# gphocs-dev/G-PhoCS

Hardware: AMD Instinct MI355X
Metric: locus-likelihood evals/sec (+ MCMC iters/sec), 100k loci, 1/2/4/8 MI355X (higher is better)
Workload: dtype f64

## Files before the change

g-phocs_amd/csrc/gph_backend.h:

```cpp
#pragma once

struct GphGrid { int x, y; };


#ifdef GPH_HOSTEMU
#define SETDEV(e) ((void)0)

struct gph_engine : gph_engine_state {
  std::vector<char> lds;
};

static int dev_alloc(void **p, size_t bytes) { *p = calloc(1, bytes ? bytes : 1); return *p ? 0 : GPH_EHIP; }
static void dev_free(void *p) { free(p); }
static int h2d(gph_engine *, void *d, const void *h, size_t n) { memcpy(d, h, n); return 0; }
static int d2h(gph_engine *, void *h, const void *d, size_t n) { memcpy(h, d, n); return 0; }
static int acc_zero(gph_engine *, void *p, size_t bytes) { if (p) memset(p, 0, bytes); return 0; }
static int stream_sync(gph_engine *e) { e->n_syncs++; return 0; }
static int collect_times(gph_engine *) { return 0; }
static int tm_begin(gph_engine *, int) { return -1; }
static void tm_end(gph_engine *, int) {}
static int push_G(gph_engine *e) { e->G_dirty = false; return 0; }
static int pull_G(gph_engine *e) { e->n_syncs++; return 0; }
static int pull_row(gph_engine *e) { memcpy(e->h_red, e->d_red, sizeof(double) * GPH_RED_ROW); e->n_syncs++; return 0; }
static bool resident(const gph_engine *) { return false; }
static int flush_pending(gph_engine *) { return 0; }
static int stage_defer(gph_engine *, int, int, int, bool &queued) { queued = false; return 0; }
static void flat_launched(gph_engine *, int, int) {}

static int reduce_local(gph_engine *e, int sec, int ncols)
{
  double *red = e->d_red + sec * GPH_RED_STRIDE;
  for (int c = 0; c < ncols; c++) {
    double s = 0, mn = 1e300, mx = -1e300;
    for (int64_t g = 0; g < e->L; g++) {
      double v;
      if (sec == 0) v = e->dev.out[(size_t)g * GPH_OUT_SLOTS + c];
      else v = e->dev.stats[(size_t)g * ncols + c];
      s += v; mn = v < mn ? v : mn; mx = v > mx ? v : mx;
    }
    red[c] = s; red[GPH_RED_COLS + c] = mn; red[2 * GPH_RED_COLS + c] = mx;
  }
  red[3 * GPH_RED_COLS] = (double)*e->dev.err;
  return 0;
}

static int backend_open(gph_engine *e)
{
  e->G_h = (GphGlobal *)calloc(1, sizeof(GphGlobal));
  e->G_d = e->G_h;
  e->h_red = (double *)calloc(GPH_RED_ROW, sizeof(double));
  e->d_red = (double *)calloc(GPH_RED_ROW, sizeof(double));
  e->d_gather = e->d_red;
  return 0;
}
static void backend_close(gph_engine *e) { free(e->h_red); free(e->G_h); }
static int wide_terms_bytes(int P) { return 8 * P; }
static int zero_error_word(gph_engine *e) { if (e->dev.err) *e->dev.err = 0; return 0; }
static int loci_loaded(gph_engine *) { return 0; }
static int scan_lds_limit(gph_engine *) { return 0; }
static int peer_stream(gph_engine *, gph_comm *) { return 0; }
static void runtime_version(char *buf, size_t n) { snprintf(buf, n, "host emulation (no HIP runtime)"); }
#ifdef GPH_BOUNDS
static int oob_take(int32_t *where) { *where = gph_oob_word; gph_oob_word = 0; return 0; }
#endif

static void launch_pre(gph_engine *e)
{
  g_model = e->G_h->model; g_lay = e->lay; gph_G_emu = e->G_h;
  GPH_KA_MODEL(e->ka, e); e->ka.lay = e->lay; e->ka.G = e->G_h;
}
template <class... P, class... A>
static int launch_loci(gph_engine *e, int cls, void (*kernel)(int, GphKargs, GphDev, int, P...), A &&...args)
{
  launch_pre(e);
  for (auto &bk : e->buckets) {
    e->lds.assign(bk.lds_bytes + 8 * e->lay.Pmax + 64, 0);
    gph_sm = e->lds.data();
    for (int b = 0; b < bk.count; b++) kernel(b, e->ka, e->dev, bk.j0, static_cast<P>(args)...);
  }
  e->last_which = cls; e->cls_launches[cls] += 1; e->n_launches++;
  return 0;
}
template <class... P, class... A>
static int launch_wave(gph_engine *e, int cls, void (*kernel)(int, GphKargs, GphDev, int, P...), size_t lds_bytes, A &&...args)
{
  launch_pre(e);
  e->lds.assign(lds_bytes + 64, 0);
  gph_sm = e->lds.data();
  kernel(0, e->ka, e->dev, 0, static_cast<P>(args)...);
  e->last_which = cls; e->cls_launches[cls] += 1;
  return 0;
}
template <class... P, class... A>
static int run_blocks(std::vector<char> &lds, GphGrid grid, int block, size_t lds_bytes, void (*kernel)(GphBlk, P...), A &&...args)
{
  for (int x = 0; x < grid.x; x++)
    for (int y = 0; y < grid.y; y++) {
      lds.assign(lds_bytes + 64, 0);
      kernel(GphBlk{x, y, block, lds.data()}, static_cast<P>(args)...);
    }
  return 0;
}
template <class... P, class... A>
static int launch_grid(gph_engine *e, GphGrid grid, int block, size_t lds_bytes, void (*kernel)(GphBlk, P...), A &&...args)
{
  return run_blocks(e->lds, grid, block, lds_bytes, kernel, args...);
}

static int debug_math(const double *x, const double *y, int n, double *out, int)
{
  GphKargs ka;
  memset(&ka, 0, sizeof ka);
  fill_math_constants(ka);
  std::vector<char> lds;
  return run_blocks(lds, GphGrid{(n + 255) / 256, 1}, 256, 0, k_debug_math, ka, x, y, n, out);
}

#else
#define HIPCHK(x) do { hipError_t e_ = (x); if (e_ != hipSuccess) { fprintf(stderr, "gphocs_hip: %s failed: %s (%s:%d)\n", #x, hipGetErrorString(e_), __FILE__, __LINE__); return GPH_EHIP; } } while (0)
#define SETDEV(e) do { if (hipSetDevice((e)->cfg.device) != hipSuccess) return GPH_EHIP; } while (0)

struct gph_engine : gph_engine_state {
  unsigned *d_ticket = nullptr;
  int pend_nc0 = 0, pend_nc1 = 0;
  GphStageList pend_sl = {0, {0}, {0}};
  int pend_iteration = 0;
  hipStream_t stream = nullptr;
  hipStream_t stream_wide = nullptr;
  hipEvent_t ev_fork = nullptr, ev_join = nullptr;
  bool side_stream = true;
  struct Tm { hipEvent_t a, b; int which; };
  std::vector<Tm> tm;
  size_t tm_used = 0;
};

static int dev_alloc(void **p, size_t bytes) { return hipMalloc(p, bytes ? bytes : 16) == hipSuccess ? 0 : GPH_EHIP; }
static void dev_free(void *p) { if (p) (void)hipFree(p); }
static int collect_times(gph_engine *e)
{
  for (size_t i = 0; i < e->tm_used; i++) {
    float ms = 0;
    if (hipEventElapsedTime(&ms, e->tm[i].a, e->tm[i].b) == hipSuccess) { e->last_ms[e->tm[i].which] = ms; e->cls_ms[e->tm[i].which] += ms; }
  }
  e->tm_used = 0;
  return 0;
}
static int stream_sync(gph_engine *e)
{
  HIPCHK(hipStreamSynchronize(e->stream));
  e->n_syncs++;
  return collect_times(e);
}
static int h2d(gph_engine *e, void *d, const void *h, size_t n)
{
  HIPCHK(hipMemcpyAsync(d, h, n, hipMemcpyHostToDevice, e->stream));
  HIPCHK(hipStreamSynchronize(e->stream));
  return 0;
}
static int d2h(gph_engine *e, void *h, const void *d, size_t n)
{
  HIPCHK(hipMemcpyAsync(h, d, n, hipMemcpyDeviceToHost, e->stream));
  HIPCHK(hipStreamSynchronize(e->stream));
  return 0;
}
static int acc_zero(gph_engine *e, void *p, size_t bytes)
{
  if (p) HIPCHK(hipMemsetAsync(p, 0, bytes, e->stream));
  return 0;
}
static int tm_begin(gph_engine *e, int which)
{
  if (!((e->timing_mask >> which) & 1)) return -1;
  if (e->tm_used == e->tm.size()) {
    gph_engine::Tm t;
    if (hipEventCreate(&t.a) != hipSuccess || hipEventCreate(&t.b) != hipSuccess) return -1;
    e->tm.push_back(t);
  }
  e->tm[e->tm_used].which = which;
  (void)hipEventRecord(e->tm[e->tm_used].a, e->stream);
  return (int)e->tm_used++;
}
static void tm_end(gph_engine *e, int slot) { if (slot >= 0) (void)hipEventRecord(e->tm[slot].b, e->stream); }
static int push_G(gph_engine *e)
{
  e->G_dirty = false;
  return h2d(e, e->G_d, e->G_h, sizeof(GphGlobal));
}
static int pull_G(gph_engine *e)
{
  HIPCHK(hipMemcpyAsync(e->G_h, e->G_d, sizeof(GphGlobal), hipMemcpyDeviceToHost, e->stream));
  { int rcs = stream_sync(e); if (rcs) return rcs; }
  e->mirror_current = true;
  return 0;
}
static int pull_row(gph_engine *e)
{
  HIPCHK(hipMemcpyAsync(e->h_red, e->d_red, sizeof(double) * GPH_RED_ROW, hipMemcpyDeviceToHost, e->stream));
  return stream_sync(e);
}
static bool resident(const gph_engine *e)
{
  if (e->force_host || e->allreduce || e->var_rates) return false;
  if (e->comm && !gph_comm_on_stream(e->comm)) return false;
  return true;
}
static void flat_launched(gph_engine *e, int cls, int k) { e->n_launches += k; if (cls >= 0) e->last_which = cls; }

static void launch_pre(gph_engine *e) { GPH_KA_MODEL(e->ka, e); e->ka.lay = e->lay; e->ka.G = e->G_d; }
template <class... P, class... A>
static int launch_on(hipStream_t stream, GphGrid grid, int block, size_t lds_bytes, void (*kernel)(P...), A &&...args)
{
  hipLaunchKernelGGL(kernel, dim3((unsigned)grid.x, (unsigned)grid.y), dim3((unsigned)block), lds_bytes, stream, static_cast<P>(args)...);
  HIPCHK(hipGetLastError());
  return 0;
}
template <class... P, class... A>
static int launch_grid(gph_engine *e, GphGrid grid, int block, size_t lds_bytes, void (*kernel)(P...), A &&...args)
{
  return launch_on(e->stream, grid, block, lds_bytes, kernel, args...);
}

static int flush_pending(gph_engine *e)
{
  const bool red = e->pend_nc0 > 0 || e->pend_nc1 > 0;
  if (!red && e->pend_sl.n == 0) return 0;
  const GphStageList sl = e->pend_sl;
  const int nc0 = e->pend_nc0, nc1 = e->pend_nc1;
  e->pend_nc0 = e->pend_nc1 = 0;
  e->pend_sl.n = 0;
  const bool multi = e->comm && gph_comm_world(e->comm) > 1;
  int rc;
  launch_pre(e);
  if (red) {
    const bool inkernel = multi && e->peer_rows != nullptr;
    const int fuse = sl.n > 0 && (!multi || inkernel);
    GphPeerX X{1, 0, 0, 0, nullptr, nullptr, nullptr, 0};
    if (inkernel) X = GphPeerX{gph_comm_world(e->comm), gph_comm_rank(e->comm), e->peer_stride, 0, e->peer_rows, e->peer_flags, e->d_gather, gph_comm_peer_next_gen(e->comm)};
    if ((rc = launch_grid(e, GphGrid{GPH_RED_BLOCKS, 1}, GPH_RED_THREADS, 0, k_reduce_stage, e->ka, e->dev, nc0, nc1, e->d_part, e->d_ticket,
                          e->d_red, fuse, sl, e->pend_iteration, X))) return rc;
    e->n_launches++;
    if (inkernel) {
      e->n_collectives++;
    } else if (multi) {
      if (gph_comm_allgather_stream(e->comm, e->d_red, e->d_gather, GPH_RED_ROW, (void *)e->stream)) return GPH_EHIP;
      e->n_collectives++;
    } else if (e->comm) {
      e->n_collectives++;
      if (gph_comm_allgather_stream(e->comm, e->d_red, e->d_gather, GPH_RED_ROW, (void *)e->stream)) return GPH_EHIP;
    }
    if (fuse) return 0;
  }
  if (sl.n > 0) {
    const double *rows = e->comm ? e->d_gather : e->d_red;
    if ((rc = launch_grid(e, GphGrid{1, 1}, GPH_RED_THREADS, 0, k_global, e->ka, rows, world_of(e), sl, e->pend_iteration))) return rc;
    e->n_launches++;
  }
  return 0;
}
static int reduce_local(gph_engine *e, int sec, int ncols)
{
  if (resident(e)) {
    if (e->pend_sl.n > 0) { int rcf = flush_pending(e); if (rcf) return rcf; }
    if (sec == 0) e->pend_nc0 = ncols; else e->pend_nc1 = ncols;
    return 0;
  }
  int rc;
  if ((rc = flush_pending(e))) return rc;
  GphStageList none = {0, {0}, {0}};
  launch_pre(e);
  if ((rc = launch_grid(e, GphGrid{GPH_RED_BLOCKS, 1}, GPH_RED_THREADS, 0, k_reduce_stage, e->ka, e->dev, sec == 0 ? ncols : 0, sec == 1 ? ncols : 0,
                        e->d_part, e->d_ticket, e->d_red, 0, none, 0, GphPeerX{1, 0, 0, 0, nullptr, nullptr, nullptr, 0}))) return rc;
  e->n_launches += 1;
  return 0;
}
static int stage_defer(gph_engine *e, int stage, int arg, int iteration, bool &queued)
{
  queued = resident(e);
  if (!queued) return flush_pending(e);
  if (e->pend_sl.n == 6) { int rcf = flush_pending(e); if (rcf) return rcf; }
  e->pend_sl.stage[e->pend_sl.n] = stage;
  e->pend_sl.arg[e->pend_sl.n] = arg;
  e->pend_sl.n++;
  e->pend_iteration = iteration;
  e->mirror_current = false;
  return 0;
}

template <class... P, class... A>
static int launch_loci(gph_engine *e, int cls, void (*kernel)(GphKargs, GphDev, int, P...), A &&...args)
{
  { int rcf = flush_pending(e); if (rcf) return rcf; }
  launch_pre(e);
  const int tms = tm_begin(e, cls);
  const size_t nb = e->buckets.size();
  const bool fork = e->side_stream && nb >= 2;
  if (fork) { HIPCHK(hipEventRecord(e->ev_fork, e->stream)); HIPCHK(hipStreamWaitEvent(e->stream_wide, e->ev_fork, 0)); }
  for (size_t bi = 0; bi < nb; bi++) {
    const gph_engine::Bucket &bk = e->buckets[bi];
    e->ka.lay.dyn_bytes = bk.lds_bytes;
    { int rcl = launch_on(fork && bi + 1 < nb ? e->stream_wide : e->stream, GphGrid{bk.count, 1}, GPH_WAVE, bk.lds_bytes + e->lds_pad[cls],
                          kernel, e->ka, e->dev, bk.j0, args...); if (rcl) return rcl; }
    e->n_launches++;
  }
  if (fork) { HIPCHK(hipEventRecord(e->ev_join, e->stream_wide)); HIPCHK(hipStreamWaitEvent(e->stream, e->ev_join, 0)); }
  tm_end(e, tms);
  e->last_which = cls; e->cls_launches[cls] += 1;
  return 0;
}
template <class... P, class... A>
static int launch_wave(gph_engine *e, int cls, void (*kernel)(GphKargs, GphDev, int, P...), size_t lds_bytes, A &&...args)
{
  { int rcf = flush_pending(e); if (rcf) return rcf; }
  launch_pre(e);
  const int tms = tm_begin(e, cls);
  { int rcl = launch_on(e->stream, GphGrid{1, 1}, GPH_WAVE, lds_bytes, kernel, e->ka, e->dev, 0, args...); if (rcl) return rcl; }
  tm_end(e, tms);
  e->last_which = cls; e->cls_launches[cls] += 1;
  return 0;
}

static int fill_math_tables(GphKargs &ka)
{
  void *p = nullptr;
  if (hipGetSymbolAddress(&p, HIP_SYMBOL(gph_log_t_d)) != hipSuccess) return 1;
  ka.log_t = (const double *)p;
  if (hipGetSymbolAddress(&p, HIP_SYMBOL(gph_exp_t_d)) != hipSuccess) return 1;
  ka.exp_t = (const uint64_t *)p;
  return 0;
}
static int backend_open(gph_engine *e)
{
  int ndev = 0;
  if (hipGetDeviceCount(&ndev) != hipSuccess || ndev <= e->cfg.device) {
    fprintf(stderr, "gphocs_hip: no usable HIP device %d (found %d) -- this library has no CPU path\n", e->cfg.device, ndev);
    return GPH_EHIP;
  }
  if (hipSetDevice(e->cfg.device) != hipSuccess || fill_math_tables(e->ka)) {
    fprintf(stderr, "gphocs_hip: cannot resolve the device math tables\n");
    return GPH_EHIP;
  }
  if (const char *ov = getenv("GPH_SIDE_STREAM")) e->side_stream = atoi(ov) != 0;
  const bool nb_ = getenv("GPH_NONBLOCKING_STREAM") && atoi(getenv("GPH_NONBLOCKING_STREAM")) != 0;
  if ((nb_ ? hipStreamCreateWithFlags(&e->stream, hipStreamNonBlocking) : hipStreamCreate(&e->stream)) != hipSuccess ||
      hipStreamCreateWithFlags(&e->stream_wide, hipStreamNonBlocking) != hipSuccess ||
      hipEventCreateWithFlags(&e->ev_fork, hipEventDisableTiming) != hipSuccess || hipEventCreateWithFlags(&e->ev_join, hipEventDisableTiming) != hipSuccess ||
      hipHostMalloc((void **)&e->G_h, sizeof(GphGlobal), hipHostMallocDefault) != hipSuccess ||
      hipMalloc((void **)&e->G_d, sizeof(GphGlobal)) != hipSuccess ||
      hipHostMalloc((void **)&e->h_red, sizeof(double) * GPH_RED_ROW * 64, hipHostMallocDefault) != hipSuccess ||
      hipMalloc((void **)&e->d_red, sizeof(double) * GPH_RED_ROW) != hipSuccess ||
      hipMemset(e->d_red, 0, sizeof(double) * GPH_RED_ROW) != hipSuccess ||
      hipMalloc((void **)&e->d_ticket, 64) != hipSuccess || hipMemset(e->d_ticket, 0, 64) != hipSuccess ||
      hipStreamSynchronize(nullptr) != hipSuccess) return GPH_EHIP;
  e->d_gather = e->d_red;
  return 0;
}
static void backend_close(gph_engine *e)
{
  dev_free(e->G_d);
  dev_free(e->d_ticket);
  if (e->h_red) (void)hipHostFree(e->h_red);
  if (e->G_h) (void)hipHostFree(e->G_h);
  for (auto &t : e->tm) { (void)hipEventDestroy(t.a); (void)hipEventDestroy(t.b); }
  if (e->ev_fork) (void)hipEventDestroy(e->ev_fork);
  if (e->ev_join) (void)hipEventDestroy(e->ev_join);
  if (e->stream_wide) (void)hipStreamDestroy(e->stream_wide);
  if (e->stream) (void)hipStreamDestroy(e->stream);
}
static int wide_terms_bytes(int) { return 0; }
static int zero_error_word(gph_engine *e)
{
  return hipMemset(e->dev.err, 0, sizeof(int32_t)) != hipSuccess || hipStreamSynchronize(nullptr) != hipSuccess ? GPH_EHIP : 0;
}
static int loci_loaded(gph_engine *e)
{
  const void *ks[] = {(const void *)k_init, (const void *)k_sweep, (const void *)k_tau_eval, (const void *)k_tau_finish,
                      (const void *)k_mix_eval, (const void *)k_mix_finish,
                      (const void *)k_sync, (const void *)k_check, (const void *)k_lrate_apply, (const void *)k_lrate_prep,
                      (const void *)k_unit};
  int pad_max = 0;
  if (const char *pe = getenv("GPH_LDS_PAD")) {
    for (const char *q = pe; *q;) {
      int w = -1, by = 0;
      if (sscanf(q, "%d:%d", &w, &by) == 2 && w >= 0 && w < 16 && by >= 0) { e->lds_pad[w] = by; pad_max = by > pad_max ? by : pad_max; }
      while (*q && *q != ',') q++;
      if (*q == ',') q++;
    }
  }
  if (e->lay.lds_bytes + pad_max + (int)sizeof(GphLds) > 160 * 1024) {
    fprintf(stderr, "gphocs_hip: %d-byte image + %d-byte sequence block%s = %d bytes of LDS per locus, the CU has %d%s\n", (int)sizeof(GphLds),
            e->lay.lds_bytes, pad_max ? " + GPH_LDS_PAD" : "", e->lay.lds_bytes + pad_max + (int)sizeof(GphLds), 160 * 1024,
            getenv("GPH_HUGE_LDS") ? " (GPH_HUGE_LDS is set: lower it, the block then stays in HBM)" : "");
    return GPH_EARG;
  }
  for (auto k : ks) HIPCHK(hipFuncSetAttribute(k, hipFuncAttributeMaxDynamicSharedMemorySize, e->lay.lds_bytes + pad_max));
  return 0;
}
static int scan_lds_limit(gph_engine *e)
{
  HIPCHK(hipFuncSetAttribute((const void *)k_lrate_scan, hipFuncAttributeMaxDynamicSharedMemorySize, e->lr_lds_bytes));
  return 0;
}
static int peer_stream(gph_engine *e, gph_comm *c)
{
  if (!(c && gph_comm_world(c) > 1 && gph_comm_on_stream(c))) return 0;
  double *rows = nullptr; unsigned long long *flags = nullptr; int32_t stride = 0;
  int least_ = 0, greatest_ = 0;
  if (hipDeviceGetStreamPriorityRange(&least_, &greatest_) != hipSuccess) { least_ = greatest_ = 0; }
  const int levels_ = least_ - greatest_ + 1;
  if (gph_comm_peer_exchange(c, &rows, &flags, &stride) && stride >= GPH_RED_ROW && gph_comm_world(c) > levels_) {
    if (gph_comm_rank(c) == 0)
      fprintf(stderr, "gphocs_hip: the in-kernel exchange is offered for up to %d thread ranks on one device (one stream priority level "
                      "each); %d ranks use the event-ordered gather\n", levels_, gph_comm_world(c));
  } else if (gph_comm_peer_exchange(c, &rows, &flags, &stride) && stride >= GPH_RED_ROW) {
    e->peer_rows = rows; e->peer_flags = flags; e->peer_stride = stride;
    hipStream_t ns = nullptr;
    int least = 0, greatest = 0;
    if (hipDeviceGetStreamPriorityRange(&least, &greatest) != hipSuccess) { least = greatest = 0; }
    const int levels = least - greatest + 1;
    const int prio = levels > 1 ? least - (gph_comm_rank(c) % levels) : 0;
    if (hipStreamSynchronize(e->stream) != hipSuccess || hipStreamCreateWithPriority(&ns, hipStreamNonBlocking, prio) != hipSuccess) return GPH_EHIP;
    (void)hipStreamDestroy(e->stream);
    e->stream = ns;
  }
  return 0;
}
static void runtime_version(char *buf, size_t n)
{
  int rt = 0, dr = 0;
  if (hipRuntimeGetVersion(&rt) != hipSuccess) rt = -1;
  if (hipDriverGetVersion(&dr) != hipSuccess) dr = -1;
  snprintf(buf, n, "HIP runtime %d, driver %d", rt, dr);
}
#ifdef GPH_BOUNDS
static int oob_take(int32_t *where)
{
  int w = 0, z = 0;
  HIPCHK(hipMemcpyFromSymbol(&w, HIP_SYMBOL(gph_oob_word), sizeof(int)));
  if (w != 0) HIPCHK(hipMemcpyToSymbol(HIP_SYMBOL(gph_oob_word), &z, sizeof(int)));
  *where = w;
  return 0;
}
#endif
static int debug_math(const double *x, const double *y, int n, double *out, int device)
{
  double *dx = nullptr, *dy = nullptr, *dout = nullptr;
  HIPCHK(hipSetDevice(device));
  HIPCHK(hipMalloc((void **)&dx, sizeof(double) * n));
  HIPCHK(hipMalloc((void **)&dy, sizeof(double) * n));
  HIPCHK(hipMalloc((void **)&dout, sizeof(double) * 5 * n));
  HIPCHK(hipMemcpy(dx, x, sizeof(double) * n, hipMemcpyHostToDevice));
  HIPCHK(hipMemcpy(dy, y, sizeof(double) * n, hipMemcpyHostToDevice));
  GphKargs ka;
  memset(&ka, 0, sizeof ka);
  fill_math_constants(ka);
  if (fill_math_tables(ka)) return GPH_EHIP;
  { int rcl = launch_on(nullptr, GphGrid{(n + 255) / 256, 1}, 256, 0, k_debug_math, ka, dx, dy, n, dout); if (rcl) return rcl; }
  HIPCHK(hipMemcpy(out, dout, sizeof(double) * 5 * n, hipMemcpyDeviceToHost));
  (void)hipFree(dx); (void)hipFree(dy); (void)hipFree(dout);
  return 0;
}
#endif
```

g-phocs_amd/csrc/gph_engine.hip:

```cpp
#include <stdio.h>
#include <stdlib.h>
#include <stddef.h>
#include <string.h>
#include <vector>
#include <string>
#include <algorithm>
#if defined(GPH_HOSTEMU) && defined(GPH_EMU64)
#define GPH_EMU64_IMPL
#endif
#include "gph_kernels.h"
#include "gph_global.h"
#include "gph_summary.h"
#include "gph_coalstats.h"
#include "gph_timeslices.h"
#include "gph_ancestry.h"
#include "gph_genetrees.h"
#include "gph_comm.h"
#include "../../include/gphocs_hip.h"

#ifdef GPH_HOSTEMU
thread_local char *gph_sm = nullptr;
thread_local GphLds gph_lds;
GphLayout g_lay;
GphModel g_model;
// ... 140 lines not shown
      if (col < ncols) reduce_run(src, stride, col, g0 + q, g1, GPH_RED_SUBS, s, mn, mx);
      for (int c0 = 64 * half; c0 < ncols && c0 < 64 * (half + 1); c0 += 16) {
        __syncthreads();
        if (col >= c0 && col < c0 + 16) { sh[0][q][col - c0] = s; sh[1][q][col - c0] = mn; sh[2][q][col - c0] = mx; }
        __syncthreads();
        if (threadIdx.x < 16 && c0 + (int)threadIdx.x < ncols) {
          const int c = threadIdx.x;
          double ts = 0.0, tmn = 1e300, tmx = -1e300;
          for (int k = 0; k < GPH_RED_SUBS; k++) {
            ts += sh[0][k][c];
            tmn = sh[1][k][c] < tmn ? sh[1][k][c] : tmn;
            tmx = sh[2][k][c] > tmx ? sh[2][k][c] : tmx;
          }
          part[(0 * GPH_RED_BLOCKS + b) * GPH_RED_COLS + c0 + c] = ts;
          part[(1 * GPH_RED_BLOCKS + b) * GPH_RED_COLS + c0 + c] = tmn;
          part[(2 * GPH_RED_BLOCKS + b) * GPH_RED_COLS + c0 + c] = tmx;
        }
      }
    }
    __syncthreads();
    return;
  }
  const int ng = 64 / cw, Q = GPH_RED_SUBS * ng;
  const int lane = threadIdx.x & 63, col = lane % cw, q = (threadIdx.x >> 6) * ng + lane / cw;
  double s = 0.0, mn = 1e300, mx = -1e300;
  if (col < ncols) reduce_run(src, stride, col, g0 + q, g1, Q, s, mn, mx);
  for (int c0 = 0; c0 < ncols; c0 += 16) {
    __syncthreads();
    if (col >= c0 && col < c0 + 16) { sh[0][q][col - c0] = s; sh[1][q][col - c0] = mn; sh[2][q][col - c0] = mx; }
    __syncthreads();
    if (threadIdx.x < 16 && c0 + (int)threadIdx.x < ncols) {
      const int c = threadIdx.x;
      double ts = 0.0, tmn = 1e300, tmx = -1e300;
      for (int k = 0; k < Q; k++) {
        ts += sh[0][k][c];
        tmn = sh[1][k][c] < tmn ? sh[1][k][c] : tmn;
        tmx = sh[2][k][c] > tmx ? sh[2][k][c] : tmx;
      }
      part[(0 * GPH_RED_BLOCKS + b) * GPH_RED_COLS + c0 + c] = ts;
      part[(1 * GPH_RED_BLOCKS + b) * GPH_RED_COLS + c0 + c] = tmn;
      part[(2 * GPH_RED_BLOCKS + b) * GPH_RED_COLS + c0 + c] = tmx;
    }
  }
  __syncthreads();
}
__device__ void reduce_final_body(int ncols, int cbase, const double *part, double *red, double (*sh)[GPH_RED_SUBS][128])
{
  part += cbase; red += cbase;
  const int cw = ncols <= 64 ? 64 : 128;
  const int col = threadIdx.x % cw, h = threadIdx.x / cw;
  const int per = GPH_RED_BLOCKS / GPH_RED_SUBS;
  static_assert((GPH_RED_BLOCKS / GPH_RED_SUBS) % 16 == 0, "the final pass folds sixteen block partials per step");
  for (int sub = h; sub < GPH_RED_SUBS; sub += GPH_RED_THREADS / cw) {
    double s = 0.0, mn = 1e300, mx = -1e300;
    if (col < ncols)
      for (int b0 = sub * per; b0 < (sub + 1) * per; b0 += 16) {
        double vs[16], vn[16], vx[16];
#pragma unroll
        for (int u = 0; u < 16; u++) {
          vs[u] = part[(0 * GPH_RED_BLOCKS + b0 + u) * GPH_RED_COLS + col];
          vn[u] = part[(1 * GPH_RED_BLOCKS + b0 + u) * GPH_RED_COLS + col];
          vx[u] = part[(2 * GPH_RED_BLOCKS + b0 + u) * GPH_RED_COLS + col];
        }
#pragma unroll
        for (int u = 0; u < 16; u++) { s += vs[u]; mn = vn[u] < mn ? vn[u] : mn; mx = vx[u] > mx ? vx[u] : mx; }
      }
    if (col < 128) { sh[0][sub][col] = s; sh[1][sub][col] = mn; sh[2][sub][col] = mx; }
  }
  __syncthreads();
  if (h == 0 && col < ncols) {
    double s = 0.0, mn = 1e300, mx = -1e300;
    for (int k = 0; k < GPH_RED_SUBS; k++) {
      s += sh[0][k][col];
      mn = sh[1][k][col] < mn ? sh[1][k][col] : mn;
      mx = sh[2][k][col] > mx ? sh[2][k][col] : mx;
    }
    red[col] = s;
    red[GPH_RED_COLS + col] = mn;
    red[2 * GPH_RED_COLS + col] = mx;
  }
  __syncthreads();
}
struct GphPeerX { int world, rank, stride, pad; double *rows; unsigned long long *flags; double *gather; unsigned long long gen; };
__global__ void __launch_bounds__(GPH_RED_THREADS) k_reduce_stage(GphKargs KA, GphDev D, int nc0, int nc1, double *part, unsigned *ticket, double *red,
                                                                  int do_stage, GphStageList SL, int iteration, GphPeerX X)
{
  __shared__ union { double p[3][GPH_RED_SUBS * 4][16]; double f[3][GPH_RED_SUBS][128]; GphStageShared st; } sh;
  __shared__ int s_last;
  if (nc0 > 0) reduce_partial_body(D, 0, nc0, 0, nc0, part, sh.p);
  for (int cb = 0; cb < nc1; cb += 128) reduce_partial_body(D, 1, nc1 - cb < 128 ? nc1 - cb : 128, cb, nc1, part + 3 * GPH_RED_BLOCKS * GPH_RED_COLS, sh.p);
  __syncthreads();
  if (threadIdx.x == 0) { __threadfence(); s_last = atomicAdd(ticket, 1u) == gridDim.x - 1; }
  __syncthreads();
  if (!s_last) return;
  __builtin_amdgcn_fence(__ATOMIC_ACQUIRE, "agent");
  if (nc0 > 0) reduce_final_body(nc0, 0, part, red, sh.f);
  for (int cb = 0; cb < nc1; cb += 128) reduce_final_body(nc1 - cb < 128 ? nc1 - cb : 128, cb, part + 3 * GPH_RED_BLOCKS * GPH_RED_COLS, red + GPH_RED_STRIDE, sh.f);
  if (threadIdx.x == 0) { red[3 * GPH_RED_COLS] = (double)*D.err; *ticket = 0; }
  __syncthreads();
  const double *rows = red;
  int world = 1;
  if (X.world > 1) {
    double *mine = X.rows + (size_t)(2 * X.rank + (int)(X.gen & 1)) * X.stride;
    for (int c = threadIdx.x; c < GPH_RED_ROW; c += blockDim.x) mine[c] = red[c];
    __threadfence_system();
    __syncthreads();
    if (threadIdx.x == 0) {
      __atomic_thread_fence(__ATOMIC_RELEASE);
      __hip_atomic_store(&X.flags[X.rank], X.gen, __ATOMIC_RELEASE, __HIP_MEMORY_SCOPE_SYSTEM);
      const unsigned long long t0 = __builtin_amdgcn_s_memrealtime();
      for (int r = 0; r < X.world; r++) {
        while (__hip_atomic_load(&X.flags[r], __ATOMIC_ACQUIRE, __HIP_MEMORY_SCOPE_SYSTEM) < X.gen) {
          __builtin_amdgcn_s_sleep(32);
          if (__builtin_amdgcn_s_memrealtime() - t0 > 400000000ull) {
            atomicMax(D.err, 9997); red[3 * GPH_RED_COLS] = 9997.0; r = X.world; break; }
        }
      }
    }
    __syncthreads();
    __threadfence_system();
    for (int r = 0; r < X.world; r++) {
      const double *src = r == X.rank ? red : X.rows + (size_t)(2 * r + (int)(X.gen & 1)) * X.stride;
      for (int c = threadIdx.x; c < GPH_RED_ROW; c += blockDim.x) X.gather[(size_t)r * GPH_RED_ROW + c] = src[c];
    }
    __syncthreads();
    rows = X.gather; world = X.world;
  }
  if (do_stage) stages_body(KA, rows, world, SL, iteration, sh.st);
}
#endif

#ifdef GPH_HOSTEMU
static void k_debug_math(GphBlk b, GphKargs KA, const double *x, const double *y, int n, double *o)
{
  (void)KA;
  for (int i = b.x * b.dim; i < (b.x + 1) * b.dim && i < n; i++) {
    o[i] = gph_exp(x[i]); o[n + i] = gph_log(x[i]); o[2 * n + i] = sqrt(fabs(x[i]));
    o[3 * n + i] = x[i] / y[i]; o[4 * n + i] = floor(x[i]);
  }
}
#else
__global__ void k_debug_math(GphKargs KA, const double *x, const double *y, int n, double *o)
{
  int i = blockIdx.x * blockDim.x + threadIdx.x;
  if (i >= n) return;
  o[i] = gph_exp(x[i]);
  o[n + i] = gph_log(x[i]);
  o[2 * n + i] = sqrt(fabs(x[i]));
  o[3 * n + i] = x[i] / y[i];
  o[4 * n + i] = floor(x[i]);
}
#endif

#define GPH_NCLS 18
struct SmRows {
  char *d = nullptr;
  size_t esz = 0;
  int32_t n = 0, cap = 0, fill = 0;
};
struct SmParts {
  double *d_part = nullptr;
  int32_t rd = 0, chunk = 0, nchunks = 0;
  int32_t chunk_next = 0;
};

struct gph_engine_state {
  gph_config cfg;
  std::vector<int32_t> samplesPerPop, popFather, popSon0, popSon1, bandSrc, bandTgt;
  GphLayout lay;
  GphDev dev;
  GphGlobal *G_h = nullptr, *G_d = nullptr;
  bool G_dirty = true;
  int64_t n_huge = 0;
  double *peer_rows = nullptr;
  unsigned long long *peer_flags = nullptr;
  std::vector<void *> deferred_free;
  int32_t peer_stride = 0;
  int32_t last_error_code = 0;
  long long last_error_locus = -1;
  bool in_error_dump = false;
  int64_t L = 0;
  size_t cond_bytes = 0, pages_bytes = 0, seq_bytes_total = 0;
  std::vector<uint64_t> h_cond_off;
  std::vector<int32_t> h_P;
  std::vector<int32_t> h_orig;
  struct Bucket { int j0, count, lds_bytes; };
  std::vector<Bucket> buckets;
  double *d_mutRate = nullptr;
  int init_predraws = 0;
  bool var_rates = false;
  GphLrRec *d_lrec = nullptr;
  GphLrPre *d_lpre = nullptr;
  double lr_hits = 0;
  int32_t *d_slot_of = nullptr;
  double *d_lr_result = nullptr, *d_lr_gscr = nullptr;
  char *d_ref_page = nullptr, *d_ref_seq = nullptr;
  std::vector<uint64_t> h_seq_off;
  GphLrArgs lr;
  int lr_lds_bytes = 0;
  int lds_pad[16] = {0};
  double *d_part = nullptr, *d_red = nullptr, *d_gather = nullptr;
  double *h_red = nullptr;
  gph_comm *comm = nullptr;
  gph_allreduce_fn allreduce = nullptr;
  void *allreduce_user = nullptr;
  bool force_host = false;
  int64_t n_syncs = 0, n_collectives = 0, n_launches = 0;
  uint32_t seedz = 0;
  bool loaded = false, seeded = false, model_set = false, initialized = false;
  GphKargs ka;
  bool sync_pending = false;
  bool fin_owed = false;
  bool mix_owed = false;
  int32_t slog_sel = 0;
  bool mirror_current = true;
  bool no_fuse = false;
  gph_counters counters = {0, 0, 0.0, 0};
  struct { double *d = nullptr; int32_t ncol = 0; int64_t samples = 0; std::vector<std::string> names; } ls;
  struct { SmParts part; SmRows rows; int32_t bd = 0; std::string name; } cs;
  struct { SmParts part; SmRows rows; GphTsShape shape = {}; std::string name; } ts;
  struct { double *d_acc = nullptr; SmRows rows; int32_t ncol = 0; int64_t samples = 0; GphAnShape shape = {}; std::vector<int32_t> iters; std::string name; } an;
  struct { SmRows rows; GphGtShape shape = {}; int32_t *d_sel = nullptr; std::vector<int64_t> sel; std::vector<int32_t> iters; } gt;
  double last_ms[GPH_NCLS] = {0};
  double cls_launches[GPH_NCLS] = {0}, cls_ms[GPH_NCLS] = {0};
  double cls_evals0[16] = {0}, cls_bytes0[16] = {0}, cls_nodes0[16] = {0};
  int last_which = 0;
  uint32_t timing_mask = 0xffffffffu;
};

static int align_up(int x, int a) { return (x + a - 1) / a * a; }

static void build_layout(GphLayout &y, int n, int Kc, int K, int B, int rootPop, int Pmax, int cnt16)
{
  memset(&y, 0, sizeof y);
  y.n = n; y.N = 2 * n - 1; y.K = K; y.Kc = Kc; y.B = B; y.rootPop = rootPop;
  y.E = 2 * n + 4 * GPH_MAX_MIGS + 3 * B + K + 10;
  y.RB = GPH_MAX_MIGS + 2 * B;
#define OFS(f) ((int32_t)offsetof(GphLds, f))
  y.o_ev = OFS(ev); y.o_nd = OFS(nd); y.o_sv = OFS(sv); y.o_mig_age = OFS(mig_age);
  y.o_coal = OFS(coal); y.o_migst = OFS(migst); y.o_rb_age = OFS(rb_age); y.o_fscal = OFS(fscal);
  y.o_iscal = OFS(iscal);
  y.o_nev = OFS(nev);
  y.o_first = OFS(first);
  y.o_mig_i = OFS(mig_i); y.o_living = OFS(living); y.o_ncoal = OFS(ncoal); y.o_nmig = OFS(nmig); y.o_rb_i = OFS(rb_i);
  y.page_bytes = align_up(OFS(s_dcoal), 16);
#undef OFS
  y.Pmax = Pmax;
  y.cnt16 = cnt16;
  y.dyn_bytes = 0;
  y.lds_bytes = GPH_Q_TERMS(Pmax, n, cnt16) + (Pmax > GPH_WAVE ? 8 * Pmax : 8 * GPH_WAVE);
  y.huge_P = 0x7fffffff;
}

static void build_model_static(gph_engine_state *e)
{
  GphModel &m = e->G_h->model;
  const gph_config &c = e->cfg;
  memset(&m, 0, sizeof m);
  for (int p = 0; p < c.K; p++) {
    m.popFather[p] = e->popFather[p];
    m.popSon0[p] = e->popSon0[p];
    m.popSon1[p] = e->popSon1[p];
    gph_popmask mask = 0;
    for (int d = 0; d < c.K; d++) {
      int x = d;
      while (x >= 0) { if (x == p) { mask |= (gph_popmask)1 << d; break; } x = e->popFather[x]; }
    }
    m.isAnc[p] = mask;
  }
  int cum = 0;
  for (int p = 0; p < c.Kc; p++) { m.samplesPerPop[p] = e->samplesPerPop[p]; cum += e->samplesPerPop[p]; m.cumSamples[p] = cum; }
  for (int b = 0; b < c.B; b++) { m.bandSrc[b] = e->bandSrc[b]; m.bandTgt[b] = e->bandTgt[b]; m.bandsInto[e->bandTgt[b]][b >> 5] |= 1u << (b & 31); }
  for (int p = 0; p < c.K; p++)
    for (int b = 0; b < c.B; b++) if ((m.isAnc[e->bandTgt[b]] >> p) & 1) m.bandsOver[p][b >> 5] |= 1u << (b & 31);
  std::vector<int> order;
  struct Rec { static void go(gph_engine_state *e, int pop, std::vector<int> &o) {
    if (pop >= e->cfg.Kc) { go(e, e->popSon0[pop], o); go(e, e->popSon1[pop], o); }
    o.push_back(pop); } };
  Rec::go(e, c.rootPop, order);
  for (size_t i = 0; i < order.size(); i++) m.postOrder[i] = order[i];
  GphGlobal &G = *e->G_h;
  G.n = c.n; G.K = c.K; G.Kc = c.Kc; G.B = c.B; G.rootPop = c.rootPop; G.Ltot = (double)c.L_total;
  G.tau_limit = (long long)1 << 62;
}

#ifdef GPH_WALKSTAT
long long gph_ws[4];
struct GphWsPrint { ~GphWsPrint() { fprintf(stderr, "WALKSTAT proposals %lld: prune steps %.2f, regraft steps %.2f, common prefix %.2f per proposal\n", gph_ws[3], (double)gph_ws[0] / gph_ws[3], (double)gph_ws[1] / gph_ws[3], (double)gph_ws[2] / gph_ws[3]); } } gph_ws_print;
#endif
#if GPH_BIG_BANDS
#define GPH_KA_MODEL(ka, e) ((void)0)
#else
#define GPH_KA_MODEL(ka, e) ((ka).model = (e)->G_h->model)
#endif
static void fill_math_constants(GphKargs &ka)
{
  const double ec[8] = GPH_EXP_CONSTS, lc[18] = GPH_LOG_CONSTS;
  const double rc[6] = {1.0 / 30269.0, 1.0 / 30307.0, 1.0 / 30323.0, 30269.0, 30307.0, 30323.0};
  memcpy(&ka.mathc[0], ec, sizeof ec);
  memcpy(&ka.mathc[8], lc, sizeof lc);
  memcpy(&ka.mathc[26], rc, sizeof rc);
}
static int world_of(const gph_engine *e);
#include "gph_backend.h"
static int world_of(const gph_engine *e) { return e->comm ? gph_comm_world(e->comm) : 1; }
static int push_if_dirty(gph_engine *e) { return e->G_dirty ? push_G(e) : 0; }

static int reduce_stats(gph_engine *e) { return reduce_local(e, 1, 2 * e->cfg.K + 2 * e->cfg.B); }

struct StageCols { int ns = 0, nm = 0, nx = 0; int s[GPH_RED_COLS + 32][2], m[8][2], x[8][2]; };
static void stage_columns(const gph_engine *e, int stage, StageCols &c)
{
  const int C = 2 * e->cfg.K + 2 * e->cfg.B;
  auto S = [&](int sec, int col) { c.s[c.ns][0] = sec; c.s[c.ns][1] = col; c.ns++; };
  auto M = [&](int sec, int col) { c.m[c.nm][0] = sec; c.m[c.nm][1] = col; c.nm++; };
  auto X = [&](int sec, int col) { c.x[c.nx][0] = sec; c.x[c.nx][1] = col; c.nx++; };
  auto counters = [&]() { S(0, 8); S(0, 9); S(0, 10); S(0, 13); X(0, 11); X(0, -1); };
  auto totals = [&]() { for (int k = 0; k < C; k++) S(1, k); };
  switch (stage) {
  case GS_INIT_DONE: counters(); S(0, 0); S(0, 1); totals(); break;
  case GS_SWEEP_DONE: counters(); for (int k = 0; k < 8; k++) S(0, k); S(0, 12); M(0, 15); totals(); break;
  case GS_TOTALS: totals(); break;
  case GS_TAU_DECIDE: case GS_SAGE_DECIDE: counters(); S(0, 0); S(0, 1); S(0, 3); S(0, 4); M(0, 14); break;
  case GS_MIX_DECIDE: counters(); S(0, 0); break;
  case GS_REFRESH_DONE: counters(); M(0, 0); S(0, 1); S(0, 2); break;
  case GS_CHECK_DONE: counters(); M(0, 0); S(0, 1); S(0, 2); totals(); break;
  case GS_COUNT_ONLY: counters(); S(0, 0); S(0, 1); S(0, 3); S(0, 4); M(0, 14); break;
  default: break;
  }
}
static bool stage_reads_row(int stage)
{
  switch (stage) {
  case GS_INIT_DONE: case GS_SWEEP_DONE: case GS_TOTALS: case GS_TAU_DECIDE: case GS_SAGE_DECIDE: case GS_MIX_DECIDE:
  case GS_REFRESH_DONE: case GS_CHECK_DONE: case GS_COUNT_ONLY: return true;
  default: return false;
  }
}
static double *colp(double *row, const int sc[2], int kind)
{
  if (sc[1] < 0) return row + 3 * GPH_RED_COLS;
  return row + sc[0] * GPH_RED_STRIDE + kind * GPH_RED_COLS + sc[1];
}

static int run_stage(gph_engine *e, int stage, int arg, int iteration)
{
  int rc;
  bool queued;
  if ((rc = stage_defer(e, stage, arg, iteration, queued)) || queued) return rc;
  GphRed R;
  R.rows = e->h_red; R.world = 1;
  if (stage_reads_row(stage)) {
    if ((rc = pull_row(e))) return rc;
    if (e->allreduce || e->comm) {
      StageCols c;
      stage_columns(e, stage, c);
      double sums[GPH_RED_COLS + 32], mins[16];
      for (int k = 0; k < c.ns; k++) sums[k] = *colp(e->h_red, c.s[k], 0);
      for (int k = 0; k < c.nm; k++) mins[k] = *colp(e->h_red, c.m[k], 1);
      for (int k = 0; k < c.nx; k++) mins[c.nm + k] = -*colp(e->h_red, c.x[k], 2);
      if (e->allreduce) rc = e->allreduce(e->allreduce_user, sums, c.ns, mins, c.nm + c.nx);
      else rc = gph_comm_allreduce_host(e->comm, sums, c.ns, mins, c.nm + c.nx);
      if (rc) return GPH_EHIP;
      e->n_collectives++;
      for (int k = 0; k < c.ns; k++) *colp(e->h_red, c.s[k], 0) = sums[k];
      for (int k = 0; k < c.nm; k++) *colp(e->h_red, c.m[k], 1) = mins[k];
      for (int k = 0; k < c.nx; k++) *colp(e->h_red, c.x[k], 2) = -mins[c.nm + k];
    }
  }
  e->G_h->iteration = iteration;
  gg_stage(*e->G_h, R, stage, arg);
  return push_G(e);
}

static void dump_one_locus(const gph_engine *e, FILE *f, long long global_locus, const char *pg, const char *cb, int P)
{
  const GphLayout &y = e->lay;
  const double *fs = (const double *)(pg + y.o_fscal);
  const int32_t *is = (const int32_t *)(pg + y.o_iscal);
  const GphNode *nd = (const GphNode *)(pg + y.o_nd);
  const int16_t *ne = (const int16_t *)(pg + y.o_nev);
  const int16_t *first = (const int16_t *)(pg + y.o_first);
  const GphEv *evr = (const GphEv *)(pg + y.o_ev);
  fprintf(f, "LOCUS %lld root %d dataLnL %a genLnL %a rng %u %u %u\n", (long long)global_locus, is[IS_ROOT],
          fs[FS_DATALNL], fs[FS_GENLNL], (unsigned)is[IS_RX], (unsigned)is[IS_RY], (unsigned)is[IS_RZ]);
  if (e->var_rates) fprintf(f, "R %a\n", fs[FS_MUTRATE]);
  for (int i = 0; i < y.N; i++)
    fprintf(f, "N %d %d %d %d %a %d %d\n", i, nd[i].father, nd[i].left, nd[i].right, nd[i].age, nd[i].npop, i < y.n ? -1 : ne[i]);
  for (int pop = 0; pop < y.K; pop++) {
    fprintf(f, "C %d", pop);
    int guard = 0;
    for (int ev = first[pop]; ev >= 0 && guard++ < y.E; ev = evr[ev].next)
      fprintf(f, " %d:%d:%d:%d:%a", ev, evr[ev].type, evr[ev].node, evr[ev].nlin, evr[ev].time);
    fprintf(f, "\n");
  }
  fprintf(f, "S");
  for (int pop = 0; pop < y.K; pop++)
    fprintf(f, " %a %d", ((const double *)(pg + y.o_coal))[pop], ((const int16_t *)(pg + y.o_ncoal))[pop]);
  for (int b = 0; b < y.B; b++)
    fprintf(f, " %a %d", ((const double *)(pg + y.o_migst))[b], ((const int16_t *)(pg + y.o_nmig))[b]);
  fprintf(f, "\n");
  fprintf(f, "M %d", is[IS_NUM_MIGS]);
  for (int i = 0; i < is[IS_NUM_MIGS]; i++) {
    int mg = ((const int16_t *)(pg + y.o_living))[i];
    const int16_t *mi = (const int16_t *)(pg + y.o_mig_i) + mg * MG_COUNT;
    fprintf(f, " %d:%d:%d:%d:%d:%d:%d:%a", mg, mi[MG_BRANCH], mi[MG_BAND], mi[MG_SPOP], mi[MG_TPOP], mi[MG_SEV],
            mi[MG_TEV], ((const double *)(pg + y.o_mig_age))[mg]);
  }
  fprintf(f, "\n");
  if (cb) {
    for (int i = y.n; i < y.N; i++) {
      const double *c = (const double *)(cb + ((size_t)((int)(((uint32_t)is[IS_CBIT0 + (i >> 5)] >> (i & 31)) & 1) * (y.n - 1) + (i - y.n)) * P) * 32);
      fprintf(f, "K %d", i);
      for (int k = 0; k < 4 * P; k++) fprintf(f, " %a", c[k]);
      fprintf(f, "\n");
    }
  }
}

static void eng_free(gph_engine *e, void *p)
{
  if (!p) return;
  if (e->peer_rows) e->deferred_free.push_back(p);
  else dev_free(p);
}

static int check_error(gph_engine *e)
{
  const int code = e->G_h->error;
  if (code != 0) {
    const long long gl = e->G_h->error_locus;
    e->last_error_code = code;
    e->last_error_locus = gl;
    if (code == 75) fprintf(stderr, "gphocs_hip: synchronizeEvents found an inconsistency (Fatal Error 0075/0076)\n");
    else if (code == 9999) fprintf(stderr, "gphocs_hip: checkAll failed at iteration %d\n", e->G_h->iteration);
    else if (gl >= 0) fprintf(stderr, "gphocs_hip: Fatal Error %04d reported by a locus kernel, first in locus %lld (iteration %d)\n", code, gl, e->G_h->iteration);
    else fprintf(stderr, "gphocs_hip: Fatal Error %04d reported by a locus kernel\n", code);
    const long long lo = gl - e->cfg.locus_begin;
    if (gl >= 0 && lo >= 0 && lo < e->L && !e->in_error_dump) {
      e->in_error_dump = true;
      int64_t slot = -1;
      for (int64_t j = 0; j < e->L; j++) if (e->h_orig[j] == lo) { slot = j; break; }
      std::vector<char> pg(e->lay.page_bytes);
      if (slot >= 0 && !d2h(e, pg.data(), (const char *)e->dev.pages + (size_t)slot * e->lay.page_bytes, e->lay.page_bytes)) {
        fprintf(stderr, "gphocs_hip: genealogy and event chains of locus %lld:\n", gl);
        dump_one_locus(e, stderr, gl, pg.data(), nullptr, 0);
      }
      e->in_error_dump = false;
    }
    return GPH_EKERNEL;
  }
  return 0;
}
static int finish_sync(gph_engine *e)
{
  { int rcf = flush_pending(e); if (rcf) return rcf; }
  if (resident(e)) { int rc = pull_G(e); if (rc) return rc; }
  return check_error(e);
}

static int run_stage_now(gph_engine *e, int stage, int arg);
static int mix_finish_owed(gph_engine *e)
{
  if (!e->mix_owed) return 0;
  e->mix_owed = false;
  return launch_loci(e, 7, k_mix_finish, 0);
}
static int flush_sync(gph_engine *e, bool now)
{
  int rc;
  if ((rc = mix_finish_owed(e))) return rc;
  if (!e->sync_pending) return 0;
  e->sync_pending = false;
  if ((rc = push_if_dirty(e))) return rc;
  if ((rc = launch_loci(e, 8, k_sync, 0))) return rc;
  if ((rc = reduce_local(e, 0, GPH_OUT_SLOTS))) return rc;
  if (now) return run_stage_now(e, GS_REFRESH_DONE, 0);
  return run_stage(e, GS_REFRESH_DONE, 0, e->G_h->iteration);
}

static int run_stage_now(gph_engine *e, int stage, int arg)
{
  const bool fh = e->force_host;
  e->force_host = true;
  int rc = run_stage(e, stage, arg, e->G_h->iteration);
  e->force_host = fh;
  if (rc) return rc;
  return check_error(e);
}

extern "C" {

int gph_engine_create(const gph_config *cfg, gph_engine **out)
{
  if (!cfg || !out) return GPH_EARG;
  if (cfg->n > 200 || cfg->K > 39 || cfg->B > 100)
    fprintf(stderr, "gphocs_hip: n=%d K=%d B=%d exceed even the reference's compile-time caps (NS 200, 2*NSPECIES-1 = 39, MAX_MIG_BANDS 100: upstream src/patch.h:17-22)\n", cfg->n, cfg->K, cfg->B);
  if (cfg->n < 2 || cfg->n > GPH_CAP_LEAVES || cfg->K > GPH_CAP_K || cfg->B > GPH_CAP_B || cfg->K != 2 * cfg->Kc - 1) {
    fprintf(stderr, "gphocs_hip: unsupported dimensions n=%d K=%d B=%d (this library variant: n<=%d leaves, K<=%d populations, B<=%d bands; the largest variant covers the reference's own caps 200 / 39 / 100, upstream src/patch.h:17-22)\n",
            cfg->n, cfg->K, cfg->B, GPH_CAP_LEAVES, GPH_CAP_K, GPH_CAP_B);
    return GPH_EARG;
  }
  gph_engine *e = new gph_engine();
  e->cfg = *cfg;
  e->samplesPerPop.assign(cfg->samplesPerPop, cfg->samplesPerPop + cfg->Kc);
  e->popFather.assign(cfg->popFather, cfg->popFather + cfg->K);
  e->popSon0.assign(cfg->popSon0, cfg->popSon0 + cfg->K);
  e->popSon1.assign(cfg->popSon1, cfg->popSon1 + cfg->K);
  if (cfg->B > 0) { e->bandSrc.assign(cfg->bandSrc, cfg->bandSrc + cfg->B); e->bandTgt.assign(cfg->bandTgt, cfg->bandTgt + cfg->B); }
  e->cfg.samplesPerPop = e->samplesPerPop.data();
  e->cfg.popFather = e->popFather.data();
  e->cfg.popSon0 = e->popSon0.data();
  e->cfg.popSon1 = e->popSon1.data();
  e->cfg.bandSrc = e->bandSrc.data();
  e->cfg.bandTgt = e->bandTgt.data();
  memset(&e->dev, 0, sizeof e->dev);
  memset(&e->ka, 0, sizeof e->ka);
  fill_math_constants(e->ka);
  if (const char *fh = getenv("GPH_HOST_DECISIONS")) e->force_host = atoi(fh) != 0;
  if (const char *nf = getenv("GPH_NO_FUSE")) e->no_fuse = atoi(nf) != 0;
  if (int rc = backend_open(e)) { gph_engine_destroy(e); return rc; }
  memset(e->G_h, 0, sizeof(GphGlobal));
  e->G_h->error_locus = -1;
  build_model_static(e);
  *out = e;
  return 0;
}

void gph_engine_destroy(gph_engine *e)
{
  if (!e) return;
  dev_free(e->dev.pages); dev_free(e->dev.shadow); dev_free(e->dev.cond); dev_free((void *)e->dev.cond_off);
  dev_free((void *)e->dev.seq); dev_free((void *)e->dev.seq_off); dev_free((void *)e->dev.orig); dev_free((void *)e->dev.P); dev_free(e->dev.out); dev_free(e->dev.stats); dev_free(e->d_mutRate);
  dev_free(e->d_lrec); dev_free(e->d_lpre); dev_free(e->d_slot_of); dev_free(e->d_lr_result); dev_free(e->d_lr_gscr); dev_free(e->d_ref_page); dev_free(e->d_ref_seq);
  dev_free(e->d_part); dev_free(e->dev.err);
  dev_free(e->ls.d); dev_free(e->cs.part.d_part); dev_free(e->cs.rows.d); dev_free(e->ts.part.d_part); dev_free(e->ts.rows.d);
  dev_free(e->an.d_acc); dev_free(e->an.rows.d);
  dev_free(e->gt.rows.d); dev_free(e->gt.d_sel);
  for (void *p : e->deferred_free) dev_free(p);
  e->deferred_free.clear();
  dev_free((void *)e->dev.slog_map); dev_free(e->dev.slog); dev_free(e->dev.slog_n);
  if (e->d_gather != e->d_red) dev_free(e->d_gather);
  dev_free(e->d_red);
  backend_close(e);
  delete e;
}

int gph_engine_set_allreduce(gph_engine *e, gph_allreduce_fn fn, void *user)
{
  if (!e) return GPH_EARG;
  e->allreduce = fn;
  e->allreduce_user = user;
  return 0;
}

int gph_engine_set_comm(gph_engine *e, gph_comm *c)
{
  if (!e) return GPH_EARG;
  SETDEV(e);
  e->comm = c;
  if (e->d_gather != e->d_red) { dev_free(e->d_gather); e->d_gather = e->d_red; }
  if (c && gph_comm_world(c) > 1 && gph_comm_on_stream(c)) {
    if (gph_comm_world(c) > 64) return GPH_EARG;
    if (dev_alloc((void **)&e->d_gather, sizeof(double) * GPH_RED_ROW * gph_comm_world(c))) return GPH_EHIP;
  }
  e->peer_rows = nullptr; e->peer_flags = nullptr; e->peer_stride = 0;
  return peer_stream(e, c);
}

GphGlobal *gph_engine_global_(gph_engine *e) { if (!e) return nullptr; e->G_dirty = true; return e->G_h; }
const GphGlobal *gph_engine_global_ro_(gph_engine *e) { return e ? e->G_h : nullptr; }

int gph_engine_load_loci(gph_engine *e, int64_t L, const int64_t *poff, const uint8_t *leafcodes,
                         const uint16_t *numPhases, const int32_t *counts, const double *mutRates)
{
  if (!e || L <= 0 || !poff || !leafcodes || !numPhases || !counts) return GPH_EARG;
  if (e->loaded) { fprintf(stderr, "gphocs_hip: gph_engine_load_loci called twice on one engine\n"); return GPH_ESTATE; }
  SETDEV(e);
  const int n = e->cfg.n;
  int Pmax = 1;
  for (int64_t g = 0; g < L; g++) { int P = (int)(poff[g + 1] - poff[g]); if (P > Pmax) Pmax = P; if (P < 0) return GPH_EARG; }
  int cnt16 = 1;
  for (int64_t i = 0; i < poff[L]; i++) if (counts[i] < 0 || counts[i] > 65535) { cnt16 = 0; break; }
  if (const char *ov = getenv("GPH_CNT16")) cnt16 = cnt16 && atoi(ov) != 0;
  build_layout(e->lay, n, e->cfg.Kc, e->cfg.K, e->cfg.B, e->cfg.rootPop, Pmax, cnt16);
  {
    int budget = 32 * 1024;
    if (budget < (int)sizeof(GphLds) + 16 * 1024) budget = (int)sizeof(GphLds) + 16 * 1024;
    if (const char *ov = getenv("GPH_HUGE_LDS")) {
      budget = atoi(ov);
      if (budget <= 0) { fprintf(stderr, "gphocs_hip: GPH_HUGE_LDS=%s is not a byte count\n", ov); return GPH_EARG; }
    }
    if (budget > 160 * 1024) budget = 160 * 1024;
    int hp = GPH_WAVE;
    while (hp < Pmax && (int)sizeof(GphLds) + GPH_Q_BYTES(hp + 1, n, cnt16) <= budget) hp++;
    e->lay.huge_P = hp >= Pmax ? 0x7fffffff : hp;
  }
  e->L = L;
  e->h_orig.resize(L);
  for (int64_t g = 0; g < L; g++) e->h_orig[g] = (int32_t)g;
  std::stable_sort(e->h_orig.begin(), e->h_orig.end(), [&](int32_t a, int32_t b) {
    return (poff[a + 1] - poff[a]) > (poff[b + 1] - poff[b]); });
  e->buckets.clear();
  {
    int64_t nwide = 0, nhuge = 0;
    while (nhuge < L && (poff[e->h_orig[nhuge] + 1] - poff[e->h_orig[nhuge]]) > e->lay.huge_P) nhuge++;
    nwide = nhuge;
    while (nwide < L && (poff[e->h_orig[nwide] + 1] - poff[e->h_orig[nwide]]) > GPH_WAVE) nwide++;
    e->n_huge = nhuge;
    if (nhuge > 0 && e->cfg.locus_begin == 0)
      fprintf(stderr, "gphocs_hip: %lld loci with more than %d phased patterns (up to %d) keep their sequence block in HBM\n",
              (long long)nhuge, e->lay.huge_P, Pmax);
    if (nhuge > 0) {
      gph_engine::Bucket bk;
      bk.j0 = 0; bk.count = (int)nhuge;
      bk.lds_bytes = 64;
      e->buckets.push_back(bk);
    }
    if (nwide > nhuge) {
      const int pw = (int)(poff[e->h_orig[nhuge] + 1] - poff[e->h_orig[nhuge]]);
      gph_engine::Bucket bk;
      bk.j0 = (int)nhuge; bk.count = (int)(nwide - nhuge);
      bk.lds_bytes = GPH_Q_TERMS(pw, n, cnt16) + wide_terms_bytes(pw);
      e->buckets.push_back(bk);
    }
    if (nwide < L) {
      const int pn = (int)(poff[e->h_orig[nwide] + 1] - poff[e->h_orig[nwide]]);
      gph_engine::Bucket bk;
      bk.j0 = (int)nwide; bk.count = (int)(L - nwide);
      bk.lds_bytes = GPH_Q_BYTES(pn, n, cnt16);
      {
        auto resident = [](int bytes) { const int g = (bytes + 1279) / 1280; const int w = 128 / g; return w < 4 * GPH_SWEEP_WAVES_ ? w : 4 * GPH_SWEEP_WAVES_; };
        const int base = (int)sizeof(GphLds) + bk.lds_bytes;
        const int full = 8 * ((pn + 7) & ~7);
        e->lay.lds_sum = 1;
        if (resident(base + full) == resident(base)) bk.lds_bytes += full;
        else {
          int room = (base + 1279) / 1280 * 1280;
          while (resident(room + 1280) == resident(base)) room += 1280;
          bk.lds_bytes = (room - (int)sizeof(GphLds)) & ~15;
        }
        if (const char *ov = getenv("GPH_LDS_SUM")) {
          e->lay.lds_sum = atoi(ov) != 0;
          bk.lds_bytes = GPH_Q_BYTES(pn, n, cnt16) + (e->lay.lds_sum ? full : 0);
        }
      }
      e->buckets.push_back(bk);
    }
  }
  e->lay.lds_bytes = 0;
  for (auto &bk : e->buckets) if (bk.lds_bytes > e->lay.lds_bytes) e->lay.lds_bytes = bk.lds_bytes;
  e->h_cond_off.resize(L + 1);
  e->h_P.resize(L);
  std::vector<uint64_t> seq_off(L + 1);
  std::vector<double> rates(L, 1.0);
  uint64_t off = 0, soff = 0;
  for (int64_t j = 0; j < L; j++) {
    int64_t g = e->h_orig[j];
    int P = (int)(poff[g + 1] - poff[g]);
    e->h_P[j] = P;
    e->h_cond_off[j] = off;
    off += (uint64_t)2 * (n - 1) * P * 32;
    seq_off[j] = soff;
    soff += GPH_Q_BYTES(P, n, cnt16);
    if (P > e->lay.huge_P) soff += (uint64_t)8 * ((P + 1) & ~1);
    if (mutRates) rates[j] = mutRates[g];
  }
  e->h_cond_off[L] = off;
  seq_off[L] = soff;
  e->h_seq_off = seq_off;
  std::vector<char> seq(soff, 0);
  for (int64_t j = 0; j < L; j++) {
    int64_t g = e->h_orig[j];
    int P = e->h_P[j];
    char *blk = seq.data() + seq_off[j];
    for (int p = 0; p < P; p++) {
      for (int i = 0; i < n; i++) {
        uint8_t c = leafcodes[(size_t)(poff[g] + p) * n + i];
        if (c > 4) return GPH_EARG;
        blk[GPH_Q_LEAF + p * GPH_Q_NH(n) + (i >> 1)] |= (char)(c << ((i & 1) << 2));
      }
      ((uint16_t *)(blk + GPH_Q_PHASES(P, n)))[p] = numPhases[poff[g] + p];
      if (cnt16) ((uint16_t *)(blk + GPH_Q_COUNT(P, n)))[p] = (uint16_t)counts[poff[g] + p];
      else ((int32_t *)(blk + GPH_Q_COUNT(P, n)))[p] = counts[poff[g] + p];
    }
  }
  e->cond_bytes = off;
  e->seq_bytes_total = soff;
  e->pages_bytes = (size_t)L * e->lay.page_bytes;
  int rc = 0;
  rc |= dev_alloc((void **)&e->dev.pages, e->pages_bytes);
  rc |= dev_alloc((void **)&e->dev.shadow, e->pages_bytes);
  rc |= dev_alloc((void **)&e->dev.cond, e->cond_bytes);
  rc |= dev_alloc((void **)&e->dev.cond_off, sizeof(uint64_t) * (L + 1));
  rc |= dev_alloc((void **)&e->dev.seq, seq.size());
  rc |= dev_alloc((void **)&e->dev.seq_off, sizeof(uint64_t) * (L + 1));
  rc |= dev_alloc((void **)&e->dev.P, sizeof(int32_t) * 2 * L);
  rc |= dev_alloc((void **)&e->dev.orig, sizeof(int32_t) * L);
  rc |= dev_alloc((void **)&e->dev.out, sizeof(double) * GPH_OUT_SLOTS * L);
  rc |= dev_alloc((void **)&e->dev.stats, sizeof(double) * (2 * e->cfg.K + 2 * e->cfg.B) * L);
  rc |= dev_alloc((void **)&e->d_part, sizeof(double) * 2 * 3 * GPH_RED_BLOCKS * GPH_RED_COLS);
  rc |= dev_alloc((void **)&e->dev.err, sizeof(int32_t));
  if (!rc) rc = zero_error_word(e);
  if (mutRates) rc |= dev_alloc((void **)&e->d_mutRate, sizeof(double) * L);
  if (rc) { fprintf(stderr, "gphocs_hip: device allocation failed\n"); return GPH_EHIP; }
  rc |= h2d(e, (void *)e->dev.cond_off, e->h_cond_off.data(), sizeof(uint64_t) * (L + 1));
  rc |= h2d(e, (void *)e->dev.seq, seq.data(), seq.size());
  rc |= h2d(e, (void *)e->dev.seq_off, seq_off.data(), sizeof(uint64_t) * (L + 1));
  {
    std::vector<int32_t> pu((size_t)2 * L);
    for (int64_t j = 0; j < L; j++) {
      const int64_t g = e->h_orig[j];
      int U = 0;
      for (int64_t p = poff[g]; p < poff[g + 1]; p++) U += numPhases[p] > 0;
      pu[2 * j] = e->h_P[j]; pu[2 * j + 1] = U;
    }
    rc |= h2d(e, (void *)e->dev.P, pu.data(), sizeof(int32_t) * 2 * L);
  }
  rc |= h2d(e, (void *)e->dev.orig, e->h_orig.data(), sizeof(int32_t) * L);
  if (mutRates) rc |= h2d(e, e->d_mutRate, rates.data(), sizeof(double) * L);
  if (rc) return GPH_EHIP;
  e->dev.L = (int32_t)L;
  e->dev.Ltot = (int32_t)e->cfg.L_total;
  e->dev.locus_begin = e->cfg.locus_begin;
  e->loaded = true;
  return loci_loaded(e);
}

int gph_engine_set_model(gph_engine *e, const double *theta, const double *popAge, const double *sampleAge,
                         const double *migRate, const double *bandStart, const double *bandEnd)
{
  if (!e || !theta || !popAge || !sampleAge) return GPH_EARG;
  GphModel &m = e->G_h->model;
  for (int p = 0; p < e->cfg.K; p++) { gg_set_theta(*e->G_h, p, theta[p]); m.popAge[p] = popAge[p]; m.sampleAge[p] = sampleAge[p]; }
  for (int b = 0; b < e->cfg.B; b++) { gg_set_mig(*e->G_h, b, migRate[b]); m.bandStart[b] = bandStart[b]; m.bandEnd[b] = bandEnd[b]; }
  e->model_set = true;
  e->G_dirty = true;
  return 0;
}

int gph_engine_seed(gph_engine *e, uint32_t seed)
{
  if (!e) return GPH_EARG;
  e->seedz = 170u * (seed % 178u) + 137u;
  e->seeded = true;
  return 0;
}

int gph_engine_init_genealogies(gph_engine *e, double *sumGen, double *sumData)
{
  if (!e || !e->loaded || !e->seeded || !e->model_set) return GPH_ESTATE;
  SETDEV(e);
  { int rcf = flush_pending(e); if (rcf) return rcf; }
  e->mix_owed = e->fin_owed = e->sync_pending = false;
  if (e->G_h->mix_flag || e->G_h->tau_flag) { e->G_h->mix_flag = 0; e->G_h->tau_flag = 0; e->G_dirty = true; }
  { int rcp = push_if_dirty(e); if (rcp) return rcp; }
  if (e->ls.d && e->ls.ncol != gph_ls_columns(e->cfg.K, e->cfg.B, e->var_rates)) { int rce = gph_engine_locus_summary_enable(e, 1); if (rce) return rce; }
  e->ls.samples = e->an.samples = 0;
  e->cs.rows.fill = e->ts.rows.fill = e->an.rows.fill = e->gt.rows.fill = 0;
  e->an.iters.clear();
  e->gt.iters.clear();
  { int rcz = acc_zero(e, e->ls.d, sizeof(double) * (size_t)e->ls.ncol * e->L); if (rcz) return rcz; }
  { int rcz = acc_zero(e, e->an.d_acc, sizeof(double) * (size_t)e->an.ncol * e->L); if (rcz) return rcz; }
  int rc = launch_loci(e, 3, k_init, e->seedz, e->d_mutRate, e->init_predraws);
  if (!rc) rc = reduce_local(e, 0, GPH_OUT_SLOTS);
  if (!rc) rc = reduce_stats(e);
  if (rc) return rc;
  e->G_h->nrec = 0;
  e->G_h->iteration = -1;
  if ((rc = run_stage_now(e, GS_INIT_DONE, 0))) return rc;
  { GphRed R; R.rows = e->h_red; R.world = 1;
    if (sumGen) *sumGen = R.sum(0, 0);
    if (sumData) *sumData = R.sum(0, 1); }
  e->initialized = true;
  return rc;
}

static int sweep_launch(gph_engine *e, int flags, double ftCoal, double ftMig, int &with_sync)
{
  int rc;
  with_sync = e->sync_pending ? 8 : 0;
  e->sync_pending = false;
  int with_mix = 0;
  if (e->mix_owed) {
    if (!e->mirror_current && (rc = finish_sync(e))) return rc;
    e->mix_owed = false;
    if (e->G_h->mix_flag) with_mix = 16;
  }
  if ((rc = launch_loci(e, 0, k_sweep, flags | with_sync | with_mix, ftCoal, ftMig, e->G_h->mix_c, e->G_h->mix_lnc))) return rc;
  if ((rc = reduce_local(e, 0, GPH_OUT_SLOTS))) return rc;
  return reduce_stats(e);
}

int gph_engine_genealogy_sweep(gph_engine *e, int32_t flags, double ftCoal, double ftMig, gph_sweep_result *out)
{
  if (!e || !e->initialized || !out) return GPH_ESTATE;
  SETDEV(e);
  int rc, with_sync;
  if ((rc = push_if_dirty(e))) return rc;
  GphGlobal &G = *e->G_h;
  const int64_t a0 = G.acc[0], a1 = G.acc[1], a2 = G.acc[2], a7 = G.acc[7];
  if ((rc = sweep_launch(e, flags, ftCoal, ftMig, with_sync))) return rc;
  if ((rc = run_stage_now(e, GS_SWEEP_DONE, with_sync))) return rc;
  GphRed R; R.rows = e->h_red; R.world = 1;
  out->accepted_internal = G.acc[0] - a0;
  out->accepted_mignode = G.acc[1] - a1;
  out->accepted_spr = G.acc[2] - a2;
  out->total_mig_nodes = G.acc[7] - a7;
  out->dData_internal = R.sum(0, 3);
  out->dLog_internal = R.sum(0, 4);
  out->dLog_mignode = R.sum(0, 5);
  out->dData_spr = R.sum(0, 6);
  out->dLog_spr = R.sum(0, 7);
  return 0;
}

int gph_engine_tau_evaluate(gph_engine *e, const gph_tau_args *a, gph_tau_result *out)
{
  if (!e || !e->initialized || !a || !out) return GPH_ESTATE;
  if (a->num_aff > 2 * GPH_MAXB) return GPH_EARG;
  SETDEV(e);
  { int rcs = flush_sync(e, true); if (rcs) return rcs; }
  GphTauArgs &A = e->G_h->tau;
  memset(&A, 0, sizeof A);
  A.ap = a->ap; A.son0 = a->son0; A.son1 = a->son1; A.isRoot = a->isRoot; A.num_aff = a->num_aff; A.mode = a->mode;
  A.tauold = a->tauold; A.taunew = a->taunew; A.taub0 = a->taub0; A.taub1 = a->taub1;
  A.taufactor0 = a->taufactor0; A.taufactor1 = a->taufactor1;
  for (int i = 0; i < a->num_aff; i++) {
    A.aff_bands[i] = a->aff_bands[i];
    A.start_or_end[i] = a->start_or_end[i];
    A.new_band_ages[i] = a->new_band_ages[i];
  }
  int rc = push_G(e);
  if (rc) return rc;
  if ((rc = launch_loci(e, 1, k_tau_eval, 0))) return rc;
  if ((rc = reduce_local(e, 0, GPH_OUT_SLOTS))) return rc;
  if ((rc = run_stage_now(e, GS_COUNT_ONLY, 1))) return rc;
  GphRed R; R.rows = e->h_red; R.world = 1;
  out->ntj0 = (int64_t)R.sum(0, 0);
  out->ntj1 = (int64_t)R.sum(0, 1);
  out->genDelta = R.sum(0, 3);
  out->dataDelta = R.sum(0, 4);
  out->first_conflict_locus = R.mn(0, 14) < 1e299 ? (int64_t)R.mn(0, 14) : -1;
  return 0;
}

static int tau_finish_now(gph_engine *e, int flag, long long limit)
{
  if (!e || !e->initialized) return GPH_ESTATE;
  SETDEV(e);
  e->G_h->tau_flag = flag;
  e->G_h->tau_limit = limit;
  gg_fill_fin(*e->G_h, flag, limit);
  int rc = push_G(e);
  if (rc) return rc;
  return launch_loci(e, 5, k_tau_finish, 0);
}
int gph_engine_tau_commit(gph_engine *e) { return tau_finish_now(e, 1, (long long)1 << 62); }
int gph_engine_tau_revert(gph_engine *e, int64_t first_conflict)
{
  return tau_finish_now(e, 0, first_conflict >= 0 ? (long long)first_conflict : (long long)1 << 62);
}

int gph_engine_mixing_evaluate(gph_engine *e, double c, double *dataDelta)
{
  if (!e || !e->initialized || !dataDelta) return GPH_ESTATE;
  SETDEV(e);
  { int rcs = flush_sync(e, true); if (rcs) return rcs; }
  e->G_h->mix_c = c;
  int rc = push_G(e);
  if (rc) return rc;
  if ((rc = launch_loci(e, 2, k_mix_eval, 0))) return rc;
  if ((rc = reduce_local(e, 0, GPH_OUT_SLOTS))) return rc;
  if ((rc = run_stage_now(e, GS_COUNT_ONLY, 2))) return rc;
  GphRed R; R.rows = e->h_red; R.world = 1;
  *dataDelta = R.sum(0, 0);
  return 0;
}

int gph_engine_mixing_commit(gph_engine *e, double c, double lnc)
{
  if (!e || !e->initialized) return GPH_ESTATE;
  SETDEV(e);
  e->G_h->mix_flag = 1; e->G_h->mix_c = c; e->G_h->mix_lnc = lnc;
  int rc = push_G(e);
  if (rc) return rc;
  return launch_loci(e, 7, k_mix_finish, 0);
}

int gph_engine_mixing_revert(gph_engine *e) { return e ? 0 : GPH_EARG; }

static int finish_owed(gph_engine *e);
static int owed_finishes(gph_engine *e)
{
  int rc = finish_owed(e);
  if (!rc) rc = mix_finish_owed(e);
  return rc;
}
static int apply_list(gph_engine *e)
{
  int rc;
  if ((rc = owed_finishes(e))) return rc;
  if ((rc = flush_pending(e))) return rc;
  launch_pre(e);
  if ((rc = launch_grid(e, GphGrid{(int)((e->L + 255) / 256), 1}, 256, 0, k_apply_list, e->ka, e->dev))) return rc;
  flat_launched(e, -1, 1);
  return 0;
}

static int apply_one(gph_engine *e, int kind, int idx, int limit, double lnc, double diff)
{
  if (!e || !e->initialized || idx < 0 || idx >= limit) return GPH_EARG;
  SETDEV(e);
  { int rco = owed_finishes(e); if (rco) return rco; }
  GphGlobal &G = *e->G_h;
  G.napply = 1;
  G.apply[0].kind = kind; G.apply[0].idx = idx; G.apply[0].lnc = lnc; G.apply[0].diff = diff;
  int rc = push_G(e);
  if (rc) return rc;
  return apply_list(e);
}
int gph_engine_apply_theta(gph_engine *e, int32_t pop, double lnc, double thetaold, double thetanew)
{
  return apply_one(e, 0, pop, e ? e->cfg.K : 0, lnc, (1 / thetanew - 1 / thetaold));
}
int gph_engine_apply_migrate(gph_engine *e, int32_t band, double lnc, double old_rate, double new_rate)
{
  return apply_one(e, 1, band, e ? e->cfg.B : 0, lnc, (new_rate - old_rate));
}

int gph_engine_get_totals(gph_engine *e, double *cs, double *nc, double *ms, double *nm)
{
  if (!e || !e->initialized) return GPH_ESTATE;
  SETDEV(e);
  const int K = e->cfg.K, B = e->cfg.B;
  int rc;
  if ((rc = push_if_dirty(e))) return rc;
  if ((rc = mix_finish_owed(e))) return rc;
  if ((rc = reduce_stats(e))) return rc;
  if ((rc = run_stage_now(e, GS_TOTALS, 0))) return rc;
  const GphGlobal &G = *e->G_h;
  for (int p = 0; p < K; p++) { if (cs) cs[p] = G.tot_coal[p]; if (nc) nc[p] = G.tot_ncoal[p]; }
  for (int b = 0; b < B; b++) { if (ms) ms[b] = G.tot_mig[b]; if (nm) nm[b] = G.tot_nmig[b]; }
  return rc;
}

int gph_engine_synchronize(gph_engine *e, int32_t refresh, double *oldGen, double *newGen)
{
  if (!e || !e->initialized) return GPH_ESTATE;
  SETDEV(e);
  if (!refresh) {
    e->sync_pending = true;
    if (oldGen) *oldGen = 0.0;
    if (newGen) *newGen = 0.0;
    return 0;
  }
  int rc;
  if ((rc = flush_sync(e, true))) return rc;
  if ((rc = push_if_dirty(e))) return rc;
  if ((rc = launch_loci(e, 8, k_sync, refresh))) return rc;
  if ((rc = reduce_local(e, 0, GPH_OUT_SLOTS))) return rc;
  if ((rc = run_stage_now(e, GS_REFRESH_DONE, 0))) return rc;
  GphRed R; R.rows = e->h_red; R.world = 1;
  if (oldGen) *oldGen = R.sum(0, 1);
  if (newGen) *newGen = R.sum(0, 2);
  return rc;
}

int gph_engine_check_all(gph_engine *e, int32_t *ok, double *sumData, double *sumGen)
{
  if (!e || !e->initialized) return GPH_ESTATE;
  SETDEV(e);
  int rc;
  if ((rc = flush_sync(e, true))) return rc;
  if ((rc = push_if_dirty(e))) return rc;
  if ((rc = launch_loci(e, 4, k_check, 0))) return rc;
  if ((rc = reduce_local(e, 0, GPH_OUT_SLOTS))) return rc;
  if ((rc = reduce_stats(e))) return rc;
  e->G_h->nrec = 0;
  rc = run_stage_now(e, GS_CHECK_DONE, 0);
  if (ok) *ok = e->G_h->error != 9999;
  if (e->G_h->error == 9999) { e->G_h->error = 0; e->G_h->error_locus = -1; e->G_dirty = true; rc = 0; }
  { GphRed R; R.rows = e->h_red; R.world = 1;
    if (sumData) *sumData = R.sum(0, 1);
    if (sumGen) *sumGen = R.sum(0, 2); }
  return rc;
}

int gph_engine_get_counters(gph_engine *e, gph_counters *out, int32_t reset)
{
  if (!e || !out) return GPH_EARG;
  const GphGlobal &G = *e->G_h;
  double ev = 0, nd = 0, by = 0;
  for (int k = 0; k < 16; k++) { ev += G.cls_evals[k]; nd += G.cls_nodes[k]; by += G.cls_bytes[k]; }
  out->evals = (int64_t)ev - e->counters.evals;
  out->eval_nodes = (int64_t)nd - e->counters.eval_nodes;
  out->eval_bytes = by - e->counters.eval_bytes;
  out->not_enough_migs = (int64_t)G.cnt_notenough - e->counters.not_enough_migs;
  if (reset) { e->counters.evals = (int64_t)ev; e->counters.eval_nodes = (int64_t)nd; e->counters.eval_bytes = by; e->counters.not_enough_migs = (int64_t)G.cnt_notenough; }
  return 0;
}

int gph_engine_last_kernel_ms(gph_engine *e, int32_t which, double *ms)
{
  if (!e || !ms || which < 0 || which >= GPH_NCLS) return GPH_EARG;
  *ms = e->last_ms[which];
  return 0;
}

int64_t gph_engine_num_loci(gph_engine *e) { return e ? e->L : 0; }

int gph_engine_class_stats(gph_engine *e, int32_t which, double *out5, int32_t reset)
{
  if (!e || !out5 || which < 0 || which >= GPH_NCLS) return GPH_EARG;
  const GphGlobal &G = *e->G_h;
  if (which >= 16) {
    out5[0] = e->cls_launches[which]; out5[1] = e->cls_ms[which]; out5[2] = out5[3] = out5[4] = 0.0;
    if (reset) e->cls_launches[which] = e->cls_ms[which] = 0;
    return 0;
  }
  out5[0] = e->cls_launches[which]; out5[1] = e->cls_ms[which]; out5[2] = G.cls_evals[which] - e->cls_evals0[which];
  out5[3] = G.cls_bytes[which] - e->cls_bytes0[which]; out5[4] = G.cls_nodes[which] - e->cls_nodes0[which];
  if (reset) {
    e->cls_launches[which] = e->cls_ms[which] = 0;
    e->cls_evals0[which] = G.cls_evals[which]; e->cls_bytes0[which] = G.cls_bytes[which]; e->cls_nodes0[which] = G.cls_nodes[which];
  }
  return 0;
}

int gph_engine_host_stats(gph_engine *e, int64_t *syncs, int64_t *collectives, int64_t *launches, int32_t *resident_mode)
{
  if (!e) return GPH_EARG;
  if (syncs) *syncs = e->n_syncs;
  if (collectives) *collectives = e->n_collectives;
  if (launches) *launches = e->n_launches;
  if (resident_mode) *resident_mode = resident(e) ? 1 : 0;
  return 0;
}
int gph_engine_set_timing(gph_engine *e, uint32_t class_mask)
{
  if (!e) return GPH_EARG;
  e->timing_mask = class_mask;
  return 0;
}

int gph_debug_math(const double *x, const double *y, int32_t n, double *out, int32_t device)
{
  if (!x || !y || !out || n <= 0) return GPH_EARG;
  return debug_math(x, y, n, out, device);
}

#ifndef GPH_BUILD_ID
#define GPH_BUILD_ID "unidentified"
#endif
const char *gph_build_id(void) { return GPH_BUILD_ID; }
const char *gph_build_compiler(void)
{
#ifdef __clang_version__
  return "clang " __clang_version__;
#else
  return "g++ " __VERSION__;
#endif
}
const char *gph_runtime_version(void)
{
  static char buf[96];
  runtime_version(buf, sizeof buf);
  return buf;
}

int gph_engine_steplog_enable(gph_engine *e, const int64_t *loci, int32_t n, int32_t cap)
{
#if !defined(GPH_LOGSTEPS) && !defined(GPH_BBCOUNT)
  (void)e; (void)loci; (void)n; (void)cap;
  return GPH_EARG;
#else
  if (!e || !e->loaded || n < 0 || cap < 1 || (n > 0 && !loci)) return GPH_EARG;
  SETDEV(e);
  if (e->initialized) { int rcs = flush_sync(e, true); if (!rcs) rcs = finish_sync(e); if (rcs) return rcs; }
  eng_free(e, (void *)e->dev.slog_map); eng_free(e, e->dev.slog); eng_free(e, e->dev.slog_n);
  e->dev.slog_map = nullptr; e->dev.slog = nullptr; e->dev.slog_n = nullptr; e->dev.slog_cap = 0;
  e->slog_sel = n;
  if (n == 0) return 0;
  std::vector<int32_t> map((size_t)e->L, -1);
  for (int64_t j = 0; j < e->L; j++)
    for (int k = 0; k < n; k++)
      if (e->h_orig[j] + e->cfg.locus_begin == loci[k]) map[j] = k;
  std::vector<int32_t> zero((size_t)n, 0);
  int32_t *d_map = nullptr, *d_n = nullptr;
  double *d_log = nullptr;
  if (dev_alloc((void **)&d_map, sizeof(int32_t) * e->L) || dev_alloc((void **)&d_log, sizeof(double) * 8 * (size_t)n * cap) ||
      dev_alloc((void **)&d_n, sizeof(int32_t) * n) ||
      h2d(e, d_map, map.data(), sizeof(int32_t) * e->L) || h2d(e, d_n, zero.data(), sizeof(int32_t) * n)) {
    eng_free(e, d_map); eng_free(e, d_log); eng_free(e, d_n);
    e->slog_sel = 0;
    return GPH_EHIP;
  }
  e->dev.slog_map = d_map; e->dev.slog = d_log; e->dev.slog_n = d_n;
  e->dev.slog_cap = cap;
  return 0;
#endif
}
int gph_engine_steplog_fetch(gph_engine *e, int32_t idx, double *out, int32_t max_records, int32_t *nrec, int32_t reset)
{
#if !defined(GPH_LOGSTEPS) && !defined(GPH_BBCOUNT)
  (void)e; (void)idx; (void)out; (void)max_records; (void)nrec; (void)reset;
  return GPH_EARG;
#else
  if (!e || !e->dev.slog || idx < 0 || idx >= e->slog_sel || !nrec) return GPH_EARG;
  SETDEV(e);
  { int rcs = finish_sync(e); if (rcs) return rcs; }
  int32_t n = 0;
  if (d2h(e, &n, e->dev.slog_n + idx, sizeof n)) return GPH_EHIP;
  *nrec = n;
#ifdef GPH_BBCOUNT
  n = e->dev.slog_cap;
#endif
  const int32_t m = std::min(std::min(n, e->dev.slog_cap), max_records);
  if (out && m > 0 && d2h(e, out, e->dev.slog + (size_t)idx * e->dev.slog_cap * 8, sizeof(double) * 8 * (size_t)m)) return GPH_EHIP;
  if (reset) { const int32_t z = 0; if (h2d(e, e->dev.slog_n + idx, &z, sizeof z)) return GPH_EHIP; }
  return 0;
#endif
}

int gph_engine_hbm_bytes(gph_engine *e, double *bytes)
{
  if (!e || !bytes) return GPH_EARG;
  *bytes = 2.0 * e->pages_bytes + (double)e->cond_bytes + (double)e->seq_bytes_total + 8.0 * GPH_OUT_SLOTS * e->L;
  return 0;
}

int gph_engine_set_locus_rates(gph_engine *e, const double *rates, int32_t draws, int32_t variable)
{
  if (!e || !e->loaded || e->initialized || !rates || draws < 0) return GPH_ESTATE;
  SETDEV(e);
  std::vector<double> r(e->L);
  for (int64_t j = 0; j < e->L; j++) r[j] = rates[e->h_orig[j]];
  if (!e->d_mutRate && dev_alloc((void **)&e->d_mutRate, sizeof(double) * e->L)) return GPH_EHIP;
  if (h2d(e, e->d_mutRate, r.data(), sizeof(double) * e->L)) return GPH_EHIP;
  e->init_predraws = draws;
  e->var_rates = variable != 0;
  return 0;
}

static int xreduce(gph_engine *e, double *sums, int nsum, double *mins, int nmin)
{
  int rc = 0;
  if (e->allreduce) rc = e->allreduce(e->allreduce_user, sums, nsum, mins, nmin);
  else if (e->comm) rc = gph_comm_allreduce_host(e->comm, sums, nsum, mins, nmin);
  else return 0;
  e->n_collectives++;
  return rc ? GPH_EHIP : 0;
}
static bool multi_rank(const gph_engine *e) { return e->allreduce || (e->comm && gph_comm_world(e->comm) > 1); }
static int lr_share(gph_engine *e, bool mine, std::vector<double> &v)
{
  if (!multi_rank(e)) return 0;
  for (size_t off = 0; off < v.size(); off += 24) {
    double buf[24];
    const int nn = (int)(v.size() - off < 24 ? v.size() - off : 24);
    for (int i = 0; i < nn; i++) buf[i] = mine ? v[off + i] : 0.0;
    int rc = xreduce(e, buf, nn, nullptr, 0);
    if (rc) return rc;
    for (int i = 0; i < nn; i++) v[off + i] = buf[i];
  }
  return 0;
}

int gph_engine_locus_rate_update(gph_engine *e, double finetune, double alpha, gph_locus_rate_result *io)
{
  if (!e || !e->initialized || !io) return GPH_ESTATE;
  io->accepted = 0;
  if (finetune <= 0.0) return 0;
  const bool owner = e->cfg.locus_begin == 0;
  SETDEV(e);
  if (!multi_rank(e) && (!owner || e->cfg.L_total != e->L)) {
    fprintf(stderr, "gphocs_hip: UpdateLocusRate over a shard of the loci needs the all-reduce hook (gph_engine_set_allreduce)\n");
    return GPH_EARG;
  }
  int rc = 0;
  if ((rc = flush_sync(e, true))) return rc;
  if ((rc = push_if_dirty(e))) return rc;
  const GphLayout &y = e->lay;
  const int n = e->cfg.n, N = 2 * n - 1;
  std::vector<char> refpg(y.page_bytes, 0);
  int jr = -1;
  if (owner) {
    for (int64_t j = 0; j < e->L; j++) if (e->h_orig[j] == 0) jr = (int)j;
    if ((rc = d2h(e, refpg.data(), e->dev.pages + (size_t)jr * y.page_bytes, y.page_bytes))) return rc;
  }
  {
    std::vector<double> v(4 * N + 4, 0.0);
    if (owner) {
      const uint32_t *w = (const uint32_t *)(refpg.data() + y.o_nd);
      for (int i = 0; i < 4 * N; i++) v[i] = (double)w[i];
      v[4 * N] = ((const double *)(refpg.data() + y.o_fscal))[FS_MUTRATE];
      v[4 * N + 1] = ((const double *)(refpg.data() + y.o_fscal))[FS_DATALNL];
      v[4 * N + 2] = (double)((const int32_t *)(refpg.data() + y.o_iscal))[IS_ROOT];
      v[4 * N + 3] = (double)e->h_P[jr];
    }
    if ((rc = lr_share(e, owner, v))) return rc;
    if (!owner) {
      uint32_t *w = (uint32_t *)(refpg.data() + y.o_nd);
      for (int i = 0; i < 4 * N; i++) w[i] = (uint32_t)v[i];
      ((double *)(refpg.data() + y.o_fscal))[FS_MUTRATE] = v[4 * N];
      ((double *)(refpg.data() + y.o_fscal))[FS_DATALNL] = v[4 * N + 1];
      ((int32_t *)(refpg.data() + y.o_iscal))[IS_ROOT] = (int32_t)v[4 * N + 2];
    }
    e->lr.ref_P = (int32_t)v[4 * N + 3];
    e->lr.rref0 = v[4 * N];
    e->lr.likref0 = v[4 * N + 1];
  }
  const int Pr = e->lr.ref_P, Pmax = y.Pmax > Pr ? y.Pmax : Pr;
  if (!e->d_lrec) {
    std::vector<int32_t> slot_of(e->L);
    for (int64_t j = 0; j < e->L; j++) slot_of[e->h_orig[j]] = (int32_t)j;
    const int seqb = align_up(GPH_Q_TERMS(Pmax, n, y.cnt16) + (Pmax > GPH_WAVE ? 8 * Pmax : 0), 16), ndb = N * (int)sizeof(GphNode);
    const int fixed = 2 * seqb + 2 * ndb;
    const int progb = GPH_BIG_TREE ? 0 : (n - 1) * GPH_WAVE * 16;
    const int lfb = !GPH_BIG_TREE && Pr >= 1 && Pr <= GPH_WAVE ? n * Pr * 32 : 0;
    const int budget = 96 * 1024 - (int)sizeof(GphLds) - progb - align_up(N * 8, 16) - lfb;
    int Pscr = (budget - fixed) / ((n - 1) * 32);
    if (const char *ov = getenv("GPH_LR_PSCR")) Pscr = atoi(ov) < Pscr ? atoi(ov) : Pscr;
    if (Pscr > Pmax) Pscr = Pmax;
    if (Pscr < 0) Pscr = 0;
    const double finetune0 = e->lr.finetune; (void)finetune0;
    const int32_t refP = e->lr.ref_P; const double r0 = e->lr.rref0, l0 = e->lr.likref0;
    memset(&e->lr, 0, sizeof e->lr);
    e->lr.ref_P = refP; e->lr.rref0 = r0; e->lr.likref0 = l0;
    e->lr.o_rseq = seqb; e->lr.o_gnd = 2 * seqb; e->lr.o_rnd = 2 * seqb + ndb; e->lr.o_scr = fixed; e->lr.Pscr = Pscr;
    e->lr.o_prog = fixed + (n - 1) * Pscr * 32;
    e->lr.o_pe = e->lr.o_prog + progb;
    e->lr.o_lf = lfb ? e->lr.o_pe + align_up(N * 8, 16) : 0;
    e->lr_lds_bytes = e->lr.o_pe + align_up(N * 8, 16) + lfb;
    {
      const int lds_max = 160 * 1024;
      double too_big[1] = {e->lr_lds_bytes + (int)sizeof(GphLds) > lds_max ? 1.0 : 0.0};
      if (multi_rank(e) && (rc = xreduce(e, too_big, 1, nullptr, 0))) return rc;
      if (too_big[0] != 0.0) {
        if (e->lr_lds_bytes + (int)sizeof(GphLds) > lds_max)
          fprintf(stderr, "gphocs_hip: locus-mut-rate VAR: the serial scan of UpdateLocusRate needs %d bytes of LDS for two sequence "
                          "blocks of up to %d phased patterns (%d bytes each) next to the %d-byte image; the CU has %d\n",
                  e->lr_lds_bytes, Pmax, seqb, (int)sizeof(GphLds), lds_max);
        memset(&e->lr, 0, sizeof e->lr);
        return GPH_EARG;
      }
    }
    e->lr.ref_seq_bytes = GPH_Q_BYTES(Pr, n, y.cnt16);
    rc |= dev_alloc((void **)&e->d_lrec, sizeof(GphLrRec) * e->L);
    rc |= dev_alloc((void **)&e->d_lpre, sizeof(GphLrPre) * e->L);
    rc |= dev_alloc((void **)&e->d_slot_of, sizeof(int32_t) * e->L);
    rc |= dev_alloc((void **)&e->d_lr_result, sizeof(double) * 16);
    rc |= dev_alloc((void **)&e->d_lr_gscr, Pmax > Pscr ? sizeof(double) * 4 * (size_t)(n - 1) * Pmax : 16);
    rc |= dev_alloc((void **)&e->d_ref_page, y.page_bytes);
    rc |= dev_alloc((void **)&e->d_ref_seq, e->lr.ref_seq_bytes + 16);
    if (rc) return GPH_EHIP;
    if (h2d(e, e->d_slot_of, slot_of.data(), sizeof(int32_t) * e->L)) return GPH_EHIP;
    e->lr.result = e->d_lr_result; e->lr.rec = e->d_lrec; e->lr.pre = e->d_lpre; e->lr.slot_of = e->d_slot_of; e->lr.gscr = e->d_lr_gscr;
    std::vector<char> seqblk(e->lr.ref_seq_bytes + 16, 0);
    if (owner && e->lr.ref_seq_bytes > 0 &&
        (rc = d2h(e, seqblk.data(), e->dev.seq + e->h_seq_off[jr], e->lr.ref_seq_bytes))) return rc;
    {
      std::vector<double> v(e->lr.ref_seq_bytes / 4, 0.0);
      if (owner) for (size_t i = 0; i < v.size(); i++) v[i] = (double)((const uint32_t *)seqblk.data())[i];
      if ((rc = lr_share(e, owner, v))) return rc;
      if (!owner) for (size_t i = 0; i < v.size(); i++) ((uint32_t *)seqblk.data())[i] = (uint32_t)v[i];
    }
    if (e->lr.ref_seq_bytes > 0 && h2d(e, e->d_ref_seq, seqblk.data(), e->lr.ref_seq_bytes)) return GPH_EHIP;
    e->lr.ref_seq = e->d_ref_seq;
    e->lr.ref_page = e->d_ref_page;
    if ((rc = scan_lds_limit(e))) return rc;
  }
  if (h2d(e, e->d_ref_page, refpg.data(), y.page_bytes)) return GPH_EHIP;
  e->lr.finetune = finetune; e->lr.alpha = alpha;
  e->lr.first = owner ? 1 : 0;
  if ((rc = launch_loci(e, 11, k_lrate_prep, finetune, e->d_lpre))) return rc;
  if ((rc = reduce_local(e, 0, GPH_OUT_SLOTS))) return rc;
  if ((rc = run_stage_now(e, GS_COUNT_ONLY, 11))) return rc;
  double st[8] = {0.0, e->lr.rref0, e->lr.likref0, io->dataLogLikelihood, io->logLikelihood, io->rateVar, 0.0, 0.0};
  double res[16] = {0};
  for (int guard = 0; (int64_t)st[0] < e->cfg.L_total; guard++) {
    if (guard > 1 << 20) return GPH_ESTATE;
    const bool mine = (int64_t)st[0] == e->cfg.locus_begin;
    double nx[8] = {0, 0, 0, 0, 0, 0, 0, 0};
    if (mine) {
      e->lr.rref0 = st[1]; e->lr.likref0 = st[2];
      e->lr.dataLnL = st[3]; e->lr.logL = st[4]; e->lr.rateVar = st[5];
      if ((rc = launch_wave(e, 9, k_lrate_scan, e->lr_lds_bytes, e->lr))) return rc;
      if ((rc = d2h(e, res, e->d_lr_result, sizeof res))) return rc;
      collect_times(e);
      if (res[4] != 0.0) { fprintf(stderr, "gphocs_hip: Fatal Error %04d reported by the locus-rate scan\n", (int)res[4]); return GPH_EKERNEL; }
      nx[0] = (double)(e->cfg.locus_begin + e->L); nx[1] = res[13]; nx[2] = res[14];
      nx[3] = res[1]; nx[4] = res[2]; nx[5] = res[3]; nx[6] = st[6] + res[0]; nx[7] = st[7] + res[5];
    }
    if (multi_rank(e)) { if ((rc = xreduce(e, nx, 8, nullptr, 0))) return rc; }
    else if (!mine) return GPH_ESTATE;
    if (nx[0] <= st[0]) { fprintf(stderr, "gphocs_hip: the ranks' locus blocks do not tile 0..L_total\n"); return GPH_EARG; }
    memcpy(st, nx, sizeof st);
  }
  if (owner) {
    GphLrRec r;
    const int32_t *is = (const int32_t *)(refpg.data() + y.o_iscal);
    r.rate = st[1]; r.lnl = st[2]; r.rx = (uint32_t)is[IS_RX]; r.ry = (uint32_t)is[IS_RY]; r.rz = (uint32_t)is[IS_RZ];
    r.flag = (int32_t)st[6] << 2;
    if (h2d(e, e->d_lrec + jr, &r, sizeof r)) return GPH_EHIP;
  }
  if ((rc = launch_loci(e, 10, k_lrate_apply, e->d_lrec))) return rc;
  if ((rc = reduce_local(e, 0, GPH_OUT_SLOTS))) return rc;
  if ((rc = run_stage_now(e, GS_COUNT_ONLY, 10))) return rc;
  io->accepted = (int64_t)st[6];
  io->dataLogLikelihood = st[3];
  io->logLikelihood = st[4];
  io->rateVar = st[5];
  e->lr_hits = st[7];
#ifdef GPH_LRSTAMP
  fprintf(stderr, "evaluator stamps: setup+exp %.0f, nodes %.0f, root %.0f cycles per call (%.0f calls, %.1f steps)\n", res[8] / res[11], res[9] / res[11], res[10] / res[11], res[11], res[12] / res[11]);
#endif
  if (getenv("GPH_LR_VERBOSE"))
    fprintf(stderr, "gphocs_hip: locus-rate scan: %.0f of %lld proposals decided with the prepared likelihood; %.3g shader cycles in %.3g s (%.0f MHz)\n",
            st[7], (long long)(e->cfg.L_total - 1), res[6], res[7] / 1e8, res[7] > 0 ? res[6] / (res[7] / 1e8) / 1e6 : 0.0);
  return 0;
}

static int finish_owed(gph_engine *e)
{
  if (!e->fin_owed) return 0;
  e->fin_owed = false;
  return launch_loci(e, 5, k_tau_finish, 0);
}
static int evaluate_fused(gph_engine *e, int cls, decltype(&k_tau_eval) kernel)
{
  int rc;
  if (e->no_fuse && (rc = finish_owed(e))) return rc;
  const int fuse = e->fin_owed;
  e->fin_owed = false;
  if ((rc = launch_loci(e, cls, kernel, fuse))) return rc;
  return reduce_local(e, 0, GPH_OUT_SLOTS);
}
static int part_sweep(gph_engine *e, int32_t iteration, double ftCoal, double ftMig)
{
  int rc, with_sync;
  if ((rc = sweep_launch(e, 7, ftCoal, ftMig, with_sync))) return rc;
  return run_stage(e, GS_SWEEP_DONE, with_sync, iteration);
}
static int part_lrate(gph_engine *e, int32_t iteration, const double *lr_alpha_finetune, int64_t *lr_accepted, double *lr_rateVar)
{
  int rc;
  GphGlobal &Gh = *e->G_h;
  gph_locus_rate_result R;
  R.accepted = 0; R.dataLogLikelihood = Gh.dataLogLikelihood; R.logLikelihood = Gh.logLikelihood; R.rateVar = *lr_rateVar;
  if ((rc = gph_engine_locus_rate_update(e, lr_alpha_finetune[1], lr_alpha_finetune[0], &R))) return rc;
  Gh.dataLogLikelihood = R.dataLogLikelihood; Gh.logLikelihood = R.logLikelihood; *lr_rateVar = R.rateVar;
  *lr_accepted += R.accepted;
  gg_rec(Gh, REC_LRATE, 0, (long long)R.accepted);
  if ((rc = push_G(e))) return rc;
  if ((rc = reduce_stats(e))) return rc;
  return run_stage(e, GS_TOTALS, 0, iteration);
}
static int part_tau(gph_engine *e, int32_t iteration, bool first_proposed)
{
  int rc;
  const GphGlobal &Gh = *e->G_h;
  const int K = Gh.K, Kc = Gh.Kc;
  for (int ap = Kc; ap < K; ++ap) {
    if ((ap > Kc || !first_proposed) && (rc = run_stage(e, GS_TAU_PROPOSE, ap, iteration))) return rc;
    if ((rc = evaluate_fused(e, 1, k_tau_eval))) return rc;
    if ((rc = run_stage(e, GS_TAU_DECIDE, ap, iteration))) return rc;
    e->fin_owed = true;
  }
  return run_stage(e, GS_TAU_END, 0, iteration);
}
static int part_sage(gph_engine *e, int32_t iteration)
{
  int rc;
  const GphGlobal &Gh = *e->G_h;
  for (int pop = 0; pop < Gh.Kc; ++pop) {
    if (!Gh.updateSampleAge[pop]) continue;
    if ((rc = run_stage(e, GS_SAGE_PROPOSE, pop, iteration))) return rc;
    if ((rc = evaluate_fused(e, 1, k_tau_eval))) return rc;
    if ((rc = run_stage(e, GS_SAGE_DECIDE, pop, iteration))) return rc;
    e->fin_owed = true;
  }
  return run_stage(e, GS_SAGE_END, 0, iteration);
}
static int part_mix(gph_engine *e, int32_t iteration)
{
  int rc;
  const GphGlobal &Gh = *e->G_h;
  if ((rc = run_stage(e, GS_MIX_PROPOSE, 0, iteration))) return rc;
  if (Gh.ftMixing > 0.0) {
    if ((rc = evaluate_fused(e, 2, k_mix_eval))) return rc;
    if ((rc = run_stage(e, GS_MIX_DECIDE, 0, iteration))) return rc;
    e->mix_owed = true;
    if (e->no_fuse) return mix_finish_owed(e);
  }
  return 0;
}
static int part_refresh(gph_engine *e, int32_t iteration)
{
  int rc;
  if ((rc = launch_loci(e, 8, k_sync, 1))) return rc;
  if ((rc = reduce_local(e, 0, GPH_OUT_SLOTS))) return rc;
  return run_stage(e, GS_REFRESH_DONE, 1, iteration);
}
static int part_check(gph_engine *e, int32_t iteration)
{
  int rc;
  if ((rc = flush_sync(e, false))) return rc;
  if ((rc = launch_loci(e, 4, k_check, 0))) return rc;
  if ((rc = reduce_local(e, 0, GPH_OUT_SLOTS))) return rc;
  if ((rc = reduce_stats(e))) return rc;
  return run_stage(e, GS_CHECK_DONE, 0, iteration);
}

int gph_engine_iteration_(gph_engine *e, int32_t iteration, const double *lr_alpha_finetune, int64_t *lr_accepted, double *lr_rateVar)
{
  if (!e || !e->initialized) return GPH_ESTATE;
  SETDEV(e);
  int rc;
  GphGlobal &Gh = *e->G_h;
  if ((rc = push_if_dirty(e))) return rc;
  if ((rc = part_sweep(e, iteration, Gh.ftCoalTime, Gh.ftMigTime))) return rc;
  if (lr_alpha_finetune && (rc = part_lrate(e, iteration, lr_alpha_finetune, lr_accepted, lr_rateVar))) return rc;
  if ((rc = run_stage(e, GS_THETA, 0, iteration))) return rc;
  if (Gh.Kc < Gh.K && (rc = run_stage(e, GS_TAU_PROPOSE, Gh.Kc, iteration))) return rc;
  if ((rc = apply_list(e))) return rc;
  if ((rc = part_tau(e, iteration, true))) return rc;
  if ((rc = part_sage(e, iteration))) return rc;
  if (Gh.doMixing && (rc = part_mix(e, iteration))) return rc;
  if ((rc = finish_owed(e))) return rc;
  if ((iteration == Gh.startMig || (iteration + 1) % Gh.samplesPerLog == 0) && (rc = mix_finish_owed(e))) return rc;
  if (iteration == Gh.startMig) {
    if ((rc = run_stage(e, GS_STARTMIG, 0, iteration))) return rc;
    if ((rc = part_refresh(e, iteration))) return rc;
  } else {
    e->sync_pending = true;
  }
  if ((iteration + 1) % Gh.samplesPerLog == 0 && (rc = part_check(e, iteration))) return rc;
  return finish_sync(e);
}

int gph_engine_part_(gph_engine *e, int32_t part, int32_t iteration, const double *lr_alpha_finetune, int64_t *lr_accepted, double *lr_rateVar)
{
  if (!e || !e->initialized) return GPH_ESTATE;
  SETDEV(e);
  int rc = 0;
  GphGlobal &Gh = *e->G_h;
  if ((rc = push_if_dirty(e))) return rc;
  if (part != GPH_PART_SWEEP && part != GPH_PART_SYNC) { int rcm = mix_finish_owed(e); if (rcm) return rcm; }
  if (part == GPH_PART_LRATE || part == GPH_PART_TAU || part == GPH_PART_SAGE || part == GPH_PART_MIX) {
    int rcs = flush_sync(e, true);
    if (rcs) return rcs;
  }
  switch (part) {
  case GPH_PART_SWEEP: rc = part_sweep(e, iteration, Gh.ftCoalTime, Gh.ftMigTime); break;
  case GPH_PART_LRATE: rc = lr_alpha_finetune ? part_lrate(e, iteration, lr_alpha_finetune, lr_accepted, lr_rateVar) : GPH_EARG; break;
  case GPH_PART_THETA: rc = run_stage(e, GS_THETA_ONLY, 0, iteration); if (!rc) rc = apply_list(e); break;
  case GPH_PART_MIGR: rc = run_stage(e, GS_MIGR_ONLY, 0, iteration); if (!rc) rc = apply_list(e); break;
  case GPH_PART_TAU: rc = part_tau(e, iteration, false); break;
  case GPH_PART_SAGE: rc = part_sage(e, iteration); break;
  case GPH_PART_MIX: rc = part_mix(e, iteration); break;
  case GPH_PART_SYNC: e->sync_pending = true; break;
  case GPH_PART_REFRESH: e->sync_pending = false; rc = part_refresh(e, iteration); break;
  case GPH_PART_CHECK: Gh.nrec = 0; e->G_dirty = true; rc = push_if_dirty(e); if (!rc) rc = part_check(e, iteration); break;
  default: return GPH_EARG;
  }
  if (rc) return rc;
  if ((rc = finish_owed(e))) return rc;
  if (part != GPH_PART_MIX && (rc = mix_finish_owed(e))) return rc;
  return finish_sync(e);
}

int gph_engine_unit(gph_engine *e, int32_t op, int32_t arg, double *out, int32_t stride)
{
  if (!e || !e->initialized || !out || op < 0 || op > 8 || stride < 3 * (e->cfg.n - 1) || stride < 4) return GPH_EARG;
  if ((op == 3 && stride < 1 + 5 * (2 * e->cfg.n - 1)) || (op == 6 && stride < 13)) return GPH_EARG;
  if ((op == 3 || op == 6) && (arg < 0 || arg >= 2 * e->cfg.n - 1)) return GPH_EARG;
  if (op == 8 && (arg < 0 || arg > 100000)) return GPH_EARG;
  SETDEV(e);
  { int rcs = flush_sync(e, true); if (!rcs) rcs = finish_sync(e); if (rcs) return rcs; }
  if (op == 2) {
    if (arg < e->cfg.Kc || arg >= e->cfg.K) return GPH_EARG;
    GphGlobal &G = *e->G_h;
    const GphModel &M = G.model;
    GphTauArgs &A = G.tau;
    memset(&A, 0, sizeof A);
    const int ap = arg, s0 = M.popSon0[ap], s1 = M.popSon1[ap], isRoot = ap == e->cfg.rootPop;
    const double tauold = M.popAge[ap];
    double taub0 = gg_max2(M.popAge[s0], M.popAge[s1]);
    taub0 = gg_max2(taub0, M.sampleAge[s0]);
    taub0 = gg_max2(taub0, M.sampleAge[s1]);
    const double taub1 = isRoot ? GG_OLDAGE : M.popAge[M.popFather[ap]];
    const double taunew = taub0 + 0.55 * (gg_min2(taub1, tauold * 1.4) - taub0);
    A.ap = ap; A.son0 = s0; A.son1 = s1; A.isRoot = isRoot;
    A.tauold = tauold; A.taunew = taunew; A.taub0 = taub0; A.taub1 = taub1;
    A.taufactor0 = (taunew - taub0) / (tauold - taub0);
    A.taufactor1 = isRoot ? A.taufactor0 : (taunew - taub1) / (tauold - taub1);
    e->G_dirty = true;
  }
  { int rcp = push_if_dirty(e); if (rcp) return rcp; }
  double *d_out = nullptr;
  const size_t bytes = sizeof(double) * (size_t)stride * e->L;
  if (dev_alloc((void **)&d_out, bytes)) return GPH_EHIP;
  int rc = acc_zero(e, d_out, bytes);
  if (!rc) rc = launch_loci(e, 12, k_unit, op, arg, d_out, stride);
  if (!rc) rc = reduce_local(e, 0, GPH_OUT_SLOTS);
  if (!rc) rc = run_stage_now(e, GS_COUNT_ONLY, 12);
  if (!rc) rc = d2h(e, out, d_out, bytes);
  dev_free(d_out);
  return rc;
}

int gph_engine_last_error(gph_engine *e, int64_t *locus, int32_t *code)
{
  if (!e) return GPH_EARG;
  if (locus) *locus = e->last_error_locus;
  if (code) *code = e->last_error_code;
  return 0;
}

int gph_engine_debug_break_chain(gph_engine *e, int64_t global_locus, int32_t pop)
{
  if (!e || !e->initialized || pop < 0 || pop >= e->cfg.K) return GPH_EARG;
  SETDEV(e);
  { int rcs = flush_sync(e, true); if (!rcs) rcs = finish_sync(e); if (rcs) return rcs; }
  const long long lo = global_locus - e->cfg.locus_begin;
  if (lo < 0 || lo >= e->L) return GPH_EARG;
  int64_t slot = -1;
  for (int64_t j = 0; j < e->L; j++) if (e->h_orig[j] == lo) { slot = j; break; }
  if (slot < 0) return GPH_ESTATE;
  const GphLayout &y = e->lay;
  std::vector<char> pg(y.page_bytes);
  char *dp = (char *)e->dev.pages + (size_t)slot * y.page_bytes;
  int rc = d2h(e, pg.data(), dp, y.page_bytes);
  if (rc) return rc;
  const int16_t *first = (const int16_t *)(pg.data() + y.o_first);
  GphEv *evr = (GphEv *)(pg.data() + y.o_ev);
  if (first[pop] < 0) return GPH_ESTATE;
  evr[first[pop]].next = -1;
  return h2d(e, dp, pg.data(), y.page_bytes);
}

int gph_engine_debug_oob(gph_engine *e, int32_t *where, int32_t *checked)
{
  if (!e || !where || !checked) return GPH_EARG;
  *where = 0;
#ifndef GPH_BOUNDS
  *checked = 0;
  return 0;
#else
  *checked = 1;
  SETDEV(e);
  if (e->initialized) { int rcs = flush_sync(e, true); if (!rcs) rcs = finish_sync(e); if (rcs) return rcs; }
  return oob_take(where);
#endif
}

#if defined(GPH_HOSTEMU) && defined(GPH_EMU64)
int gph_debug_emu64_stats(long long *waves, long long *rendezvous)
{
  if (waves) *waves = gph_emu::tw.waves_total;
  if (rendezvous) *rendezvous = gph_emu::tw.rendezvous_total;
  return gph_emu::g_enabled;
}
#endif

int gph_engine_dump_loci(gph_engine *e, const char *path, int32_t withCond, int32_t append)
{
  if (!e || !e->initialized || !path) return GPH_ESTATE;
  SETDEV(e);
  { int rcs = flush_sync(e, true); if (!rcs) rcs = finish_sync(e); if (rcs) return rcs; }
  const GphLayout &y = e->lay;
  std::vector<char> pages(e->pages_bytes), cond(withCond ? e->cond_bytes : 0);
  int rc = d2h(e, pages.data(), e->dev.pages, e->pages_bytes);
  if (!rc && withCond) rc = d2h(e, cond.data(), e->dev.cond, e->cond_bytes);
  if (rc) return rc;
  FILE *f = fopen(path, append ? "a" : "w");
  if (!f) return GPH_EARG;
  std::vector<int32_t> slot_of(e->L);
  for (int64_t j = 0; j < e->L; j++) slot_of[e->h_orig[j]] = (int32_t)j;
  const int dstride = getenv("GPH_DUMP_STRIDE") && atoi(getenv("GPH_DUMP_STRIDE")) > 0 ? atoi(getenv("GPH_DUMP_STRIDE")) : 1;
  for (int64_t go = 0; go < e->L; go++) {
    if ((go + e->cfg.locus_begin) % dstride != 0) continue;
    const int64_t g = slot_of[go];
    dump_one_locus(e, f, go + e->cfg.locus_begin, pages.data() + (size_t)g * y.page_bytes, withCond ? cond.data() + e->h_cond_off[g] : nullptr, e->h_P[g]);
  }
  fclose(f);
  return 0;
}

enum { SETTLE_PAGES, SETTLE_PAGES_AND_AGES, SETTLE_CHAIN };
static int sample_settle(gph_engine *e, int level)
{
  if (level == SETTLE_CHAIN) { int rcp = push_if_dirty(e); if (rcp) return rcp; }
  if (level != SETTLE_PAGES) { int rcw = finish_owed(e); if (rcw) return rcw; }
  if (e->mix_owed && e->mirror_current && !e->G_h->mix_flag) e->mix_owed = false;
  return mix_finish_owed(e);
}

static int sample_begin(gph_engine *e, int cls, int &tms)
{
  tms = -1;
  { int rcf = flush_pending(e); if (rcf) return rcf; }
  tms = tm_begin(e, cls);
  return 0;
}
static void sample_end(gph_engine *e, int cls, int k, int tms)
{
  tm_end(e, tms);
  flat_launched(e, cls, k);
  e->cls_launches[cls] += 1;
}

static void rows_free(gph_engine *e, SmRows &b) { eng_free(e, b.d); b = SmRows{}; }
static int rows_alloc(SmRows &b, size_t esz, int32_t n, int32_t cap)
{
  if (dev_alloc((void **)&b.d, esz * (size_t)n * cap)) { b.d = nullptr; return GPH_EHIP; }
  b.esz = esz; b.n = n; b.cap = cap; b.fill = 0;
  return 0;
}
static void *rows_next(const SmRows &b) { return b.d + b.esz * (size_t)b.n * b.fill; }
static int rows_fetch(gph_engine *e, SmRows &b, void *out, int32_t *rows)
{
  *rows = b.fill;
  if (b.fill > 0) { int rc = d2h(e, out, b.d, b.esz * (size_t)b.n * b.fill); if (rc) return rc; }
  b.fill = 0;
  return 0;
}

static void parts_free(gph_engine *e, SmParts &p) { eng_free(e, p.d_part); p.d_part = nullptr; p.rd = p.chunk = p.nchunks = 0; }
static int parts_alloc(gph_engine *e, SmParts &p, int32_t rd, int32_t default_chunk)
{
// ... 464 lines not shown
```

g-phocs_amd/csrc/gph_kernels.h:

```cpp
#pragma once
#include "gph_rt.h"

struct GphDev {
  char *pages;
  char *shadow;
  char *cond;
  const uint64_t *cond_off;
  const char *seq;
  const uint64_t *seq_off;
  const int32_t *P;
  const int32_t *orig;
  double *out;
  double *stats;
  int32_t L;
  int32_t Ltot;
  int64_t locus_begin;
  int32_t *err;
  const int32_t *slog_map;
  double *slog;
  int32_t *slog_n;
  int32_t slog_cap, pad_;
};

#include "gph_locus.h"


#undef GPH_FILE_ID
#define GPH_FILE_ID 2
GPH_DEV void copy16_g2l(int lds_off, const char *src, int bytes) { gph_copy16_in(GPH_SMB + lds_off, src, bytes >> 4); }
GPH_DEV void page_in(const char *page) { gph_copy16_in(GPH_LDSP(&gph_lds), page, g_lay.page_bytes >> 4); }
GPH_DEV void page_out(char *page) { gph_copy16_out(page, GPH_LDSP(&gph_lds), g_lay.page_bytes >> 4); }

GPH_DEV void scratch_init(const GphDev &D, int g, int P, uint64_t cond_off)
{
  int k;
  for (k = 0; k < CN_COUNT; k++) setCNT(k, 0);
  setCNT(CN_P, P);
  setCNT(CN_QPH, GPH_Q_PHASES(P, g_lay.n)); setCNT(CN_QCNT, GPH_Q_COUNT(P, g_lay.n)); setCNT(CN_QTERMS, GPH_Q_TERMS(P, g_lay.n, g_lay.cnt16));
  setCNT(CN_SUMLDS, g_lay.lds_sum && GPH_Q_TERMS(P, g_lay.n, g_lay.cnt16) + 8 * ((P + 7) & ~7) <= g_lay.dyn_bytes);
  if (P > g_lay.huge_P) {
    const uint64_t a_ = (uint64_t)(uintptr_t)(D.seq + D.seq_off[g]);
    setCNT(CN_HUGE, 1); setCNT(CN_SEQLO, (int)(uint32_t)a_); setCNT(CN_SEQHI, (int)(uint32_t)(a_ >> 32));
  }
  sf64(&GphLds::s_cntf, 0, 0.0);
#if defined(GPH_STAMPS) || defined(GPH_HOSTEMU)
  for (k = 0; k < 8; k++) gph_lds.s_stamp[k] = 0.0;
#endif
  set_cond_base(D.cond + cond_off);
  delta_clear(0);
  delta_clear(1);
}

GPH_DEV void stage_in_copy(const GphDev &D, int g, const char *pages, int withSeq, int &P_, uint64_t &co_)
{
  constexpr int PCH = (int)((offsetof(GphLds, s_dcoal) + 1023) / 1024);
  constexpr int SCH = 2;
  uint64_t o0 = 0, o1 = 0;
  if (withSeq) { o0 = D.seq_off[g]; o1 = D.seq_off[g + 1]; }
  P_ = D.P[2 * g];
  co_ = D.cond_off[g];
  gph_copy16_in2<PCH, SCH>(GPH_LDSP(&gph_lds), pages + (size_t)g * g_lay.page_bytes, g_lay.page_bytes >> 4, GPH_SMB, D.seq + o0,
                           P_ > g_lay.huge_P ? 0 : (int)(o1 - o0) >> 4);
  GPH_SYNC();
}
GPH_DEV void stage_in(const GphDev &D, int g, const char *pages, int withSeq)
{
  int P_; uint64_t co_;
  stage_in_copy(D, g, pages, withSeq, P_, co_);
  load_scalars();
  scratch_init(D, g, P_, co_);
}
GPH_DEV void stage_out_evaluated(const GphDev &D, int g)
{
  flush_scalars();
  GPH_SYNC();
  char *sh = D.shadow + (size_t)g * g_lay.page_bytes;
  if (ISC(IS_RB_NUM) != 0) { page_out(sh); return; }
  gph_copy16_out(sh + g_lay.o_nd, GPH_LDSP(&gph_lds.nd), g_lay.N);
  gph_copy16_out(sh + g_lay.o_mig_age, GPH_LDSP(&gph_lds.mig_age), (g_lay.page_bytes - g_lay.o_mig_age) >> 4);
}
GPH_DEV void stage_in_evaluated(const GphDev &D, int g, int withSeq)
{
  int P_; uint64_t co_;
  stage_in_copy(D, g, D.pages, withSeq, P_, co_);
  const char *sh = D.shadow + (size_t)g * g_lay.page_bytes;
  const int32_t *is = (const int32_t *)(sh + g_lay.o_iscal);
  if (RFL(is[IS_RB_NUM]) != 0) {
    page_in(sh);
  } else {
    gph_copy16_in(GPH_LDSP(&gph_lds.nd), sh + g_lay.o_nd, g_lay.N);
    gph_copy16_in(GPH_LDSP(&gph_lds.mig_age), sh + g_lay.o_mig_age, (g_lay.page_bytes - g_lay.o_mig_age) >> 4);
  }
  GPH_SYNC();
  load_scalars();
  scratch_init(D, g, P_, co_);
}
GPH_DEV void stage_out(const GphDev &D, int g, char *pages, int unused)
{
  (void)unused;
  flush_scalars();
  GPH_SYNC();
  page_out(pages + (size_t)g * g_lay.page_bytes);
  if (pages == D.pages) {
    const int K = g_lay.K, B = g_lay.B, C = 2 * K + 2 * B;
    for (int c = GPH_LANE; c < C; c += GPH_NLANES) {
      double v;
      if (c < K) v = gph_lds.coal[c];
      else if (c < 2 * K) v = (double)gph_lds.ncoal[c - K];
      else if (c < 2 * K + B) v = gph_lds.migst[c - 2 * K];
      else v = (double)gph_lds.nmig[c - 2 * K - B];
      D.stats[(size_t)g * C + c] = v;
    }
  }
}
GPH_DEV double eval_bytes(int U)
{
  const int P = CNT(CN_P), full = CNT(CN_EVALS) - CNT(CN_EMPTY);
  if (P <= 0 || full <= 0) return 0.0;
  return (double)(96ll * (CNT(CN_NODES) - CNT(CN_NODES0)) * P + (long long)(20 * g_lay.N + 8 * U + 8) * full);
}
GPH_DEV void out_common(const GphDev &D, int g)
{
  const double bytes_ = eval_bytes(D.P[2 * g + 1]);
  if (GPH_LANE == 0) {
    double *o = D.out + (size_t)g * GPH_OUT_SLOTS;
    o[8] = CNT(CN_EVALS);
    o[9] = CNT(CN_NODES);
    o[10] = bytes_;
    o[11] = gph_errcode() != 0 ? (double)((((long long)1 << 30) - (long long)(D.orig[g] + D.locus_begin)) * 16384 + (gph_errcode() & 16383)) : 0.0;
    o[13] = CNT(CN_NOTENOUGH);
    if (gph_errcode() != 0) {
      gph_raise(D.err, gph_errcode());
    }
  }
}
#define OUT(g, k, v) do { if (GPH_LANE == 0) D.out[(size_t)(g) * GPH_OUT_SLOTS + (k)] = (v); } while (0)

GPH_DEV void random_gtree(GphRng &rng)
{
  const int n = g_lay.n;
  int pi, pop, nextId = n, num, node1, node2, choice, a, b, base, cur = 0;
  double t, T;
  for (pi = 0; pi < g_lay.K; pi++) {
    pop = g_model.postOrder[pi];
    if (pop < g_lay.Kc) {
      node1 = pop > 0 ? g_model.cumSamples[pop - 1] : 0;
      num = g_model.cumSamples[pop] - node1;
      base = cur;
      for (node2 = 0; node2 < num; ++node2) {
        si16(&GphLds::s_targets, base + node2, node1 + node2);
        setNPOP(node1 + node2, pop);
        setNEV(node1 + node2, -1);
        setLEFT(node1 + node2, -1);
        setRGHT(node1 + node2, -1);
        setFATH(node1 + node2, -1);
        setAGE(node1 + node2, g_model.sampleAge[pop]);
      }
    } else {
      base = gi16(&GphLds::s_dpops, 0, g_model.popSon0[pop]);
      num = cur - base;
    }
    si16(&GphLds::s_dpops, 0, pop, base);
    T = g_model.popAge[pop];
    if (pop < g_lay.Kc) T = g_model.sampleAge[pop];
    for (; num > 1; num--, nextId++) {
      t = -(g_model.theta[pop] / (num * (num - 1.))) * gph_log_u(l_rndu(rng));
      T += t;
      if (pop != g_lay.rootPop && T > g_model.popAge[g_model.popFather[pop]]) break;
      choice = (int)(num * l_rndu(rng));
      a = gi16(&GphLds::s_targets, base + choice);
      si16(&GphLds::s_targets, base + choice, gi16(&GphLds::s_targets, base + num - 1));
      choice = (int)((num - 1) * l_rndu(rng));
      b = gi16(&GphLds::s_targets, base + choice);
      si16(&GphLds::s_targets, base + choice, nextId);
// ... 79 lines not shown
    lnacc = dgen + lnLd;
    if (gph_failed()) break;
    const bool take_ = UNI(lnacc >= 0) || UNI(l_rndu(rng) < gph_exp_u(lnacc));
    GPH_SLOG(3, take_, lnacc, 0, 0, 0, 0);
    if (take_) {
      acc++;
      setFS(FS_GENLNL, FS(FS_GENLNL) + dgen);
      sf64(&GphLds::s_cntf, 2, gf64(&GphLds::s_cntf, 2) + lnLd);
      sf64(&GphLds::s_cntf, 3, gf64(&GphLds::s_cntf, 3) + (dgen + lnLd) / D.Ltot);
      accept_event_chain_changes(0);
      lik_reset_saved();
    } else {
      reject_event_chain_changes(0);
      lik_revert();
    }
  }
  OUT(g, 0, acc);
  OUT(g, 3, gf64(&GphLds::s_cntf, 2));
  OUT(g, 4, gf64(&GphLds::s_cntf, 3));
}

template <class RNG> GPH_DEV void sweep_mignodes(const GphDev &D, int g, double finetune, RNG &rng)
{
  int mi, mignode, pop_s, pop_t, ev_s, ev_t, below, mig_below, mig_above, father, acc = 0, totmigs = 0;
  double t, tnew, tb0, tb1, dgen, lnacc, dLog = 0;
  for (mi = 0; mi < ISC(IS_NUM_MIGS); mi++) {
    mignode = LIVING(mi);
    t = MAGE(mignode);
    pop_s = MG(mignode, MG_SPOP);
    pop_t = MG(mignode, MG_TPOP);
    ev_s = MG(mignode, MG_SEV);
    ev_t = MG(mignode, MG_TEV);
    below = MG(mignode, MG_BRANCH);
    tb0 = g_model.bandStart[MG(mignode, MG_BAND)];
    tb1 = g_model.bandEnd[MG(mignode, MG_BAND)];
    mig_below = find_last_mig(below, t);
    mig_above = find_first_mig(below, t);
    if (mig_below >= 0) tb0 = gmax2(tb0, MAGE(mig_below));
    else tb0 = gmax2(tb0, AGE(below));
    if (mig_above >= 0) tb1 = gmin2(tb1, MAGE(mig_above));
    else {
      father = FATH(below);
      if (father < 0) tb1 = gmin2(tb1, GPH_OLDAGE);
      else tb1 = gmin2(tb1, AGE(father));
    }
    tnew = t + finetune * l_rnd2normal8(rng);
    tnew = l_reflect(tnew, tb0, tb1);
    if (UNI(fabs(tnew - t) < 1e-15)) { acc++; continue; }
    GPH_SLOG(4, mignode, t, tnew, 0, 0, 0);
    dgen = consider_event_move(0, ev_s, pop_s, t, pop_s, tnew);
    dgen += consider_event_move(1, ev_t, pop_t, t, pop_t, tnew);
    lnacc = dgen;
    if (gph_failed()) break;
    const bool take_ = UNI(lnacc >= 0) || UNI(l_rndu(rng) < gph_exp_u(lnacc));
    GPH_SLOG(3, take_, lnacc, 0, 0, 0, 0);
    if (take_) {
      acc++;
      setFS(FS_GENLNL, FS(FS_GENLNL) + dgen);
      dLog += dgen / D.Ltot;
      accept_event_chain_changes(0);
      accept_event_chain_changes(1);
      setMAGE(mignode, tnew);
    } else {
      reject_event_chain_changes(0);
      reject_event_chain_changes(1);
    }
  }
  for (mi = 0; mi < g_lay.B; mi++) totmigs += NMIGB(mi);
  OUT(g, 1, acc);
  OUT(g, 5, dLog);
  OUT(g, 12, totmigs);
}

template <class RNG> GPH_DEV void sweep_spr(const GphDev &D, int g, RNG &rng)
{
  int node, res, father, father_pop_old, sibling, b, i, mig, ev, target, pop, acc = 0, fpn, fen;
  double lnLd, lnacc, t_new;
  sf64(&GphLds::s_cntf, 5, 0.0);
  sf64(&GphLds::s_cntf, 6, 0.0);
  for (node = 0; node < g_lay.N; node++) {
    if (node == ISC(IS_ROOT)) continue;
    father = FATH(node);
    { const GphNodeS F_ = ld_node(father);
      father_pop_old = F_.npop;
      sibling = F_.left + F_.right - node; }
    GPH_SLOG(5, node, father, father_pop_old, 0, 0, 0);
#if GPH_BIG_BANDS || defined(GPH_TWO_WALKS)
    { STAMPA_BEGIN(3); trace_lineage<0>(node, rng); STAMPA_END(3); }
    { STAMPA_BEGIN(4); res = trace_lineage<1>(node, rng); STAMPA_END(4); }
#else
    { STAMPA_BEGIN(3); res = trace_pair(node, rng); STAMPA_END(3); }
#endif
#ifdef GPH_WALKSTAT
    { extern long long gph_ws[4]; int n0 = DI(0, DI_NEV), n1 = DI(1, DI_NEV), c = 0;
      while (c < n0 && c < n1 && gph_lds.s_dev[0][c] == gph_lds.s_dev[1][c]) c++;
      gph_ws[0] += n0; gph_ws[1] += n1; gph_ws[2] += c; gph_ws[3] += 1; }
#endif
    lnLd = -FS(FS_DATALNL);
    { STAMP_BEGIN(1); lnLd += lik_compute(1); STAMP_END(1); }
    lnacc = lnLd;
    if (gph_failed()) break;
    const bool take_ = res >= 0 && (UNI(lnacc >= 0) || UNI(l_rndu(rng) < gph_exp_u(lnacc)));
    GPH_SLOG(3, take_, lnacc, 0, 0, 0, 0);
    if (take_) {
      STAMPC_BEGIN(2);
      acc++;
      setFS(FS_GENLNL, FS(FS_GENLNL) + (SPRLN(1) - SPRLN(0)));
      sf64(&GphLds::s_cntf, 5, gf64(&GphLds::s_cntf, 5) + lnLd);
      sf64(&GphLds::s_cntf, 6, gf64(&GphLds::s_cntf, 6) + (lnLd - SPRLN(0) + SPRLN(1)) / D.Ltot);
      target = SPRI(SI_TARGET);
      t_new = AGE(father);
      for (i = 0; i < ISC(IS_NUM_MIGS); i++) {
        mig = LIVING(i);
        if (MG(mig, MG_BRANCH) == father) setMG(mig, MG_BRANCH, sibling);
        if (target == father) target = sibling;
        if (MG(mig, MG_BRANCH) == target && MAGE(mig) >= t_new) setMG(mig, MG_BRANCH, father);
      }
      remove_event(SPRI(SI_FEV_OLD), father_pop_old);
      fen = SPRI(SI_FEV_NEW);
      setETYPE(fen, GPH_COAL);
      setENODE(fen, father);
      setNEV(father, fen);
      fpn = SPRI(SI_FPOP_NEW);
      if (fpn != father_pop_old) {
        setNPOP(father, fpn);
        setNCOAL(father_pop_old, NCOAL(father_pop_old) - 1);
        setNCOAL(fpn, NCOAL(fpn) + 1);
      }
      replace_mig_nodes(node);
      (void)ev; (void)b; (void)pop;
      GPH_EACH(k, DI(1, DI_NEV)) { const int q = gph_lds.s_dev[1][k]; gph_lds.ev[q].nlin = (uint8_t)(gph_lds.ev[q].nlin + 1); }
      GPH_EACH1(k, g_lay.B) gph_lds.migst[k] = gph_lds.migst[k] + (gph_lds.s_dmig[1][k] - gph_lds.s_dmig[0][k]);
      GPH_EACH1(k, g_lay.K) gph_lds.coal[k] = gph_lds.coal[k] + (gph_lds.s_dcoal[1][k] - gph_lds.s_dcoal[0][k]);
      lik_reset_saved();
      STAMPC_END(2);
    } else {
      STAMPC_BEGIN(3);
      if (res >= 0) remove_event(SPRI(SI_FEV_NEW), SPRI(SI_FPOP_NEW));
      for (i = 0; i < SPRI(SI_NNEW); i++) {
        b = SPRA(SA_NEWBAND, i);
        remove_event(SPRA(SA_NEWIN, i), g_model.bandTgt[b]);
        remove_event(SPRA(SA_NEWOUT, i), g_model.bandSrc[b]);
      }
      GPH_EACH(k, DI(0, DI_NEV)) { const int q = gph_lds.s_dev[0][k]; gph_lds.ev[q].nlin = (uint8_t)(gph_lds.ev[q].nlin + 1); }
      lik_revert();
      STAMPC_END(3);
    }
  }
  OUT(g, 2, acc);
  OUT(g, 6, gf64(&GphLds::s_cntf, 5));
  OUT(g, 7, gf64(&GphLds::s_cntf, 6));
}

GPH_DEV void kb_sweep(const GphDev &D, int g, int flags, double ftCoal, double ftMig, double mix_c, double mix_lnc)
{
  STAMP_BEGIN(0);
  if (flags & 16) {
    stage_in_evaluated(D, g, 1);
    mix_commit_body(mix_c, mix_lnc);
  } else {
    stage_in(D, g, D.pages, 1);
  }
  GPH_SLOG_OPEN(D, g);
  GphRngB rng;
  rng_load(rng);
  OUT(g, 15, (flags & 8) ? (double)synchronize_events() : 1.0);
  OUT(g, 0, 0.0); OUT(g, 1, 0.0); OUT(g, 2, 0.0); OUT(g, 3, 0.0); OUT(g, 4, 0.0);
  OUT(g, 5, 0.0); OUT(g, 6, 0.0); OUT(g, 7, 0.0); OUT(g, 12, 0.0);
  { STAMP_BEGIN(5); if ((flags & 1) && ftCoal > 0.0) sweep_internal(D, g, ftCoal, rng); STAMP_END(5); }
  { STAMPC_BEGIN(4); if ((flags & 2) && ftMig > 0.0 && !gph_failed()) sweep_mignodes(D, g, ftMig, rng); STAMPC_END(4); }
  { STAMP_BEGIN(6); if ((flags & 4) && !gph_failed()) sweep_spr(D, g, rng); STAMP_END(6); }
  rng_store(rng);
  out_common(D, g);
  STAMP_END(0);
#if defined(GPH_STAMPS) && !defined(GPH_HOSTEMU)
  for (int k = 0; k < 8; k++) OUT(g, k, gph_lds.s_stamp[k]);
#endif
  stage_out(D, g, D.pages, 1);
}

GPH_DEV void kb_tau_eval(const GphDev &D, int g, gph_ctau &A, int fuse)
{
  const int ap = A.ap, s0 = A.son0, s1 = A.son1;
  double age_mt, new_age = 0.0, dGen = 0, dData = 0, gd;
  int srcP, tgtP, fatherNode, inode, inORout = -1, ev = -1, n1_0 = 0, n1_1 = 0, i, mig, mig1, band, pop;
  int conflict = 0, k;
  stage_in_after_finish(D, g, fuse);
  setISC(IS_CONFLICT_LOG, 1);
  setISC(IS_RB_NUM, 0);
  for (i = 0; i < ISC(IS_NUM_MIGS); i++) {
    if (conflict == 0) {
      pop = -1;
      mig = LIVING(i);
      band = MG(mig, MG_BAND);
      srcP = MG(mig, MG_SPOP);
      tgtP = MG(mig, MG_TPOP);
      age_mt = MAGE(mig);
      if (age_mt < A.taub0 || age_mt > A.taub1) continue;
      if (A.mode) {
        const int up = age_mt > A.tauold;
        const double tb = up ? A.taub1 : A.taub0, tf = up ? A.taufactor1 : A.taufactor0;
        if (srcP == ap) {
          inORout = 1;
          ev = MG(mig, MG_TEV);
          pop = tgtP;
          new_age = tb + tf * (age_mt - tb);
          if (up) n1_1++; else n1_0++;
        } else if (tgtP == ap) {
          inORout = 0;
          ev = MG(mig, MG_SEV);
          pop = srcP;
          new_age = tb + tf * (age_mt - tb);
          if (up) n1_1++; else n1_0++;
        }
      } else
      if ((srcP == s0 && tgtP == s1) || (srcP == s1 && tgtP == s0)) {
        n1_0++;
      } else if (srcP == ap) {
        inORout = 1;
        ev = MG(mig, MG_TEV);
        pop = tgtP;
        new_age = A.taub1 + A.taufactor1 * (age_mt - A.taub1);
        n1_1++;
      } else if (tgtP == ap) {
        inORout = 0;
        ev = MG(mig, MG_SEV);
        pop = srcP;
        new_age = A.taub1 + A.taufactor1 * (age_mt - A.taub1);
        n1_1++;
      } else if ((srcP == s0 || srcP == s1) && MAGE(mig) > A.taub0) {
        inORout = 1;
        ev = MG(mig, MG_TEV);
        pop = tgtP;
        new_age = A.taub0 + A.taufactor0 * (age_mt - A.taub0);
        n1_0++;
      } else if ((tgtP == s0 || tgtP == s1) && MAGE(mig) > A.taub0) {
        inORout = 0;
        ev = MG(mig, MG_SEV);
        pop = srcP;
        new_age = A.taub0 + A.taufactor0 * (age_mt - A.taub0);
        n1_0++;
      }
      if (ev >= 0) {
        inode = MG(mig, MG_BRANCH);
        if (new_age >= g_model.bandEnd[band]) conflict = 1;
        else if (new_age <= g_model.bandStart[band]) conflict = 1;
        else if (inORout == 0 && new_age > age_mt) {
          fatherNode = FATH(inode);
          mig1 = find_first_mig(inode, MAGE(mig));
          if (mig1 >= 0 && MG(mig1, MG_SPOP) != ap && MG(mig1, MG_SPOP) != s0 && MG(mig1, MG_SPOP) != s1 &&
              new_age >= MAGE(mig1))
            conflict = 1;
          else if (fatherNode >= 0 && new_age >= AGE(fatherNode))
            conflict = 1;
        } else if (inORout == 1 && new_age < age_mt) {
          mig1 = find_last_mig(inode, MAGE(mig));
          if (mig1 >= 0 && MG(mig1, MG_TPOP) != ap && MG(mig1, MG_TPOP) != s0 && MG(mig1, MG_TPOP) != s1 &&
              new_age <= MAGE(mig1))
            conflict = 1;
          else if (new_age <= AGE(inode))
            conflict = 1;
        }
        if (conflict != 1) {
          k = ISC(IS_RB_NUM);
          setRBI(0, k, ev);
          setRBI(2, k, pop);
          setRBAGE(k, new_age);
          setISC(IS_RB_NUM, k + 1);
          ev = -1;
        }
      }
    }
  }
  if (conflict) {
    setISC(IS_RB_NUM, 0);
  } else {
    for (i = 0; i < A.num_aff; i++) {
      int guard = 0;
      band = A.aff_bands[i];
      tgtP = g_model.bandTgt[band];
      for (ev = FIRSTEV(tgtP); ev >= 0;) {
        const GphEvS R = ld_ev(ev);
        if (R.node == band &&
            ((R.type == GPH_MIG_BAND_START && A.start_or_end[i]) || R.type == GPH_MIG_BAND_END))
          break;
        if (++guard > GPH_CAP_E) { ev = -1; break; }
        ev = R.next;
      }
      if (ev < 0) { gph_fail(74); break; }
      k = ISC(IS_RB_NUM);
      setRBI(0, k, ev);
      setRBI(2, k, tgtP);
      setRBAGE(k, A.new_band_ages[i]);
      setISC(IS_RB_NUM, k + 1);
    }
    if (!gph_failed()) {
      gd = rubber_band_ripple(1);
      if (A.mode) {
        gd += rubber_band(ap, g_model.popAge[ap], A.taub1, A.tauold, A.taufactor1, 0, &n1_1);
        gd += rubber_band(ap, g_model.popAge[ap], A.taub0, A.tauold, A.taufactor0, 0, &n1_0);
      } else {
        if (A.isRoot) gd += rubber_band(ap, g_model.popAge[ap], A.taub0, A.tauold, A.taufactor1, 0, &n1_1);
        else gd += rubber_band(ap, g_model.popAge[ap], A.taub1, A.tauold, A.taufactor1, 0, &n1_1);
        gd += rubber_band(s0, g_model.popAge[s0], A.taub0, A.tauold, A.taufactor0, 0, &n1_0);
        gd += rubber_band(s1, g_model.popAge[s1], A.taub0, A.tauold, A.taufactor0, 0, &n1_0);
      }
      setFS(FS_GENDELTA, gd);
      dGen += gd;
      if (A.mode || n1_0 + n1_1) {
        dData -= FS(FS_DATALNL);
        dData += lik_compute(1, true);
      }
    }
  }
  OUT(g, 0, conflict ? 0 : n1_0);
  OUT(g, 1, conflict ? 0 : n1_1);
  OUT(g, 2, conflict);
  OUT(g, 14, conflict ? (double)(D.orig[g] + D.locus_begin) : 1e300);
  OUT(g, 3, dGen);
  OUT(g, 4, dData);
  out_common(D, g);
  stage_out_evaluated(D, g);
}

GPH_DEV void tau_commit_body(gph_cfin &F)
{
  int dummy = 0, i, mig, nw, ev;
  double age;
  setFS(FS_GENLNL, FS(FS_GENLNL) + FS(FS_GENDELTA));
  if (F.mode) {
    rubber_band(F.ap, F.age_ap, F.taub1, F.tauold, F.taufactor1, 1, &dummy);
// ... 672 lines not shown
```

g-phocs_amd/csrc/gph_locus.h:

```cpp
#pragma once
#include "gph_rt.h"

template <bool GPH_GM> struct GphCtxT {
#ifndef GPH_HOSTEMU
  GPH_DEV gph_cmodel &gmodel() const
  {
#if GPH_BIG_BANDS
    return *(gph_cmodel *)&(((gph_ckargs *)__builtin_amdgcn_kernarg_segment_ptr())->G->model);
#else
    if constexpr (GPH_GM) return *(gph_cmodel *)&(((gph_ckargs *)__builtin_amdgcn_kernarg_segment_ptr())->G->model);
    else return ((gph_ckargs *)__builtin_amdgcn_kernarg_segment_ptr())->model;
#endif
  }
#endif
  GphPad<IS_COUNT + CN_COUNT + SI_COUNT> r_pad;
#ifdef GPH_LOGSTEPS
  double *slog_ = nullptr;
  int32_t *slog_n_ = nullptr;
  int32_t slog_cap_ = 0;
  long long slog_gen_ = 0;
#define GPH_SLOG_OPEN(D, g) do { slog_ = nullptr; if ((D).slog_map && (D).slog_map[g] >= 0) { const int si_ = (D).slog_map[g]; \
      slog_ = (D).slog + (size_t)si_ * (D).slog_cap * 8; slog_n_ = (D).slog_n + si_; slog_cap_ = (D).slog_cap; } } while (0)
#define GPH_SLOG(kind, a, b, c, d, e, f) do { if (slog_ && GPH_LANE == 0) { const int k_ = (*slog_n_)++; if (k_ < slog_cap_) { double *r_ = slog_ + (size_t)k_ * 8; \
      r_[0] = (kind); r_[1] = (double)(a); r_[2] = (double)(b); r_[3] = (double)(c); r_[4] = (double)(d); r_[5] = (double)(e); r_[6] = (double)(f); r_[7] = 0.0; } } } while (0)
// ... 99 lines not shown
#define DI(inst, k) RFL(gph_lds.s_di[inst][k])
#define setDI(inst, k, v) (gph_lds.s_di[inst][k] = (v))
#define SPRI(k) GPH_PADGET(IS_COUNT + CN_COUNT + (k))
#define setSPRI(k, v) GPH_PADSET(IS_COUNT + CN_COUNT + (k), (v))
#define SPRA(k, i) gi16(&GphLds::s_spri16, (k) * GPH_MAX_MIGS + GPH_IX((i), GPH_MAX_MIGS))
#define setSPRA(k, i, v) si16(&GphLds::s_spri16, (k) * GPH_MAX_MIGS + GPH_IX((i), GPH_MAX_MIGS), (v))
#define SPRAGE(i) gf64(&GphLds::s_sprf, GPH_IX((i), GPH_MAX_MIGS + 2))
#define setSPRAGE(i, v) sf64(&GphLds::s_sprf, GPH_IX((i), GPH_MAX_MIGS + 2), (v))
#define SPRLN(r) gf64(&GphLds::s_sprf, GPH_MAX_MIGS + (r))
#define setSPRLN(r, v) sf64(&GphLds::s_sprf, GPH_MAX_MIGS + (r), (v))
#define CNT(k) GPH_PADGET(IS_COUNT + (k))
#define setCNT(k, v) GPH_PADSET(IS_COUNT + (k), (v))

struct LiveList {
  uint64_t bits;
  int n;
};
#if GPH_BIG_BANDS
GPH_DEV int ll_get(const LiveList &l, int i) { (void)l; return gu8(&GphLds::s_live, i); }
GPH_DEV void ll_set(LiveList &l, int i, int v) { (void)l; su8(&GphLds::s_live, i, v); }
GPH_DEV void ll_push(LiveList &l, int v) { ll_set(l, l.n, v); l.n++; }
GPH_DEV int ll_find(const LiveList &l, int v)
{
  for (int i = 0; i < l.n; i++) if (ll_get(l, i) == v) return i;
  return l.n;
}
#else
GPH_DEV int ll_get(const LiveList &l, int i) { return (int)((l.bits >> (4 * i)) & 15); }
GPH_DEV void ll_set(LiveList &l, int i, int v) { l.bits = (l.bits & ~((uint64_t)15 << (4 * i))) | ((uint64_t)v << (4 * i)); }
GPH_DEV void ll_push(LiveList &l, int v) { ll_set(l, l.n, v); l.n++; }
GPH_DEV int ll_find(const LiveList &l, int v)
{
  const uint64_t x = l.bits ^ (0x1111111111111111ull * (uint64_t)v);
  uint64_t t = (x - 0x1111111111111111ull) & ~x & 0x8888888888888888ull;
  if (l.n < 16) t &= (((uint64_t)1 << (4 * l.n)) - 1);
  return t ? (int)(__builtin_ctzll(t) >> 2) : l.n;
}
#endif
GPH_DEV void ll_swap_remove(LiveList &l, int i) { l.n--; ll_set(l, i, ll_get(l, l.n)); }

struct GphNodeS { double age; int father, left, right, npop; };
GPH_DEVHOT GphNodeS ld_node(int node)
{
  GphNodeS r;
  const gph_w4 w = gph_ld16(&gph_lds.nd[GPH_IX(node, GPH_CAP_N)]);
  union { double d; uint32_t u[2]; } t;
  t.u[0] = w.x; t.u[1] = w.y;
  const int w2 = RFL((int)w.z), w3 = RFL((int)w.w);
  r.age = t.d;
  r.father = (int)(int16_t)w2;
  r.left = w2 >> 16;
  r.right = (int)(int16_t)w3;
  r.npop = w3 >> 16;
  return r;
}
struct GphEvS { double time; int next, prev, node, nlin, type; };
GPH_DEVHOT GphEvS ld_ev(int ev)
{
  GphEvS r;
  const gph_w4 w = gph_ld16(&gph_lds.ev[GPH_IX(ev, GPH_CAP_E)]);
  union { double d; uint32_t u[2]; } t;
  t.u[0] = w.x; t.u[1] = w.y;
  const int w2 = RFL((int)w.z), w3 = RFL((int)w.w);
  r.time = t.d;
  r.next = (int)(int16_t)w2;
  r.prev = w2 >> 16;
  r.node = (int)(int16_t)w3;
  r.nlin = (int)(uint8_t)(w3 >> 16);
  r.type = (int)((uint32_t)w3 >> 24);
  return r;
}

#define gmin2(a, b) ((a) < (b) ? (a) : (b))
#define gmax2(a, b) ((a) > (b) ? (a) : (b))

#if defined(GPH_STAMPS) && !defined(GPH_HOSTEMU)
#define STAMP_BEGIN(k) long long stamp_t0_##k = __builtin_readcyclecounter()
#define STAMP_END(k) gph_lds.s_stamp[k] += (double)(__builtin_readcyclecounter() - stamp_t0_##k)
#else
#define STAMP_BEGIN(k) ((void)0)
#define STAMP_END(k) ((void)0)
#endif
#if defined(GPH_STAMPS) && GPH_STAMPS == 2 && !defined(GPH_HOSTEMU)
#define STAMPA_BEGIN(k) ((void)0)
#define STAMPA_END(k) ((void)0)
#define STAMPB_BEGIN(k) STAMP_BEGIN(k)
#define STAMPB_END(k) STAMP_END(k)
#define STAMPC_BEGIN(k) ((void)0)
#define STAMPC_END(k) ((void)0)
#elif defined(GPH_STAMPS) && GPH_STAMPS == 3 && !defined(GPH_HOSTEMU)
#define STAMPA_BEGIN(k) ((void)0)
#define STAMPA_END(k) ((void)0)
#define STAMPB_BEGIN(k) ((void)0)
#define STAMPB_END(k) ((void)0)
#define STAMPC_BEGIN(k) STAMP_BEGIN(k)
#define STAMPC_END(k) STAMP_END(k)
#else
#define STAMPA_BEGIN(k) STAMP_BEGIN(k)
#define STAMPA_END(k) STAMP_END(k)
#define STAMPB_BEGIN(k) ((void)0)
#define STAMPB_END(k) ((void)0)
#define STAMPC_BEGIN(k) ((void)0)
#define STAMPC_END(k) ((void)0)
#endif
GPH_DEV void gph_fail(int code) { if (CNT(CN_ERROR) == 0) setCNT(CN_ERROR, code); }
GPH_DEV int gph_failed() { return CNT(CN_ERROR) != 0; }
GPH_DEV int gph_errcode() { return CNT(CN_ERROR); }

#define pad64(k) ((uint64_t)(uint32_t)ISC(k) | ((uint64_t)(uint32_t)ISC((k) + 1) << 32))
#define setpad64(k, v) do { const uint64_t pv64_ = (v); setISC((k), (int)(uint32_t)pv64_); setISC((k) + 1, (int)(uint32_t)(pv64_ >> 32)); } while (0)
#if GPH_BIG_TREE
template <int K, int Q> GPH_DEV void ns_get_words_(gph_nset &r) { if constexpr (Q < GPH_NSQ) { r.w[Q] = pad64(K + 2 * Q); ns_get_words_<K, Q + 1>(r); } }
template <int K> GPH_DEV gph_nset ns_get_() { gph_nset r; ns_get_words_<K, 0>(r); return r; }
template <int K, int Q> GPH_DEV void ns_put_words_(const gph_nset &v) { if constexpr (Q < GPH_NSQ) { setpad64(K + 2 * Q, v.w[Q]); ns_put_words_<K, Q + 1>(v); } }
template <int K> GPH_DEV void ns_put_(const gph_nset &v) { ns_put_words_<K, 0>(v); }
#endif
GPH_DEV void load_scalars() { r_pad.load(gph_lds.iscal, IS_COUNT); }
GPH_DEV void flush_scalars() { r_pad.store(gph_lds.iscal, IS_COUNT); }

GPH_DEV double gph_div_theta(double a, int pop) { return gph_quot(a, g_model.theta[pop], g_model.thetaInv[pop]); }
GPH_DEV double gph_div_by(double a, double b, double y) { return gph_quot(a, b, y); }
GPH_DEV double gph_div3(double a) { return gph_quot(a, 3.0, 1.0 / 3.0); }

struct GphRng { uint32_t x, y, z; };
GPH_DEV void rng_load(GphRng &g) { g.x = (uint32_t)ISC(IS_RX); g.y = (uint32_t)ISC(IS_RY); g.z = (uint32_t)ISC(IS_RZ); }
GPH_DEV void rng_store(const GphRng &g) { setISC(IS_RX, (int)g.x); setISC(IS_RY, (int)g.y); setISC(IS_RZ, (int)g.z); }
GPH_DEV double l_rndu(GphRng &g)
{
  uint32_t x = g.x, y = g.y, z = g.z;
  double r;
  x = 171u * x - 30269u * (x / 177u);
  y = 172u * y - 30307u * (y / 176u);
  z = 170u * z - 30323u * (z / 178u);
  g.x = x;
  g.y = y;
  g.z = z;
#if defined(GPH_HOSTEMU) || !defined(__HIP_DEVICE_COMPILE__)
  r = x / 30269.0 + y / 30307.0 + z / 30323.0;
#else
  {
    const gph_cdbl *RC = GPH_RNGC;
    const double rx = RC[0], ry = RC[1], rz = RC[2], mx = RC[3], my = RC[4], mz = RC[5];
    double xd = (double)x, yd = (double)y, zd = (double)z, q;
    q = xd * rx; double qx = __builtin_fma(__builtin_fma(-q, mx, xd), rx, q);
    q = yd * ry; double qy = __builtin_fma(__builtin_fma(-q, my, yd), ry, q);
    q = zd * rz; double qz = __builtin_fma(__builtin_fma(-q, mz, zd), rz, q);
    r = qx + qy + qz;
  }
  return __builtin_amdgcn_fract(r);
#endif
  r = (r - (int)r);
  return r;
}
#ifdef GPH_HOSTEMU
typedef GphRng GphRngB;
#else
#ifndef GPH_RNG_BATCH
#define GPH_RNG_BATCH 16
#endif
struct GphRngB {
  int pos;
  double u;
};
GPH_DEV void rng_load(GphRngB &g)
{
  setCNT(CN_RX, ISC(IS_RX)); setCNT(CN_RY, ISC(IS_RY)); setCNT(CN_RZ, ISC(IS_RZ));
  g.pos = GPH_RNG_BATCH; g.u = 0.0;
}
GPH_DEV void rng_store(const GphRngB &g)
{
  uint32_t x = (uint32_t)CNT(CN_RX), y = (uint32_t)CNT(CN_RY), z = (uint32_t)CNT(CN_RZ);
  if (g.pos < GPH_RNG_BATCH) {
    x = (uint32_t)ISC(IS_RX); y = (uint32_t)ISC(IS_RY); z = (uint32_t)ISC(IS_RZ);
    for (int k = 0; k < g.pos; k++) {
      x = 171u * x - 30269u * (x / 177u);
      y = 172u * y - 30307u * (y / 176u);
      z = 170u * z - 30323u * (z / 178u);
    }
  }
  setISC(IS_RX, (int)x); setISC(IS_RY, (int)y); setISC(IS_RZ, (int)z);
}
#ifndef GPH_RNG_ROLLED
template <int K> GPH_DEV void rng_steps_(uint32_t &x, uint32_t &y, uint32_t &z, int &vx, int &vy, int &vz)
{
  if constexpr (K < GPH_RNG_BATCH) {
    x = 171u * x - 30269u * (x / 177u);
    y = 172u * y - 30307u * (y / 176u);
    z = 170u * z - 30323u * (z / 178u);
    asm("v_writelane_b32 %0, %3, %6\n\tv_writelane_b32 %1, %4, %6\n\tv_writelane_b32 %2, %5, %6"
        : "+v"(vx), "+v"(vy), "+v"(vz) : "s"(x), "s"(y), "s"(z), "i"(K));
    rng_steps_<K + 1>(x, y, z, vx, vy, vz);
  }
}
#endif
#ifndef GPH_RNG_VECTOR_REFILL
GPH_DEV void rng_refill(GphRngB &g)
{
  uint32_t x = (uint32_t)CNT(CN_RX), y = (uint32_t)CNT(CN_RY), z = (uint32_t)CNT(CN_RZ);
  int vx = 0, vy = 0, vz = 0;
  setISC(IS_RX, (int)x); setISC(IS_RY, (int)y); setISC(IS_RZ, (int)z);
#ifndef GPH_RNG_ROLLED
  rng_steps_<0>(x, y, z, vx, vy, vz);
#else
#pragma unroll 4
  for (int k = 0; k < GPH_RNG_BATCH; k++) {
    x = 171u * x - 30269u * (x / 177u);
    y = 172u * y - 30307u * (y / 176u);
    z = 170u * z - 30323u * (z / 178u);
    asm("s_mov_b32 m0, %6\n\ts_nop 0\n\tv_writelane_b32 %0, %3, m0\n\tv_writelane_b32 %1, %4, m0\n\tv_writelane_b32 %2, %5, m0"
        : "+v"(vx), "+v"(vy), "+v"(vz) : "s"(x), "s"(y), "s"(z), "s"(k) : "m0");
  }
#endif
  setCNT(CN_RX, (int)x); setCNT(CN_RY, (int)y); setCNT(CN_RZ, (int)z);
#if defined(__HIP_DEVICE_COMPILE__)
  {
    const gph_cdbl *RC = GPH_RNGC;
    const double rx = RC[0], ry = RC[1], rz = RC[2], mx = RC[3], my = RC[4], mz = RC[5];
    double xd = (double)(uint32_t)vx, yd = (double)(uint32_t)vy, zd = (double)(uint32_t)vz, q;
    q = xd * rx; double qx = __builtin_fma(__builtin_fma(-q, mx, xd), rx, q);
    q = yd * ry; double qy = __builtin_fma(__builtin_fma(-q, my, yd), ry, q);
    q = zd * rz; double qz = __builtin_fma(__builtin_fma(-q, mz, zd), rz, q);
    g.u = __builtin_amdgcn_fract(qx + qy + qz);
  }
#endif
  g.pos = 0;
}
#else
#define GPH_RNGV_STEP \
  "v_mul_hi_u32 %[q], %[st], %[mg]\n\t" \
  "v_mul_lo_u32 %[t], %[st], %[a]\n\t" \
  "v_sub_u32 %[st], %[st], %[q]\n\t" \
  "v_lshrrev_b32 %[st], 1, %[st]\n\t" \
  "v_add_u32 %[st], %[st], %[q]\n\t" \
  "v_lshrrev_b32 %[st], 7, %[st]\n\t" \
  "v_mul_lo_u32 %[st], %[st], %[nm]\n\t" \
  "v_add_u32 %[st], %[st], %[t]\n\t" \
  "v_cndmask_b32_dpp %[h], %[h], %[st], vcc row_shl:1 row_mask:0xf bank_mask:0xf bound_ctrl:0\n\t"
#define GPH_RNGV_STEP4 GPH_RNGV_STEP GPH_RNGV_STEP GPH_RNGV_STEP GPH_RNGV_STEP
GPH_DEV void rng_refill(GphRngB &g)
{
  static_assert(GPH_RNG_BATCH == 16, "one draw per lane of a 16-lane row");
  const uint32_t x0 = (uint32_t)CNT(CN_RX), y0 = (uint32_t)CNT(CN_RY), z0 = (uint32_t)CNT(CN_RZ);
  setISC(IS_RX, (int)x0); setISC(IS_RY, (int)y0); setISC(IS_RZ, (int)z0);
#if defined(__HIP_DEVICE_COMPILE__)
  const int row = GPH_LANE >> 4;
  const bool r0 = row == 0, r1 = row == 1;
  uint32_t st = r0 ? x0 : r1 ? y0 : z0, h = 0, q, t;
  const uint32_t mg = r0 ? 0x724287f5u : r1 ? 0x745d1746u : 0x702e05c1u;
  const uint32_t a = r0 ? 171u : r1 ? 172u : 170u;
  const uint32_t nm = r0 ? 0u - 30269u : r1 ? 0u - 30307u : 0u - 30323u;
  asm("s_mov_b32 vcc_lo, 0x80008000\n\t"
      "s_mov_b32 vcc_hi, 0x80008000\n\t"
      GPH_RNGV_STEP4 GPH_RNGV_STEP4 GPH_RNGV_STEP4 GPH_RNGV_STEP4
      : [st] "+v"(st), [h] "+v"(h), [q] "=&v"(q), [t] "=&v"(t) : [mg] "v"(mg), [a] "v"(a), [nm] "v"(nm) : "vcc");
  setCNT(CN_RX, __builtin_amdgcn_readlane((int)st, 0)); setCNT(CN_RY, __builtin_amdgcn_readlane((int)st, 16));
  setCNT(CN_RZ, __builtin_amdgcn_readlane((int)st, 32));
  {
    const gph_cdbl *RC = GPH_RNGC;
    const double rr = r0 ? RC[0] : r1 ? RC[1] : RC[2], mm = r0 ? RC[3] : r1 ? RC[4] : RC[5];
    const double hd = (double)h, q0 = hd * rr;
    const double qq = __builtin_fma(__builtin_fma(-q0, mm, hd), rr, q0);
    union { double d; int32_t i[2]; } u, vy, vz;
    u.d = qq;
    const int ay = (GPH_LANE + 16) << 2, az = (GPH_LANE + 32) << 2;
    vy.i[0] = __builtin_amdgcn_ds_bpermute(ay, u.i[0]); vy.i[1] = __builtin_amdgcn_ds_bpermute(ay, u.i[1]);
    vz.i[0] = __builtin_amdgcn_ds_bpermute(az, u.i[0]); vz.i[1] = __builtin_amdgcn_ds_bpermute(az, u.i[1]);
    g.u = __builtin_amdgcn_fract(qq + vy.d + vz.d);
  }
#endif
  g.pos = 0;
}
#endif
GPH_DEV double l_rndu(GphRngB &g)
{
  if (g.pos >= GPH_RNG_BATCH) rng_refill(g);
  const double u = gph_readlane64(g.u, g.pos);
  g.pos++;
  return u;
}
#endif
template <class RNG> GPH_DEV double l_rndnormal(RNG &g)
{
  double u, v, s;
  int guard = 0;
  for (;;) {
    if (++guard > 100000) { gph_fail(89); return 0.0; }
    u = 2 * l_rndu(g) - 1;
    v = 2 * l_rndu(g) - 1;
    s = u * u + v * v;
    if (UNI(s > 0 && s < 1)) break;
  }
  s = sqrt(-2. * gph_log_u(s) / s);
  return u * s;
}
template <class RNG> GPH_DEV double l_rnd2normal8(RNG &g)
{
  const double m2s2 = 8.;
  double m2N = sqrt(m2s2 / (m2s2 + 1.));
  double s2N = sqrt(1. / (m2s2 + 1.));
  double z = m2N + l_rndnormal(g) * s2N;
  z = UNI(l_rndu(g) < 0.5) ? z : -z;
  return z;
}
GPH_DEV double l_reflect(double x, double a, double b)
{
  const double slack = 0.000000001;
  double xnew, di;
  a += slack;
  b -= slack;
  if (UNI(b <= a)) return (a + b) / 2.;
  if (UNI(x < b && x > a)) return x;
  xnew = x;
  if (UNI(xnew <= a)) xnew = 2. * a - xnew;
  di = 2. * (b - a);
  xnew = xnew - di * floor((xnew - a) / di);
  if (UNI(xnew >= b)) xnew = 2. * b - xnew;
  int guard = 0;
  while (UNI(xnew <= a || xnew >= b)) {
    if (UNI(xnew >= b)) xnew = 2. * b - xnew;
    else xnew = 2 * a - xnew;
    if (++guard > 64) { gph_fail(90); return (a + b) / 2.; }
  }
  return xnew;
}

GPH_DEV int lik_mark_cond(int node)
{
  const gph_nset d = NS_GET(IS_DIRTY0);
  if (CNT(CN_P) <= 0 || ns_has(d, node)) return 1;
  NS_PUT(IS_DIRTY0, ns_with(d, node));
  NS_PUT(IS_CBIT0, ns_flip(NS_GET(IS_CBIT0), node));
  return 0;
}
GPH_DEV void lik_save_node(int node, int recalc)
{
  if (recalc) lik_mark_cond(node);
  NS_PUT(IS_SAVED0, ns_with(NS_GET(IS_SAVED0), node));
  gph_lds.sv[node] = gph_lds.nd[node];
}
GPH_DEV void lik_adjust_age(int node, double age)
{
  lik_save_node(node, 1);
  setAGE(node, age);
}
GPH_DEV void lik_reset_saved()
{
  NS_PUT(IS_SAVED0, ns_none());
  NS_PUT(IS_DIRTY0, ns_none());
  setISC(IS_SV_ROOT, -1);
  setFS(FS_SV_DATALNL, FS(FS_DATALNL));
}
GPH_DEV void lik_revert()
{
  setFS(FS_DATALNL, FS(FS_SV_DATALNL));
  if (ISC(IS_SV_ROOT) >= 0) { setISC(IS_ROOT, ISC(IS_SV_ROOT)); setISC(IS_SV_ROOT, -1); }
  const gph_nset sv_ = NS_GET(IS_SAVED0);
  if (ns_any(sv_)) {
#if GPH_BIG_TREE
    GPH_EACH(k, g_lay.N)
#else
    GPH_EACH1(k, g_lay.N)
#endif
    {
      if (ns_has(sv_, k)) {
        GphNode r = gph_lds.sv[k];
        r.npop = gph_lds.nd[k].npop;
        gph_lds.nd[k] = r;
      }
    }
  }
  NS_PUT(IS_CBIT0, ns_xor(NS_GET(IS_CBIT0), NS_GET(IS_DIRTY0)));
  NS_PUT(IS_DIRTY0, ns_none());
  NS_PUT(IS_SAVED0, ns_none());
}

GPH_DEV double edge_prob(double len)
{
  if (len < 1e-100) return 0.0;
  return ((1 - gph_exp_u(-4 * len / 3.0)) / 4.0);
}

GPH_DEV double edge_prob_v(double len)
{
  if (len < 1e-100) return 0.0;
  return ((1 - gph_exp(gph_div3(-4 * len))) / 4.0);
}

GPH_DEV gdbl *cond_base()
{
  uint64_t lo = (uint32_t)RFL(gph_lds.s_condptr[0]), hi = (uint32_t)RFL(gph_lds.s_condptr[1]);
  return (gdbl *)(uintptr_t)(lo | (hi << 32));
}
GPH_DEV GphSeq seq_ref()
{
  GphSeq S; S.g = nullptr;
  if (CNT(CN_HUGE)) {
    const uint64_t lo = (uint32_t)CNT(CN_SEQLO), hi = (uint32_t)CNT(CN_SEQHI);
    S.g = (GPH_GLB char *)(uintptr_t)(lo | (hi << 32));
  }
  return S;
}
GPH_DEV void set_cond_base(const void *p)
{
  uint64_t v = (uint64_t)(uintptr_t)p;
  gph_lds.s_condptr[0] = (uint32_t)v;
  gph_lds.s_condptr[1] = (uint32_t)(v >> 32);
}
GPH_DEV int cond_off(int node, int bit)
{
  int P = CNT(CN_P);
  return ((bit * (g_lay.n - 1) + (node - g_lay.n)) * P) * 4;
}

template <class CP>
GPH_DEV double child_factor(int child, CP cnd, int p, int a, double pe, double qe, int q_leaf = GPH_Q_LEAF, const GphSeq SQ = GphSeq{nullptr})
{
  double s0, s1, s2, s3, sa, S, Sp;
  if (child < g_lay.n) {
    int code = GPH_LEAFCODE_S(SQ, q_leaf, p, child);
    s0 = (code == 4 || code == 0) ? 1.0 : 0.0;
    s1 = (code == 4 || code == 1) ? 1.0 : 0.0;
    s2 = (code == 4 || code == 2) ? 1.0 : 0.0;
    s3 = (code == 4 || code == 3) ? 1.0 : 0.0;
  } else {
    s0 = cnd[4 * p + 0];
    s1 = cnd[4 * p + 1];
    s2 = cnd[4 * p + 2];
    s3 = cnd[4 * p + 3];
  }
  sa = a == 0 ? s0 : a == 1 ? s1 : a == 2 ? s2 : s3;
  S = 0.0;
  S += s0;
  S += s1;
// ... 1937 lines not shown
```

g-phocs_amd/csrc/gph_types.h:

```cpp
#pragma once
#include <stdint.h>

#ifndef GPH_CAP_LEAVES
#define GPH_CAP_LEAVES 24
#endif
#ifndef GPH_CAP_K
#define GPH_CAP_K 16
#endif
#ifndef GPH_CAP_B
#define GPH_CAP_B 8
#endif
#if GPH_CAP_K > 32
#define GPH_MAXK 40
typedef uint64_t gph_popmask;
#else
#define GPH_MAXK 32
typedef uint32_t gph_popmask;
#endif
#if GPH_CAP_B > 16
#define GPH_MAXB 100
#define GPH_BIG_BANDS 1
#else
#define GPH_MAXB 16
#define GPH_BIG_BANDS 0
#endif
#define GPH_BANDW ((GPH_MAXB + 31) / 32)
#ifndef GPH_MAX_MIGS
#define GPH_MAX_MIGS 10
#endif
#if GPH_CAP_LEAVES > 32
#define GPH_BIG_TREE 1
#define GPH_NSQ ((2 * GPH_CAP_LEAVES - 1 + 63) / 64)
#else
#define GPH_BIG_TREE 0
#define GPH_NSQ 1
#endif
#define GPH_NSW (2 * GPH_NSQ)
#define GPH_OLDAGE 999.0
#define GPH_WAVE 64
#define FS_COUNT_ 5
#define IS_COUNT_ (10 + 3 * GPH_NSW)

enum { GPH_COAL = 0, GPH_IN_MIG, GPH_OUT_MIG, GPH_MIG_BAND_START, GPH_MIG_BAND_END,
       GPH_SAMPLES_START, GPH_END_CHAIN, GPH_DUMMY };

struct GphModel {
  double theta[GPH_MAXK], popAge[GPH_MAXK], sampleAge[GPH_MAXK];
  double thetaInv[GPH_MAXK];
  double logTwoTheta[GPH_MAXK], logMigRate[GPH_MAXB];
  double migRate[GPH_MAXB], bandStart[GPH_MAXB], bandEnd[GPH_MAXB];
  gph_popmask isAnc[GPH_MAXK];
  uint32_t bandsOver[GPH_MAXK][GPH_BANDW];
  uint32_t bandsInto[GPH_MAXK][GPH_BANDW];
  int32_t popFather[GPH_MAXK], popSon0[GPH_MAXK], popSon1[GPH_MAXK], samplesPerPop[GPH_MAXK];
  int32_t bandSrc[GPH_MAXB], bandTgt[GPH_MAXB];
  int32_t postOrder[GPH_MAXK];
  int32_t cumSamples[GPH_MAXK];
};

struct GphLayout {
  int32_t n, N, K, Kc, B, E, RB, rootPop;
  int32_t o_ev;
  int32_t o_nd, o_sv;
  int32_t o_mig_age, o_coal, o_migst, o_rb_age, o_fscal;
  int32_t o_nev;
  int32_t o_first;
  int32_t o_mig_i, o_living, o_ncoal, o_nmig, o_rb_i;
  int32_t o_iscal;
  int32_t page_bytes;
  int32_t Pmax;
  int32_t lds_bytes;
  int32_t lds_sum;
  int32_t cnt16;
  int32_t dyn_bytes;
  int32_t huge_P;
};
struct GphGlobal;
struct GphKargs {
#if !GPH_BIG_BANDS
  GphModel model;
#endif
  GphLayout lay;
  double mathc[32];
  const double *log_t;
  const uint64_t *exp_t;
  GphGlobal *G;
};

#define GPH_PHASES(w) ((int)(w) < 0x8000 ? (int)(w) : (1 << ((int)(w) & 31)))
#define GPH_PHASES_ENCODE_MIN 0x8000
#define GPH_Q_LEAF 0
#define GPH_Q_NH(n) (((n) + 1) >> 1)
#define GPH_Q_PHASES(P, n) (((P) * GPH_Q_NH(n) + 1) & ~1)
#define GPH_Q_COUNT(P, n) ((GPH_Q_PHASES(P, n) + 2 * (P) + 3) & ~3)
#define GPH_Q_BYTES(P, n, c16) ((GPH_Q_COUNT(P, n) + ((c16) ? 2 : 4) * (P) + 15) & ~15)
#define GPH_Q_TERMS(P, n, c16) GPH_Q_BYTES(P, n, c16)
enum { DI_ORIG = 0, DI_UPD, DI_DLIN, DI_NEV, DI_NPOPS, DI_NBANDS, DI_SRCPOP, DI_TGTPOP, DI_COUNT };
enum { SI_FEV_OLD = 0, SI_FEV_NEW, SI_FPOP_NEW, SI_TARGET, SI_NOLD, SI_NNEW, SI_COUNT };
enum { SA_OLD = 0, SA_NEWIN, SA_NEWOUT, SA_NEWBAND };
enum { CN_EVALS = 0, CN_NODES, CN_ERROR, CN_P, CN_NOTENOUGH, CN_RX, CN_RY, CN_RZ, CN_EMPTY, CN_NODES0, CN_QPH, CN_QCNT, CN_QTERMS, CN_SUMLDS, CN_HUGE, CN_SEQLO, CN_SEQHI, CN_COUNT };

enum { FS_DATALNL = 0, FS_SV_DATALNL, FS_GENLNL, FS_GENDELTA, FS_MUTRATE, FS_COUNT };
enum { IS_ROOT = 0, IS_SV_ROOT, IS_DIRTY0, IS_CBIT0 = IS_DIRTY0 + GPH_NSW, IS_SAVED0 = IS_CBIT0 + GPH_NSW,
       IS_FREE = IS_SAVED0 + GPH_NSW, IS_NUM_MIGS, IS_RB_NUM, IS_CONFLICT_LOG, IS_RX, IS_RY, IS_RZ, IS_COUNT };
static_assert(IS_COUNT <= IS_COUNT_, "page scalars");
enum { MG_BRANCH = 0, MG_BAND, MG_SPOP, MG_TPOP, MG_SEV, MG_TEV, MG_COUNT };

#define GPH_OUT_SLOTS 16
enum { OUT_ACCEPT = 0, OUT_DDATA, OUT_DLOG, OUT_EVALS, OUT_EVALNODES, OUT_EVALBYTES,
       OUT_NTJ0, OUT_NTJ1, OUT_CONFLICT, OUT_ERROR, OUT_GENLNL, OUT_DATALNL, OUT_NMIGS };

#define GPH_CAP_N (2 * GPH_CAP_LEAVES - 1)
#define GPH_CAP_E (2 * GPH_CAP_LEAVES + 4 * GPH_MAX_MIGS + 3 * GPH_CAP_B + GPH_CAP_K + 10)
#define GPH_CAP_RB (GPH_MAX_MIGS + 2 * GPH_CAP_B)

struct alignas(16) GphEv {
  double time;
  int16_t next, prev;
  int16_t node;
  uint8_t nlin;
  uint8_t type;
};

struct alignas(16) GphNode {
  double age;
  int16_t father, left, right;
  int16_t npop;
};

#if GPH_CAP_E <= 255
typedef uint8_t gph_evid;
#else
typedef uint16_t gph_evid;
#endif
struct alignas(16) GphLds {
  GphEv ev[GPH_CAP_E];
  GphNode nd[GPH_CAP_N], sv[GPH_CAP_N];
  double mig_age[GPH_MAX_MIGS];
  double coal[GPH_CAP_K], migst[GPH_CAP_B], rb_age[GPH_CAP_RB], fscal[FS_COUNT_];
  int32_t iscal[IS_COUNT_];
  int16_t nev[GPH_CAP_N];
  int16_t first[GPH_CAP_K];
  int16_t mig_i[GPH_MAX_MIGS * 6], living[GPH_MAX_MIGS], ncoal[GPH_CAP_K], nmig[GPH_CAP_B], rb_i[3 * GPH_CAP_RB];
  double s_dcoal[2][GPH_CAP_K], s_dmig[2][GPH_CAP_B];
  double s_cntf[8];
  union {
    struct { double s_sprf[GPH_MAX_MIGS + 2]; int16_t s_spri16[4 * GPH_MAX_MIGS]; };
    struct { double s_chkcoal[GPH_CAP_K], s_chkmig[GPH_CAP_B]; int16_t s_chknc[GPH_CAP_K], s_chknm[GPH_CAP_B]; };
  };
#if defined(GPH_STAMPS) || defined(GPH_HOSTEMU)
  double s_stamp[8];
#endif
  int32_t s_di[2][8];
  uint32_t s_condptr[2];
  int16_t s_dpops[2][GPH_CAP_K], s_dbands[2][GPH_CAP_B];
  int16_t s_targets[GPH_CAP_N + 1];
#if GPH_BIG_TREE || defined(GPH_HOSTEMU)
  int16_t s_ord[GPH_CAP_N + 1], s_stack[GPH_CAP_N + 1];
#endif
  gph_evid s_dev[2][GPH_CAP_E];
#if GPH_BIG_BANDS
  uint8_t s_live[(GPH_CAP_B + 15) & ~15];
#endif
#if GPH_BIG_TREE
  double s_pe[GPH_CAP_N];
#endif
#ifdef GPH_PAD
  char s_pad[GPH_PAD];
#endif
};

static_assert(GPH_CAP_LEAVES <= 200 && GPH_CAP_K <= GPH_MAXK && GPH_CAP_B <= GPH_MAXB, "capacities beyond the reference's own caps (200 leaves, 39 populations, 100 bands: patch.h:17-22)");

struct GphTauArgs {
  int32_t ap, son0, son1, isRoot, num_aff, mode;
  double tauold, taunew, taub0, taub1, taufactor0, taufactor1;
  int32_t aff_bands[GPH_MAXB * 2];
  int32_t start_or_end[GPH_MAXB * 2];
  double new_band_ages[GPH_MAXB * 2];
};

struct GphTauFin {
  int32_t ap, son0, son1, isRoot, mode, flag;
  long long limit;
  double tauold, taunew, taub0, taub1, taufactor0, taufactor1;
  double age_ap, age_s0, age_s1;
};

#if GPH_BIG_BANDS
#define GPH_RED_COLS 384
#else
#define GPH_RED_COLS 128
#endif
#define GPH_RED_STRIDE (3 * GPH_RED_COLS + 8)
#define GPH_RED_ROW (2 * GPH_RED_STRIDE)
enum { GS_INIT_DONE = 0, GS_SWEEP_DONE, GS_TOTALS, GS_THETA, GS_TAU_PROPOSE, GS_TAU_DECIDE, GS_TAU_END, GS_SAGE_PROPOSE,
       GS_SAGE_DECIDE, GS_SAGE_END, GS_MIX_PROPOSE, GS_MIX_DECIDE, GS_STARTMIG, GS_REFRESH_DONE, GS_CHECK_DONE,
       GS_COUNT_ONLY,
       GS_THETA_ONLY, GS_MIGR_ONLY };
enum { GPH_PART_SWEEP = 0, GPH_PART_LRATE, GPH_PART_THETA, GPH_PART_MIGR, GPH_PART_TAU, GPH_PART_SAGE, GPH_PART_MIX,
       GPH_PART_SYNC, GPH_PART_REFRESH, GPH_PART_CHECK };
#define GPH_REC_MAX (16 + 3 * GPH_MAXK)
struct GphRec { int32_t code, idx; int64_t acc; double dataLnL, logL; };
enum { REC_INIT = 0, REC_INT, REC_MIGN, REC_SPR, REC_LRATE, REC_THETA, REC_MIGR, REC_TAU, REC_CONFLICTS, REC_SAGE,
       REC_MIX, REC_CHECK };
struct GphApply { int32_t kind, idx; double lnc, diff; };
struct alignas(16) GphGlobal {
  GphModel model;
  GphTauArgs tau;
  long long tau_limit;
  int32_t tau_flag, mix_flag;
  double mix_c, mix_lnc;
  int32_t napply, pad0;
  GphApply apply[GPH_MAXK + GPH_MAXB];
  int32_t n, K, Kc, B, rootPop, startMig, doMixing, samplesPerLog;
  double Ltot;
  double thetaAlpha[GPH_MAXK], thetaBeta[GPH_MAXK], thetaStart[GPH_MAXK];
  double ageAlpha[GPH_MAXK], ageBeta[GPH_MAXK], ageStart[GPH_MAXK], ftTaus[GPH_MAXK];
  double mrAlpha[GPH_MAXB], mrBeta[GPH_MAXB];
  int32_t updateSampleAge[GPH_MAXK];
  double ftCoalTime, ftMigTime, ftTheta, ftMigRate, ftMixing;
  uint32_t gx, gy, gz, pad1;
  double logLikelihood, dataLogLikelihood;
  double tot_coal[GPH_MAXK], tot_ncoal[GPH_MAXK], tot_mig[GPH_MAXB], tot_nmig[GPH_MAXB];
  int64_t acc[9], accTau[GPH_MAXK], rubberband_conflicts;
  int32_t iteration, error;
  long long error_locus;
  double pend_lnacc, pend_tauold, pend_taunew, pend_taufactor0, pend_taufactor1, pend_dGen;
  int32_t pend_pop, pend_kind;
  int32_t accArr[GPH_MAXK];
  double cls_evals[16], cls_nodes[16], cls_bytes[16], cnt_notenough;
  double migRateShown[GPH_MAXB];
  int32_t nrec, shownValid;
  GphRec rec[GPH_REC_MAX];
  GphTauFin fin;
};

struct GphBlk { int x, y, dim; char *lds; };
```

Before: 436.9 million.

## Pregenerate per-locus RNG draws ahead of the sweep on a side stream

Adds a k_rng_ahead kernel that precomputes each locus's Wichmann-Hill uniform draws into a device buffer, with periodic state checkpoints. The sweep kernel then loads draws from memory rather than generating them serially in-wave. In chained iterations the pregeneration for the next sweep is launched on a separate stream so it overlaps with the remaining stages. The cost is extra HBM per locus, extra launches and event synchronisation, and replaying RNG state from checkpoints at store time to stay bit-exact.

```diff
diff --git a/g-phocs_amd/csrc/gph_backend.h b/g-phocs_amd/csrc/gph_backend.h
--- a/g-phocs_amd/csrc/gph_backend.h
+++ b/g-phocs_amd/csrc/gph_backend.h
@@ -26,6 +26,10 @@
 static int flush_pending(gph_engine *) { return 0; }
 static int stage_defer(gph_engine *, int, int, int, bool &queued) { queued = false; return 0; }
 static void flat_launched(gph_engine *, int, int) {}
+static void dev_clear_error() {}
+static int rng_ahead_side(gph_engine *, GphGrid) { return 0; }
+static int rng_ahead_wait(gph_engine *) { return 0; }
+static void rng_ahead_drain(gph_engine *) {}
 
 static int reduce_local(gph_engine *e, int sec, int ncols)
 {
@@ -129,6 +133,8 @@
   hipStream_t stream_wide = nullptr;
   hipEvent_t ev_fork = nullptr, ev_join = nullptr;
   bool side_stream = true;
+  hipStream_t stream_ra = nullptr;
+  hipEvent_t ev_ra_go = nullptr, ev_ra_done = nullptr;
   struct Tm { hipEvent_t a, b; int which; };
   std::vector<Tm> tm;
   size_t tm_used = 0;
@@ -136,6 +142,7 @@
 
 static int dev_alloc(void **p, size_t bytes) { return hipMalloc(p, bytes ? bytes : 16) == hipSuccess ? 0 : GPH_EHIP; }
 static void dev_free(void *p) { if (p) (void)hipFree(p); }
+static void dev_clear_error() { (void)hipGetLastError(); }
 static int collect_times(gph_engine *e)
 {
   for (size_t i = 0; i < e->tm_used; i++) {
@@ -206,7 +213,6 @@
 }
 static void flat_launched(gph_engine *e, int cls, int k) { e->n_launches += k; if (cls >= 0) e->last_which = cls; }
 
-static void launch_pre(gph_engine *e) { GPH_KA_MODEL(e->ka, e); e->ka.lay = e->lay; e->ka.G = e->G_d; }
 template <class... P, class... A>
 static int launch_on(hipStream_t stream, GphGrid grid, int block, size_t lds_bytes, void (*kernel)(P...), A &&...args)
 {
@@ -214,6 +220,22 @@
   HIPCHK(hipGetLastError());
   return 0;
 }
+static void launch_pre(gph_engine *e) { GPH_KA_MODEL(e->ka, e); e->ka.lay = e->lay; e->ka.G = e->G_d; }
+static int rng_ahead_side(gph_engine *e, GphGrid grid)
+{
+  if (!e->stream_ra) {
+    if (hipStreamCreateWithFlags(&e->stream_ra, hipStreamNonBlocking) != hipSuccess ||
+        hipEventCreateWithFlags(&e->ev_ra_go, hipEventDisableTiming) != hipSuccess ||
+        hipEventCreateWithFlags(&e->ev_ra_done, hipEventDisableTiming) != hipSuccess) return GPH_EHIP;
+  }
+  HIPCHK(hipEventRecord(e->ev_ra_go, e->stream));
+  HIPCHK(hipStreamWaitEvent(e->stream_ra, e->ev_ra_go, 0));
+  { int rcl = launch_on(e->stream_ra, grid, GPH_WAVE, 0, k_rng_ahead, e->ka, e->dev); if (rcl) return rcl; }
+  HIPCHK(hipEventRecord(e->ev_ra_done, e->stream_ra));
+  return 0;
+}
+static int rng_ahead_wait(gph_engine *e) { HIPCHK(hipStreamWaitEvent(e->stream, e->ev_ra_done, 0)); return 0; }
+static void rng_ahead_drain(gph_engine *e) { if (e->stream_ra) (void)hipStreamSynchronize(e->stream_ra); }
 template <class... P, class... A>
 static int launch_grid(gph_engine *e, GphGrid grid, int block, size_t lds_bytes, void (*kernel)(P...), A &&...args)
 {
@@ -361,6 +383,9 @@
   if (e->h_red) (void)hipHostFree(e->h_red);
   if (e->G_h) (void)hipHostFree(e->G_h);
   for (auto &t : e->tm) { (void)hipEventDestroy(t.a); (void)hipEventDestroy(t.b); }
+  if (e->ev_ra_go) (void)hipEventDestroy(e->ev_ra_go);
+  if (e->ev_ra_done) (void)hipEventDestroy(e->ev_ra_done);
+  if (e->stream_ra) (void)hipStreamDestroy(e->stream_ra);
   if (e->ev_fork) (void)hipEventDestroy(e->ev_fork);
   if (e->ev_join) (void)hipEventDestroy(e->ev_join);
   if (e->stream_wide) (void)hipStreamDestroy(e->stream_wide);
diff --git a/g-phocs_amd/csrc/gph_engine.hip b/g-phocs_amd/csrc/gph_engine.hip
--- a/g-phocs_amd/csrc/gph_engine.hip
+++ b/g-phocs_amd/csrc/gph_engine.hip
@@ -316,7 +316,85 @@
 }
 #endif
 
-#define GPH_NCLS 18
+GPH_HD int rng_ahead_count(int kprev, int M)
+{
+  int n = (kprev + 64 + 63) & ~63;
+  return n < 0 ? 0 : n > M ? M : n;
+}
+#ifdef GPH_HOSTEMU
+static void k_rng_ahead(GphBlk b, GphKargs KA, GphDev D)
+{
+  const int cs = D.ra_cshift, nck = (D.ra_M >> cs) + 1;
+  for (int slot = b.x * b.dim; slot < (b.x + 1) * b.dim && slot < D.L; slot++) {
+    const int32_t *is = (const int32_t *)(D.pages + (size_t)slot * KA.lay.page_bytes + KA.lay.o_iscal);
+    uint32_t x = (uint32_t)is[IS_RX], y = (uint32_t)is[IS_RY], z = (uint32_t)is[IS_RZ];
+    const int n = rng_ahead_count(D.ra_kprev[slot], D.ra_M);
+    for (int d = 0; d <= n; d++) {
+      if ((d & ((1 << cs) - 1)) == 0) {
+        uint32_t *c = D.ra_ckpt + 4 * ((size_t)GPH_IX(d >> cs, nck) * D.L + slot);
+        c[0] = x; c[1] = y; c[2] = z; c[3] = 0;
+      }
+      if (d == n) break;
+      GPH_RNG_STEP(x, y, z);
+      const double r = x / 30269.0 + y / 30307.0 + z / 30323.0;
+      D.ra_draws[(size_t)slot * D.ra_M + GPH_IX(d, D.ra_M)] = r - (int)r;
+    }
+    uint32_t *t = D.ra_tail + 4 * (size_t)slot;
+    t[0] = x; t[1] = y; t[2] = z; t[3] = (uint32_t)n;
+  }
+}
+#else
+#define GPH_RA_TILE 16
+__global__ void __launch_bounds__(GPH_WAVE) k_rng_ahead(GphKargs KA, GphDev D)
+{
+  typedef uint32_t gu32x4 __attribute__((ext_vector_type(4)));
+  __shared__ double tile[GPH_WAVE][GPH_RA_TILE + 1];
+  __shared__ int n_of[GPH_WAVE];
+  const int lane = threadIdx.x, slot0 = blockIdx.x * GPH_WAVE, slot = slot0 + lane;
+  const bool live = slot < D.L;
+  const int cs = D.ra_cshift, nck = (D.ra_M >> cs) + 1;
+  const double rx = KA.mathc[26], ry = KA.mathc[27], rz = KA.mathc[28], mx = KA.mathc[29], my = KA.mathc[30], mz = KA.mathc[31];
+  uint32_t x = 0, y = 0, z = 0;
+  int n = 0;
+  gu32x4 *ckpt = (gu32x4 *)D.ra_ckpt;
+  if (live) {
+    const int32_t *is = (const int32_t *)(D.pages + (size_t)slot * KA.lay.page_bytes + KA.lay.o_iscal);
+    x = (uint32_t)is[IS_RX]; y = (uint32_t)is[IS_RY]; z = (uint32_t)is[IS_RZ];
+    n = rng_ahead_count(D.ra_kprev[slot], D.ra_M);
+    ckpt[slot] = gu32x4{x, y, z, 0u};
+  }
+  n_of[lane] = n;
+  int nmax = n;
+  for (int o = 32; o > 0; o >>= 1) { const int w = __shfl_xor(nmax, o, GPH_WAVE); nmax = w > nmax ? w : nmax; }
+  __syncthreads();
+  for (int d0 = 0; d0 < nmax; d0 += GPH_RA_TILE) {
+    if (d0 < n) {
+#pragma unroll
+      for (int t = 0; t < GPH_RA_TILE; t++) {
+        GPH_RNG_STEP(x, y, z);
+        const double xd = (double)x, yd = (double)y, zd = (double)z;
+        double q;
+        q = xd * rx; const double qx = __builtin_fma(__builtin_fma(-q, mx, xd), rx, q);
+        q = yd * ry; const double qy = __builtin_fma(__builtin_fma(-q, my, yd), ry, q);
+        q = zd * rz; const double qz = __builtin_fma(__builtin_fma(-q, mz, zd), rz, q);
+        tile[lane][t] = __builtin_amdgcn_fract(qx + qy + qz);
+      }
+      const int d1 = d0 + GPH_RA_TILE;
+      if ((d1 & ((1 << cs) - 1)) == 0) ckpt[(size_t)GPH_IX(d1 >> cs, nck) * D.L + slot] = gu32x4{x, y, z, 0u};
+    }
+    __syncthreads();
+#pragma unroll
+    for (int i = 0; i < GPH_WAVE / 4; i++) {
+      const int r = (lane >> 4) + 4 * i, c = lane & 15;
+      if (slot0 + r < D.L && d0 < n_of[r]) D.ra_draws[(size_t)(slot0 + r) * D.ra_M + GPH_IX(d0 + c, D.ra_M)] = tile[r][c];
+    }
+    __syncthreads();
+  }
+  if (live) ((gu32x4 *)D.ra_tail)[slot] = gu32x4{x, y, z, (uint32_t)n};
+}
+#endif
+
+#define GPH_NCLS 19
 struct SmRows {
   char *d = nullptr;
   size_t esz = 0;
@@ -379,6 +457,10 @@
   int32_t slog_sel = 0;
   bool mirror_current = true;
   bool no_fuse = false;
+  bool rng_ahead = true;
+  bool ra_place_b = true, ra_b_valid = false;
+  int32_t ra_M = 512, ra_C = 16, ra_first = 320;
+  size_t ra_bytes = 0;
   gph_counters counters = {0, 0, 0.0, 0};
   struct { double *d = nullptr; int32_t ncol = 0; int64_t samples = 0; std::vector<std::string> names; } ls;
   struct { SmParts part; SmRows rows; int32_t bd = 0; std::string name; } cs;
@@ -653,7 +735,32 @@
   return check_error(e);
 }
 
+static int rng_ahead_alloc(gph_engine *e)
+{
+  const size_t L = (size_t)e->L, nck = (size_t)(e->ra_M / e->ra_C) + 1;
+  const size_t b_draws = sizeof(double) * L * e->ra_M, b_ckpt = 16 * nck * L, b_tail = 16 * L, b_kprev = sizeof(int32_t) * L;
+  GphDev &d = e->dev;
+  const bool forced = getenv("GPH_RNG_AHEAD_FAIL_ALLOC") && atoi(getenv("GPH_RNG_AHEAD_FAIL_ALLOC")) != 0;
+  if (dev_alloc((void **)&d.ra_draws, b_draws) || dev_alloc((void **)&d.ra_ckpt, b_ckpt) || dev_alloc((void **)&d.ra_tail, b_tail) ||
+      forced || dev_alloc((void **)&d.ra_kprev, b_kprev)) {
+    dev_clear_error();
+    fprintf(stderr, "gphocs_hip: no memory for %d draws ahead of the sweep per locus (%.1f MB): the sweep kernel generates its own\n",
+            e->ra_M, (double)(b_draws + b_ckpt + b_tail + b_kprev) / 1e6);
+    eng_free(e, d.ra_draws); eng_free(e, d.ra_ckpt); eng_free(e, d.ra_tail); eng_free(e, d.ra_kprev);
+    d.ra_draws = nullptr; d.ra_ckpt = nullptr; d.ra_tail = nullptr; d.ra_kprev = nullptr;
+    e->rng_ahead = false;
+    return 0;
+  }
+  std::vector<int32_t> kp(L, ((e->ra_first + 63) & ~63) - 64);
+  if (h2d(e, d.ra_kprev, kp.data(), b_kprev)) return GPH_EHIP;
+  d.ra_M = e->ra_M;
+  d.ra_cshift = e->ra_C == 64 ? 6 : 4;
+  e->ra_bytes = b_draws + b_ckpt + b_tail + b_kprev;
+  return 0;
+}
+
 extern "C" {
+static void rng_ahead_dirty(gph_engine *e);
 
 int gph_engine_create(const gph_config *cfg, gph_engine **out)
 {
@@ -683,6 +790,16 @@
   fill_math_constants(e->ka);
   if (const char *fh = getenv("GPH_HOST_DECISIONS")) e->force_host = atoi(fh) != 0;
   if (const char *nf = getenv("GPH_NO_FUSE")) e->no_fuse = atoi(nf) != 0;
+  if (const char *ra = getenv("GPH_RNG_AHEAD")) e->rng_ahead = atoi(ra) != 0;
+  if (const char *ra = getenv("GPH_RNG_AHEAD_DRAWS")) e->ra_M = atoi(ra);
+  if (const char *ra = getenv("GPH_RNG_AHEAD_PLACE")) e->ra_place_b = ra[0] == 'B' || ra[0] == 'b';
+  if (const char *ra = getenv("GPH_RNG_AHEAD_CKPT")) e->ra_C = atoi(ra);
+  if (const char *ra = getenv("GPH_RNG_AHEAD_FIRST")) e->ra_first = atoi(ra);
+  if (e->rng_ahead && (e->ra_M < 64 || e->ra_M % 64 != 0 || e->ra_M > (1 << 20) || (e->ra_C != 16 && e->ra_C != 64) || e->ra_first < 0)) {
+    fprintf(stderr, "gphocs_hip: GPH_RNG_AHEAD_DRAWS must be a multiple of 64 (up to 2^20), GPH_RNG_AHEAD_CKPT 16 or 64, GPH_RNG_AHEAD_FIRST >= 0\n");
+    delete e;
+    return GPH_EARG;
+  }
   if (int rc = backend_open(e)) { gph_engine_destroy(e); return rc; }
   memset(e->G_h, 0, sizeof(GphGlobal));
   e->G_h->error_locus = -1;
@@ -694,10 +811,12 @@
 void gph_engine_destroy(gph_engine *e)
 {
   if (!e) return;
+  rng_ahead_drain(e);
   dev_free(e->dev.pages); dev_free(e->dev.shadow); dev_free(e->dev.cond); dev_free((void *)e->dev.cond_off);
   dev_free((void *)e->dev.seq); dev_free((void *)e->dev.seq_off); dev_free((void *)e->dev.orig); dev_free((void *)e->dev.P); dev_free(e->dev.out); dev_free(e->dev.stats); dev_free(e->d_mutRate);
   dev_free(e->d_lrec); dev_free(e->d_lpre); dev_free(e->d_slot_of); dev_free(e->d_lr_result); dev_free(e->d_lr_gscr); dev_free(e->d_ref_page); dev_free(e->d_ref_seq);
   dev_free(e->d_part); dev_free(e->dev.err);
+  dev_free(e->dev.ra_draws); dev_free(e->dev.ra_ckpt); dev_free(e->dev.ra_tail); dev_free(e->dev.ra_kprev);
   dev_free(e->ls.d); dev_free(e->cs.part.d_part); dev_free(e->cs.rows.d); dev_free(e->ts.part.d_part); dev_free(e->ts.rows.d);
   dev_free(e->an.d_acc); dev_free(e->an.rows.d);
   dev_free(e->gt.rows.d); dev_free(e->gt.d_sel);
@@ -885,6 +1004,7 @@
   if (mutRates) rc |= h2d(e, e->d_mutRate, rates.data(), sizeof(double) * L);
   if (rc) return GPH_EHIP;
   e->dev.L = (int32_t)L;
+  if (e->rng_ahead && rng_ahead_alloc(e)) return GPH_EHIP;
   e->dev.Ltot = (int32_t)e->cfg.L_total;
   e->dev.locus_begin = e->cfg.locus_begin;
   e->loaded = true;
@@ -915,6 +1035,7 @@
 {
   if (!e || !e->loaded || !e->seeded || !e->model_set) return GPH_ESTATE;
   SETDEV(e);
+  rng_ahead_dirty(e);
   { int rcf = flush_pending(e); if (rcf) return rcf; }
   e->mix_owed = e->fin_owed = e->sync_pending = false;
   if (e->G_h->mix_flag || e->G_h->tau_flag) { e->G_h->mix_flag = 0; e->G_h->tau_flag = 0; e->G_dirty = true; }
@@ -940,9 +1061,28 @@
   return rc;
 }
 
-static int sweep_launch(gph_engine *e, int flags, double ftCoal, double ftMig, int &with_sync)
-{
+static void rng_ahead_drain_if(gph_engine *e, bool stale) { if (stale && e->ra_b_valid) rng_ahead_drain(e); }
+static void rng_ahead_dirty(gph_engine *e) { rng_ahead_drain_if(e, true); e->ra_b_valid = false; }
+static int rng_ahead_launch(gph_engine *e)
+{
+  if (e->dev.ra_M <= 0) return 0;
   int rc;
+  if ((rc = flush_pending(e))) return rc;
+  launch_pre(e);
+  const int tms = tm_begin(e, 18);
+  if ((rc = launch_grid(e, GphGrid{(int)((e->L + GPH_WAVE - 1) / GPH_WAVE), 1}, GPH_WAVE, 0, k_rng_ahead, e->ka, e->dev))) return rc;
+  tm_end(e, tms);
+  e->cls_launches[18] += 1; e->n_launches++;
+  return 0;
+}
+
+static int sweep_launch(gph_engine *e, int flags, double ftCoal, double ftMig, int &with_sync, bool chained = false)
+{
+  int rc;
+  const bool side = chained && e->ra_place_b && e->dev.ra_M > 0 && resident(e);
+  const bool have = side && e->ra_b_valid;
+  rng_ahead_drain_if(e, !have);
+  e->ra_b_valid = false;
   with_sync = e->sync_pending ? 8 : 0;
   e->sync_pending = false;
   int with_mix = 0;
@@ -951,7 +1091,15 @@
     e->mix_owed = false;
     if (e->G_h->mix_flag) with_mix = 16;
   }
+  if (have) { if ((rc = flush_pending(e)) || (rc = rng_ahead_wait(e))) return rc; }
+  else if ((rc = rng_ahead_launch(e))) return rc;
   if ((rc = launch_loci(e, 0, k_sweep, flags | with_sync | with_mix, ftCoal, ftMig, e->G_h->mix_c, e->G_h->mix_lnc))) return rc;
+  if (side) {
+    launch_pre(e);
+    if ((rc = rng_ahead_side(e, GphGrid{(int)((e->L + GPH_WAVE - 1) / GPH_WAVE), 1}))) return rc;
+    e->cls_launches[18] += 1; e->n_launches++;
+    e->ra_b_valid = true;
+  }
   if ((rc = reduce_local(e, 0, GPH_OUT_SLOTS))) return rc;
   return reduce_stats(e);
 }
@@ -1212,6 +1360,26 @@
 {
   if (!x || !y || !out || n <= 0) return GPH_EARG;
   return debug_math(x, y, n, out, device);
+}
+
+int gph_engine_rng_ahead_(gph_engine *e, int32_t *info, int32_t *kprev, int32_t set)
+{
+  if (!e || !e->loaded) return GPH_EARG;
+  SETDEV(e);
+  if (info) { if (set < 0) { info[0] = e->ra_place_b && e->dev.ra_M > 0 && resident(e); info[1] = e->ra_b_valid; return 0; }
+    info[0] = e->dev.ra_M > 0; info[1] = e->dev.ra_M; info[2] = 1 << e->dev.ra_cshift; info[3] = (int32_t)(e->ra_bytes / (size_t)e->L); }
+  if (!kprev) return 0;
+  if (e->dev.ra_M <= 0) return GPH_ESTATE;
+  if (e->initialized) { int rcs = finish_sync(e); if (rcs) return rcs; }
+  std::vector<int32_t> by_slot((size_t)e->L);
+  if (set) {
+    rng_ahead_dirty(e);
+    for (int64_t j = 0; j < e->L; j++) by_slot[j] = kprev[e->h_orig[j]];
+    return h2d(e, e->dev.ra_kprev, by_slot.data(), sizeof(int32_t) * e->L);
+  }
+  if (d2h(e, by_slot.data(), e->dev.ra_kprev, sizeof(int32_t) * e->L)) return GPH_EHIP;
+  for (int64_t j = 0; j < e->L; j++) kprev[e->h_orig[j]] = by_slot[j];
+  return 0;
 }
 
 #ifndef GPH_BUILD_ID
@@ -1290,7 +1458,7 @@
 int gph_engine_hbm_bytes(gph_engine *e, double *bytes)
 {
   if (!e || !bytes) return GPH_EARG;
-  *bytes = 2.0 * e->pages_bytes + (double)e->cond_bytes + (double)e->seq_bytes_total + 8.0 * GPH_OUT_SLOTS * e->L;
+  *bytes = 2.0 * e->pages_bytes + (double)e->cond_bytes + (double)e->seq_bytes_total + 8.0 * GPH_OUT_SLOTS * e->L + (double)e->ra_bytes;
   return 0;
 }
 
@@ -1336,6 +1504,7 @@
   if (!e || !e->initialized || !io) return GPH_ESTATE;
   io->accepted = 0;
   if (finetune <= 0.0) return 0;
+  rng_ahead_dirty(e);
   const bool owner = e->cfg.locus_begin == 0;
   SETDEV(e);
   if (!multi_rank(e) && (!owner || e->cfg.L_total != e->L)) {
@@ -1501,10 +1670,10 @@
   if ((rc = launch_loci(e, cls, kernel, fuse))) return rc;
   return reduce_local(e, 0, GPH_OUT_SLOTS);
 }
-static int part_sweep(gph_engine *e, int32_t iteration, double ftCoal, double ftMig)
+static int part_sweep(gph_engine *e, int32_t iteration, double ftCoal, double ftMig, bool chained = false)
 {
   int rc, with_sync;
-  if ((rc = sweep_launch(e, 7, ftCoal, ftMig, with_sync))) return rc;
+  if ((rc = sweep_launch(e, 7, ftCoal, ftMig, with_sync, chained))) return rc;
   return run_stage(e, GS_SWEEP_DONE, with_sync, iteration);
 }
 static int part_lrate(gph_engine *e, int32_t iteration, const double *lr_alpha_finetune, int64_t *lr_accepted, double *lr_rateVar)
@@ -1584,7 +1753,7 @@
   int rc;
   GphGlobal &Gh = *e->G_h;
   if ((rc = push_if_dirty(e))) return rc;
-  if ((rc = part_sweep(e, iteration, Gh.ftCoalTime, Gh.ftMigTime))) return rc;
+  if ((rc = part_sweep(e, iteration, Gh.ftCoalTime, Gh.ftMigTime, true))) return rc;
   if (lr_alpha_finetune && (rc = part_lrate(e, iteration, lr_alpha_finetune, lr_accepted, lr_rateVar))) return rc;
   if ((rc = run_stage(e, GS_THETA, 0, iteration))) return rc;
   if (Gh.Kc < Gh.K && (rc = run_stage(e, GS_TAU_PROPOSE, Gh.Kc, iteration))) return rc;
@@ -1610,6 +1779,7 @@
   SETDEV(e);
   int rc = 0;
   GphGlobal &Gh = *e->G_h;
+  rng_ahead_dirty(e);
   if ((rc = push_if_dirty(e))) return rc;
   if (part != GPH_PART_SWEEP && part != GPH_PART_SYNC) { int rcm = mix_finish_owed(e); if (rcm) return rcm; }
   if (part == GPH_PART_LRATE || part == GPH_PART_TAU || part == GPH_PART_SAGE || part == GPH_PART_MIX) {
@@ -1642,6 +1812,7 @@
   if ((op == 3 || op == 6) && (arg < 0 || arg >= 2 * e->cfg.n - 1)) return GPH_EARG;
   if (op == 8 && (arg < 0 || arg > 100000)) return GPH_EARG;
   SETDEV(e);
+  rng_ahead_dirty(e);
   { int rcs = flush_sync(e, true); if (!rcs) rcs = finish_sync(e); if (rcs) return rcs; }
   if (op == 2) {
     if (arg < e->cfg.Kc || arg >= e->cfg.K) return GPH_EARG;
diff --git a/g-phocs_amd/csrc/gph_kernels.h b/g-phocs_amd/csrc/gph_kernels.h
--- a/g-phocs_amd/csrc/gph_kernels.h
+++ b/g-phocs_amd/csrc/gph_kernels.h
@@ -20,6 +20,11 @@
   double *slog;
   int32_t *slog_n;
   int32_t slog_cap, pad_;
+  double *ra_draws;
+  uint32_t *ra_ckpt;
+  uint32_t *ra_tail;
+  int32_t *ra_kprev;
+  int32_t ra_M, ra_cshift;
 };
 
 #include "gph_locus.h"
@@ -405,7 +410,7 @@
   OUT(g, 7, gf64(&GphLds::s_cntf, 6));
 }
 
-GPH_DEV void kb_sweep(const GphDev &D, int g, int flags, double ftCoal, double ftMig, double mix_c, double mix_lnc)
+template <class RNG> GPH_DEV void kb_sweep_(const GphDev &D, int g, int flags, double ftCoal, double ftMig, double mix_c, double mix_lnc)
 {
   STAMP_BEGIN(0);
   if (flags & 16) {
@@ -415,21 +420,28 @@
     stage_in(D, g, D.pages, 1);
   }
   GPH_SLOG_OPEN(D, g);
-  GphRngB rng;
-  rng_load(rng);
+  RNG rng;
+  rng_load(rng, D, g);
   OUT(g, 15, (flags & 8) ? (double)synchronize_events() : 1.0);
   OUT(g, 0, 0.0); OUT(g, 1, 0.0); OUT(g, 2, 0.0); OUT(g, 3, 0.0); OUT(g, 4, 0.0);
   OUT(g, 5, 0.0); OUT(g, 6, 0.0); OUT(g, 7, 0.0); OUT(g, 12, 0.0);
   { STAMP_BEGIN(5); if ((flags & 1) && ftCoal > 0.0) sweep_internal(D, g, ftCoal, rng); STAMP_END(5); }
   { STAMPC_BEGIN(4); if ((flags & 2) && ftMig > 0.0 && !gph_failed()) sweep_mignodes(D, g, ftMig, rng); STAMPC_END(4); }
   { STAMP_BEGIN(6); if ((flags & 4) && !gph_failed()) sweep_spr(D, g, rng); STAMP_END(6); }
-  rng_store(rng);
+  rng_store(rng, D, g);
   out_common(D, g);
   STAMP_END(0);
 #if defined(GPH_STAMPS) && !defined(GPH_HOSTEMU)
   for (int k = 0; k < 8; k++) OUT(g, k, gph_lds.s_stamp[k]);
 #endif
   stage_out(D, g, D.pages, 1);
+}
+GPH_DEV void kb_sweep(const GphDev &D, int g, int flags, double ftCoal, double ftMig, double mix_c, double mix_lnc)
+{
+#ifdef GPH_HOSTEMU
+  if (D.ra_M <= 0) { kb_sweep_<GphRng>(D, g, flags, ftCoal, ftMig, mix_c, mix_lnc); return; }
+#endif
+  kb_sweep_<GphRngA>(D, g, flags, ftCoal, ftMig, mix_c, mix_lnc);
 }
 
 GPH_DEV void kb_tau_eval(const GphDev &D, int g, gph_ctau &A, int fuse)
diff --git a/g-phocs_amd/csrc/gph_locus.h b/g-phocs_amd/csrc/gph_locus.h
--- a/g-phocs_amd/csrc/gph_locus.h
+++ b/g-phocs_amd/csrc/gph_locus.h
@@ -275,133 +275,125 @@
   r = (r - (int)r);
   return r;
 }
+GPH_DEV void rng_load(GphRng &g, const GphDev &, int) { rng_load(g); }
+GPH_DEV void rng_store(const GphRng &g, const GphDev &, int) { rng_store(g); }
+#define GPH_RNG_STEP(x, y, z) do { x = 171u * x - 30269u * (x / 177u); y = 172u * y - 30307u * (y / 176u); z = 170u * z - 30323u * (z / 178u); } while (0)
 #ifdef GPH_HOSTEMU
-typedef GphRng GphRngB;
+struct GphRngA {
+  int k;
+  double u[64];
+};
 #else
-#ifndef GPH_RNG_BATCH
-#define GPH_RNG_BATCH 16
-#endif
-struct GphRngB {
-  int pos;
+struct GphRngA {
+  int k;
   double u;
 };
-GPH_DEV void rng_load(GphRngB &g)
-{
-  setCNT(CN_RX, ISC(IS_RX)); setCNT(CN_RY, ISC(IS_RY)); setCNT(CN_RZ, ISC(IS_RZ));
-  g.pos = GPH_RNG_BATCH; g.u = 0.0;
-}
-GPH_DEV void rng_store(const GphRngB &g)
-{
-  uint32_t x = (uint32_t)CNT(CN_RX), y = (uint32_t)CNT(CN_RY), z = (uint32_t)CNT(CN_RZ);
-  if (g.pos < GPH_RNG_BATCH) {
-    x = (uint32_t)ISC(IS_RX); y = (uint32_t)ISC(IS_RY); z = (uint32_t)ISC(IS_RZ);
-    for (int k = 0; k < g.pos; k++) {
-      x = 171u * x - 30269u * (x / 177u);
-      y = 172u * y - 30307u * (y / 176u);
-      z = 170u * z - 30323u * (z / 178u);
-    }
-  }
-  setISC(IS_RX, (int)x); setISC(IS_RY, (int)y); setISC(IS_RZ, (int)z);
-}
-#ifndef GPH_RNG_ROLLED
-template <int K> GPH_DEV void rng_steps_(uint32_t &x, uint32_t &y, uint32_t &z, int &vx, int &vy, int &vz)
-{
-  if constexpr (K < GPH_RNG_BATCH) {
-    x = 171u * x - 30269u * (x / 177u);
-    y = 172u * y - 30307u * (y / 176u);
-    z = 170u * z - 30323u * (z / 178u);
-    asm("v_writelane_b32 %0, %3, %6\n\tv_writelane_b32 %1, %4, %6\n\tv_writelane_b32 %2, %5, %6"
-        : "+v"(vx), "+v"(vy), "+v"(vz) : "s"(x), "s"(y), "s"(z), "i"(K));
-    rng_steps_<K + 1>(x, y, z, vx, vy, vz);
-  }
-}
-#endif
-#ifndef GPH_RNG_VECTOR_REFILL
-GPH_DEV void rng_refill(GphRngB &g)
-{
-  uint32_t x = (uint32_t)CNT(CN_RX), y = (uint32_t)CNT(CN_RY), z = (uint32_t)CNT(CN_RZ);
-  int vx = 0, vy = 0, vz = 0;
-  setISC(IS_RX, (int)x); setISC(IS_RY, (int)y); setISC(IS_RZ, (int)z);
-#ifndef GPH_RNG_ROLLED
-  rng_steps_<0>(x, y, z, vx, vy, vz);
-#else
-#pragma unroll 4
-  for (int k = 0; k < GPH_RNG_BATCH; k++) {
-    x = 171u * x - 30269u * (x / 177u);
-    y = 172u * y - 30307u * (y / 176u);
-    z = 170u * z - 30323u * (z / 178u);
-    asm("s_mov_b32 m0, %6\n\ts_nop 0\n\tv_writelane_b32 %0, %3, m0\n\tv_writelane_b32 %1, %4, m0\n\tv_writelane_b32 %2, %5, m0"
-        : "+v"(vx), "+v"(vy), "+v"(vz) : "s"(x), "s"(y), "s"(z), "s"(k) : "m0");
-  }
-#endif
-  setCNT(CN_RX, (int)x); setCNT(CN_RY, (int)y); setCNT(CN_RZ, (int)z);
+struct GphRngChunk { double u; int x, y, z; };
+#ifndef GPH_RNG_CHUNK_ATTR
+#define GPH_RNG_CHUNK_ATTR __noinline__
+#endif
+static __device__ GPH_RNG_CHUNK_ATTR GphRngChunk rng_chunk64(uint32_t x_, uint32_t y_, uint32_t z_)
+{
+  uint32_t x = (uint32_t)__builtin_amdgcn_readfirstlane((int)x_), y = (uint32_t)__builtin_amdgcn_readfirstlane((int)y_),
+           z = (uint32_t)__builtin_amdgcn_readfirstlane((int)z_);
+  uint32_t vx = 0, vy = 0, vz = 0;
+  const int lane = GPH_LANE;
+  GphRngChunk r;
+  r.u = 0.0;
+#pragma unroll 1
+  for (int k = 0; k < 64; k++) {
+    GPH_RNG_STEP(x, y, z);
+    const bool mine = lane == k;
+    vx = mine ? x : vx; vy = mine ? y : vy; vz = mine ? z : vz;
+  }
 #if defined(__HIP_DEVICE_COMPILE__)
   {
-    const gph_cdbl *RC = GPH_RNGC;
-    const double rx = RC[0], ry = RC[1], rz = RC[2], mx = RC[3], my = RC[4], mz = RC[5];
-    double xd = (double)(uint32_t)vx, yd = (double)(uint32_t)vy, zd = (double)(uint32_t)vz, q;
+    const double rx = 1.0 / 30269.0, ry = 1.0 / 30307.0, rz = 1.0 / 30323.0, mx = 30269.0, my = 30307.0, mz = 30323.0;
+    double xd = (double)vx, yd = (double)vy, zd = (double)vz, q;
     q = xd * rx; double qx = __builtin_fma(__builtin_fma(-q, mx, xd), rx, q);
     q = yd * ry; double qy = __builtin_fma(__builtin_fma(-q, my, yd), ry, q);
     q = zd * rz; double qz = __builtin_fma(__builtin_fma(-q, mz, zd), rz, q);
-    g.u = __builtin_amdgcn_fract(qx + qy + qz);
-  }
-#endif
-  g.pos = 0;
-}
+    r.u = __builtin_amdgcn_fract(qx + qy + qz);
+  }
+#endif
+  r.x = (int)x; r.y = (int)y; r.z = (int)z;
+  return r;
+}
+#endif
+GPH_DEV void rng_load(GphRngA &g, const GphDev &D, int slot)
+{
+  g.k = 0;
+#ifndef GPH_HOSTEMU
+  g.u = 0.0;
+#endif
+  if (D.ra_M > 0) {
+    const uint32_t *t = D.ra_tail + 4 * (size_t)GPH_IX(slot, D.L);
+    const uint64_t a = (uint64_t)(uintptr_t)(D.ra_draws + (size_t)slot * D.ra_M);
+    setCNT(CN_RX, (int)t[0]); setCNT(CN_RY, (int)t[1]); setCNT(CN_RZ, (int)t[2]); setCNT(CN_RAN, (int)t[3]);
+    setCNT(CN_RALO, (int)(uint32_t)a); setCNT(CN_RAHI, (int)(uint32_t)(a >> 32));
+  } else {
+    setCNT(CN_RX, ISC(IS_RX)); setCNT(CN_RY, ISC(IS_RY)); setCNT(CN_RZ, ISC(IS_RZ));
+  }
+}
+GPH_DEV void rng_refill(GphRngA &g)
+{
+  if (g.k < CNT(CN_RAN)) {
+    const uint64_t a = (uint64_t)(uint32_t)CNT(CN_RALO) | ((uint64_t)(uint32_t)CNT(CN_RAHI) << 32);
+#ifdef GPH_HOSTEMU
+    for (int i = 0; i < 64; i++) g.u[i] = ((const double *)(uintptr_t)a)[GPH_IX(g.k + i, CNT(CN_RAN))];
 #else
-#define GPH_RNGV_STEP \
-  "v_mul_hi_u32 %[q], %[st], %[mg]\n\t" \
-  "v_mul_lo_u32 %[t], %[st], %[a]\n\t" \
-  "v_sub_u32 %[st], %[st], %[q]\n\t" \
-  "v_lshrrev_b32 %[st], 1, %[st]\n\t" \
-  "v_add_u32 %[st], %[st], %[q]\n\t" \
-  "v_lshrrev_b32 %[st], 7, %[st]\n\t" \
-  "v_mul_lo_u32 %[st], %[st], %[nm]\n\t" \
-  "v_add_u32 %[st], %[st], %[t]\n\t" \
-  "v_cndmask_b32_dpp %[h], %[h], %[st], vcc row_shl:1 row_mask:0xf bank_mask:0xf bound_ctrl:0\n\t"
-#define GPH_RNGV_STEP4 GPH_RNGV_STEP GPH_RNGV_STEP GPH_RNGV_STEP GPH_RNGV_STEP
-GPH_DEV void rng_refill(GphRngB &g)
-{
-  static_assert(GPH_RNG_BATCH == 16, "one draw per lane of a 16-lane row");
-  const uint32_t x0 = (uint32_t)CNT(CN_RX), y0 = (uint32_t)CNT(CN_RY), z0 = (uint32_t)CNT(CN_RZ);
-  setISC(IS_RX, (int)x0); setISC(IS_RY, (int)y0); setISC(IS_RZ, (int)z0);
-#if defined(__HIP_DEVICE_COMPILE__)
-  const int row = GPH_LANE >> 4;
-  const bool r0 = row == 0, r1 = row == 1;
-  uint32_t st = r0 ? x0 : r1 ? y0 : z0, h = 0, q, t;
-  const uint32_t mg = r0 ? 0x724287f5u : r1 ? 0x745d1746u : 0x702e05c1u;
-  const uint32_t a = r0 ? 171u : r1 ? 172u : 170u;
-  const uint32_t nm = r0 ? 0u - 30269u : r1 ? 0u - 30307u : 0u - 30323u;
-  asm("s_mov_b32 vcc_lo, 0x80008000\n\t"
-      "s_mov_b32 vcc_hi, 0x80008000\n\t"
-      GPH_RNGV_STEP4 GPH_RNGV_STEP4 GPH_RNGV_STEP4 GPH_RNGV_STEP4
-      : [st] "+v"(st), [h] "+v"(h), [q] "=&v"(q), [t] "=&v"(t) : [mg] "v"(mg), [a] "v"(a), [nm] "v"(nm) : "vcc");
-  setCNT(CN_RX, __builtin_amdgcn_readlane((int)st, 0)); setCNT(CN_RY, __builtin_amdgcn_readlane((int)st, 16));
-  setCNT(CN_RZ, __builtin_amdgcn_readlane((int)st, 32));
-  {
-    const gph_cdbl *RC = GPH_RNGC;
-    const double rr = r0 ? RC[0] : r1 ? RC[1] : RC[2], mm = r0 ? RC[3] : r1 ? RC[4] : RC[5];
-    const double hd = (double)h, q0 = hd * rr;
-    const double qq = __builtin_fma(__builtin_fma(-q0, mm, hd), rr, q0);
-    union { double d; int32_t i[2]; } u, vy, vz;
-    u.d = qq;
-    const int ay = (GPH_LANE + 16) << 2, az = (GPH_LANE + 32) << 2;
-    vy.i[0] = __builtin_amdgcn_ds_bpermute(ay, u.i[0]); vy.i[1] = __builtin_amdgcn_ds_bpermute(ay, u.i[1]);
-    vz.i[0] = __builtin_amdgcn_ds_bpermute(az, u.i[0]); vz.i[1] = __builtin_amdgcn_ds_bpermute(az, u.i[1]);
-    g.u = __builtin_amdgcn_fract(qq + vy.d + vz.d);
-  }
-#endif
-  g.pos = 0;
-}
-#endif
-GPH_DEV double l_rndu(GphRngB &g)
-{
-  if (g.pos >= GPH_RNG_BATCH) rng_refill(g);
-  const double u = gph_readlane64(g.u, g.pos);
-  g.pos++;
+    int lane = GPH_LANE;
+    asm volatile("" : "+v"(lane));
+    g.u = *(const GPH_GLB double *)((const GPH_GLB char *)(uintptr_t)a + (uint32_t)(GPH_IX(g.k + lane, CNT(CN_RAN)) << 3));
+#endif
+    return;
+  }
+  uint32_t x = (uint32_t)CNT(CN_RX), y = (uint32_t)CNT(CN_RY), z = (uint32_t)CNT(CN_RZ);
+  setISC(IS_RX, (int)x); setISC(IS_RY, (int)y); setISC(IS_RZ, (int)z);
+#ifdef GPH_HOSTEMU
+  for (int i = 0; i < 64; i++) {
+    GPH_RNG_STEP(x, y, z);
+    const double r = x / 30269.0 + y / 30307.0 + z / 30323.0;
+    g.u[i] = r - (int)r;
+  }
+  setCNT(CN_RX, (int)x); setCNT(CN_RY, (int)y); setCNT(CN_RZ, (int)z);
+#else
+  const GphRngChunk c = rng_chunk64(x, y, z);
+  setCNT(CN_RX, c.x); setCNT(CN_RY, c.y); setCNT(CN_RZ, c.z);
+  g.u = c.u;
+#endif
+}
+GPH_DEV double l_rndu(GphRngA &g)
+{
+  if ((g.k & 63) == 0) rng_refill(g);
+#ifdef GPH_HOSTEMU
+  const double u = g.u[g.k & 63];
+#else
+  const double u = gph_readlane64(g.u, g.k & 63);
+#endif
+  g.k++;
   return u;
 }
-#endif
+GPH_DEV void rng_store(const GphRngA &g, const GphDev &D, int slot)
+{
+  const int k = g.k;
+  if (k > 0) {
+    uint32_t x, y, z;
+    int r;
+    if (k <= CNT(CN_RAN)) {
+      const int j = k >> D.ra_cshift;
+      const uint32_t *c = D.ra_ckpt + 4 * ((size_t)GPH_IX(j, (D.ra_M >> D.ra_cshift) + 1) * D.L + GPH_IX(slot, D.L));
+      x = (uint32_t)RFL(c[0]); y = (uint32_t)RFL(c[1]); z = (uint32_t)RFL(c[2]);
+      r = k & ((1 << D.ra_cshift) - 1);
+    } else {
+      x = (uint32_t)ISC(IS_RX); y = (uint32_t)ISC(IS_RY); z = (uint32_t)ISC(IS_RZ);
+      r = k - ((k - 1) & ~63);
+    }
+    for (int i = 0; i < r; i++) GPH_RNG_STEP(x, y, z);
+    setISC(IS_RX, (int)x); setISC(IS_RY, (int)y); setISC(IS_RZ, (int)z);
+  }
+  if (D.ra_M > 0 && GPH_LANE == 0) D.ra_kprev[GPH_IX(slot, D.L)] = k;
+}
 template <class RNG> GPH_DEV double l_rndnormal(RNG &g)
 {
   double u, v, s;
diff --git a/g-phocs_amd/csrc/gph_types.h b/g-phocs_amd/csrc/gph_types.h
--- a/g-phocs_amd/csrc/gph_types.h
+++ b/g-phocs_amd/csrc/gph_types.h
@@ -98,7 +98,7 @@
 enum { DI_ORIG = 0, DI_UPD, DI_DLIN, DI_NEV, DI_NPOPS, DI_NBANDS, DI_SRCPOP, DI_TGTPOP, DI_COUNT };
 enum { SI_FEV_OLD = 0, SI_FEV_NEW, SI_FPOP_NEW, SI_TARGET, SI_NOLD, SI_NNEW, SI_COUNT };
 enum { SA_OLD = 0, SA_NEWIN, SA_NEWOUT, SA_NEWBAND };
-enum { CN_EVALS = 0, CN_NODES, CN_ERROR, CN_P, CN_NOTENOUGH, CN_RX, CN_RY, CN_RZ, CN_EMPTY, CN_NODES0, CN_QPH, CN_QCNT, CN_QTERMS, CN_SUMLDS, CN_HUGE, CN_SEQLO, CN_SEQHI, CN_COUNT };
+enum { CN_EVALS = 0, CN_NODES, CN_ERROR, CN_P, CN_NOTENOUGH, CN_RX, CN_RY, CN_RZ, CN_EMPTY, CN_NODES0, CN_QPH, CN_QCNT, CN_QTERMS, CN_SUMLDS, CN_HUGE, CN_SEQLO, CN_SEQHI, CN_RAN, CN_RALO, CN_RAHI, CN_COUNT };
 
 enum { FS_DATALNL = 0, FS_SV_DATALNL, FS_GENLNL, FS_GENDELTA, FS_MUTRATE, FS_COUNT };
 enum { IS_ROOT = 0, IS_SV_ROOT, IS_DIRTY0, IS_CBIT0 = IS_DIRTY0 + GPH_NSW, IS_SAVED0 = IS_CBIT0 + GPH_NSW,
```

Measured after the change: 450.3 million, median of 6. +3.1%, better.
